# ugadiarov-la-phystech-edu/OCRL

Measured on AMD Instinct MI355X. Metric: images/sec (node) SLATE pretrain 128x128, 6 slots, 3 iters, higher is better.
Workload: dtype f32

## Files before the change

ocrl_amd/_lib.py:

```python
import ctypes
import os
from ctypes import c_void_p

from . import _abi

_HERE = os.path.dirname(os.path.abspath(__file__))
LIB_PATH = os.environ.get("OCRL_HIP_LIB") or os.path.join(_HERE, "libocrl_hip.so")
HEADER_PATH = os.path.join(_HERE, os.pardir, "include", "ocrl_hip.h")
DQN_HEADER_PATH = os.path.join(_HERE, os.pardir, "include", "ocrl_hip_dqn.h")
ROLLOUT_HEADER_PATH = os.path.join(_HERE, os.pardir, "include", "ocrl_hip_rollout.h")
_lib = None

if not os.path.exists(HEADER_PATH):
    raise RuntimeError(f"{HEADER_PATH} is missing: ocrl_amd derives its binding of libocrl_hip.so from the header and runs from the source tree.")
with open(HEADER_PATH) as _f:
    ABI = _abi.read(_f.read())
CONSTANTS = ABI.consts
SlateConfig, IodineConfig, GemmDesc, ConvDesc, ConvWgradDesc, XattnDesc, AcnetDesc, SpriteEnvDesc, ScenesDesc, FlatSegment = (
    ABI.structs["ocrl_" + n] for n in ("slate_config", "iodine_config", "gemm_desc", "conv_desc", "conv_wgrad_desc", "xattn_desc", "acnet_desc",
                                       "sprite_env_desc", "scenes_desc", "flat_segment"))
FLAT_MAX_SEGMENTS = CONSTANTS["OCRL_FLAT_MAX_SEGMENTS"]
if not os.path.exists(DQN_HEADER_PATH):
    raise RuntimeError(f"{DQN_HEADER_PATH} is missing: ocrl_amd derives its binding of libocrl_hip.so from the header and runs from the source tree.")
with open(DQN_HEADER_PATH) as _f:
    ABI_DQN = _abi.read(_f.read())
QnetDesc = ABI_DQN.structs["ocrl_qnet_desc"]
QNET_MAX_LAYERS = len(QnetDesc().dims)
if not os.path.exists(ROLLOUT_HEADER_PATH):
    raise RuntimeError(f"{ROLLOUT_HEADER_PATH} is missing: ocrl_amd derives its binding of libocrl_hip.so from the header and runs from the source tree.")
with open(ROLLOUT_HEADER_PATH) as _f:
    ABI_ROLLOUT = _abi.read(_f.read())


def flat_segments(segs):
    addr = lambda a: a.value if isinstance(a, c_void_p) else a
    return (FlatSegment * len(segs))(*[FlatSegment(addr(p), addr(g), addr(s0), addr(s1), int(n)) for p, g, s0, s1, n in segs])


def acnet_desc(B, F, A, dims, acts):
    d = AcnetDesc(B=B, F=F, A=A)
    for t in range(3):
        if len(dims[t]) > CONSTANTS["OCRL_ACNET_MAX_LAYERS"]:
            raise ValueError(f"ocrl_amd: at most {CONSTANTS['OCRL_ACNET_MAX_LAYERS']} layers per trunk (got {len(dims[t])})")
        d.n[t] = len(dims[t])
        for l, (w, a) in enumerate(zip(dims[t], acts[t])):
            d.dims[t][l], d.acts[t][l] = int(w), int(a)
    return d


def qnet_desc(B, F, A, dims, acts):
    if len(dims) > QNET_MAX_LAYERS or len(acts) != len(dims):
        raise ValueError(f"ocrl_amd: at most {QNET_MAX_LAYERS} hidden layers, one activation code each (got {len(dims)}, {len(acts)})")
    d = QnetDesc(B=B, F=F, A=A, n=len(dims))
    for l, (w, a) in enumerate(zip(dims, acts)):
        d.dims[l], d.acts[l] = int(w), int(a)
    return d


def gemm_desc(**kw):
    d = GemmDesc(batch=1, batch_inner=1, splitk=1, alpha=1.0, x_scale=1.0, e_scale=1.0, force_sb=-1)
    for k, v in kw.items():
        setattr(d, k, v)
    return d


def conv_desc(**kw):
    d = ConvDesc()
    for k, v in kw.items():
        setattr(d, k, v)
    return d


def conv_wgrad_desc(**kw):
    d = ConvWgradDesc()
    for k, v in kw.items():
        setattr(d, k, v)
    return d


def lib():
    global _lib
    if _lib is not None:
        return _lib
    if not os.path.exists(LIB_PATH):
        raise RuntimeError(
            f"{LIB_PATH} is missing: build it with `python -c 'import __graft_entry__ as g; g.build()'` "
            "(make -C ocrl_amd/csrc).  ocrl_amd has no CPU fallback.")
    import torch
    L = ctypes.CDLL(LIB_PATH)
    for abi in (ABI, ABI_DQN, ABI_ROLLOUT):
        for name, (restype, argtypes) in abi.functions.items():
            f = getattr(L, name)
            f.argtypes = argtypes
            if restype is not ctypes.c_int:
                f.restype = restype
    for name, cls in {**ABI.structs, **ABI_DQN.structs}.items():
        if name + "_size" in {**ABI.functions, **ABI_DQN.functions} and getattr(L, name + "_size")() != ctypes.sizeof(cls):
            raise RuntimeError(f"libocrl_hip.so: {name} is {getattr(L, name + '_size')()} bytes, this binding's {cls.__name__} {ctypes.sizeof(cls)}")
    if L.ocrl_abi_version() != CONSTANTS["OCRL_ABI_VERSION"]:
        raise RuntimeError(f"libocrl_hip.so ABI version mismatch: the library is {L.ocrl_abi_version()}, include/ocrl_hip.h {CONSTANTS['OCRL_ABI_VERSION']}")
    _lib = L
    return L


def check(rc):
    if rc:
        raise RuntimeError("ocrl_hip: " + lib().ocrl_last_error().decode())


def ptr(t):
    return None if t is None else ctypes.c_void_p(t.data_ptr())


def ptrs(ts):
    return (ctypes.c_void_p * len(ts))(*[t.data_ptr() if t is not None else None for t in ts])


def stream(device=None):
    import torch
    return ctypes.c_void_p(torch.cuda.current_stream(device).cuda_stream)
```

ocrl_amd/csrc/kernels.h:

```cpp
#pragma once
#include "common.h"
#include "../../include/ocrl_hip.h"

enum { PROF_CONV5 = 0, PROF_CONV_OTHER = 1, PROF_WGRAD = 2, PROF_GEMM = 3, PROF_SA_FWD = 4, PROF_SA_BWD = 5, PROF_ATTN_FWD = 6, PROF_ATTN_BWD = 7, PROF_NTAGS = 8 };
int prof_begin(int tag, hipStream_t st);
void prof_end(int idx, hipStream_t st);

struct GemmArgs {
    const float* A = nullptr;
    const float* B = nullptr;
    float* C = nullptr;
    int M = 0, N = 0, K = 0;
    int lda = 0, ldb = 0, ldc = 0;
    int akc = 1, bkc = 1;
    int batch = 1;
    int batch_inner = 1;
    long long sA = 0, sB = 0, sC = 0;
    long long sAi = 0, sBi = 0, sCi = 0;
    int splitk = 1;
    long long sCsplit = 0;
    float alpha = 1.f;
    const float* bias = nullptr;
    int relu = 0;
    float drop_p = 0.f;
    unsigned long long drop_seed = 0;
    unsigned drop_site = 0;
    const float* mask = nullptr; int ldmask = 0; long long sMask = 0;
    int mask_elu = 0;
    const float* resid = nullptr; int ldr = 0; long long sR = 0;
    float adrop_p = 0.f; unsigned adrop_site = 0; int adrop_ld = 0;
    float* bias_out = nullptr; long long sBias = 0;
    int a_mode = 0, b_mode = 0;
    const float* x_lse = nullptr; const int* x_tok = nullptr; float x_scale = 1.f;
    int epi_mode = 0;
    float* stat = nullptr; float* hstat = nullptr; int* hidx = nullptr;
    const float* e1 = nullptr; const float* e2 = nullptr; unsigned long long e_seed = 0;
    const float* e_lse = nullptr; const float* e_rowvec = nullptr; float e_scale = 1.f;
    int force_tile = 0;
    int force_sb = -1;
};
inline int gemm_stat_segments(int N) { return 2 * ((N + 127) / 128); }
struct GemmPlan { int bm = 0, bn = 0, sb = 0, xf = 0, epi = 0, layout = 0; };
int gemm_plan(const GemmArgs& a, GemmPlan* plan);
int gemm_launch(const GemmArgs& a, hipStream_t st);
int splitk_reduce_launch(const float* part, float* out, long long n, int splits, long long stride,
                         int accumulate, hipStream_t st);
void gemm_splitk_layout(GemmArgs& a, float* ws, long long bslab);
int gemm_splitk_launch(GemmArgs a, float* ws, long long bslab, int accumulate, hipStream_t st);

struct Drop { float p = 0.f; unsigned long long seed = 0; unsigned site = 0; };
struct Xf { int a_mode = 0, b_mode = 0; const float* lse = nullptr; const int* tok = nullptr; float scale = 1.f; };
int lin_fwd(const float* x, int ldx, const float* W, const float* b, float* y, int ldy, long long M, int N, int K, int relu, const float* resid,
            int ldr, hipStream_t st, Drop dr = Drop());
int lin_bwd_x(const float* dy, int ld_dy, const float* W, float* dx, int ldx, long long M, int N_out, int K_in, const float* mask, int ldmask,
              const float* resid, int ldr, hipStream_t st, Drop dr = Drop(), Xf xf = Xf(), float alpha = 1.f);
int lin_bwd_w(const float* dy, int ld_dy, const float* x, int ldx, float* dW, float* db, long long M, int N_out, int K_in, float alpha, float* sk,
              size_t sk_floats, hipStream_t st, Drop dr = Drop(), Xf xf = Xf(), int accumulate = 0, int max_splits = 0);

int pool_embed_launch(const float* lin, const float* cls, const float* pos, float* x0, int B, int K, int d, hipStream_t st);
int pool_rows_launch(const float* in, float* out, int B, int K, int d, int mode, hipStream_t st);
int pool_attn_launch(const float* qkv, float* P, float* O, const float* dO, float* dqkv, int B, int S, int d, int h, float p, unsigned long long seed,
                     unsigned site, int backward, hipStream_t st);

int pool_cols_launch(const float* src, int lds, float* dst, int ldd, long long rows, int ncols, int ncopy, hipStream_t st);
int pool_cls_drop_launch(const float* x, const float* resid, int ldr, float* out, int B, int N, int S, float p, unsigned long long seed, unsigned site,
                         hipStream_t st);
int pool_cls_add_launch(float* dX, const float* v, int B, int d, int S, hipStream_t st);
int pool_cls_nchunk(int B, int S, int* chunk);
struct PoolClsArgs {
    const float* X = nullptr;
    const float* Win = nullptr; const float* bin = nullptr;
    const float* q = nullptr;
    float* U = nullptr;
    float* part = nullptr;
    float* z = nullptr;
    float* stat = nullptr;
    float* o = nullptr;
    const float* dO = nullptr;
    float* G = nullptr; float* gD = nullptr;
    float* dX = nullptr;
    float* w = nullptr; float* dq = nullptr;
    const float* x0 = nullptr;
    float* dW = nullptr; float* db = nullptr;
    int B = 0, S = 0, d = 0, h = 0;
    float p = 0.f; unsigned long long seed = 0; unsigned site = 0;
};
int pool_cls_attn_fwd_launch(const PoolClsArgs& a, hipStream_t st);
int pool_cls_attn_bwd_launch(const PoolClsArgs& a, hipStream_t st);
int pool_flash_launch(const float* qkv, float* O, float* lse, const float* dO, float* Dd, float* dqkv, int B, int S, int d, int h, float p,
                      unsigned long long seed, unsigned site, int backward, hipStream_t st);

int rn_pair_fwd_launch(const float* AB, const float* b1, float* h1, int B, int K, int g, hipStream_t st);
int rn_pair_bwd_launch(const float* dh1, float* dAB, int B, int K, int g, hipStream_t st);
int rn_pairsum_fwd_launch(const float* gL, float* y, int B, int P, int g, hipStream_t st);
int rn_pairsum_bwd_launch(const float* dy, const float* gL, float* dgL, int B, int P, int g, hipStream_t st);

struct NcMap { long long sN = 0, sG = 0, sC = 0, sH = 0, sW = 0; };
struct NcFwdArgs {
    const float* X = nullptr; NcMap x;
    float* Y = nullptr; float* Y2 = nullptr; NcMap y;
    const float* w[OCRL_NATURECNN_MAX_GROUPS] = {}; const float* bias[OCRL_NATURECNN_MAX_GROUPS] = {};
    int B = 0, G = 1, cin = 0, cout = 0, H = 0, W = 0, OH = 0, OW = 0, ks = 0, stride = 0;
    int pad = 0;
};
struct NcBwdArgs {
    const float* X = nullptr; NcMap x;
    const float* dY = nullptr; NcMap dy;
    float* dX = nullptr;
    float* part = nullptr;
    int slabs = 1, slab_rows = 0;
    const float* w[OCRL_NATURECNN_MAX_GROUPS] = {};
    int B = 0, G = 1, cin = 0, cout = 0, H = 0, W = 0, OH = 0, OW = 0, ks = 0, stride = 0;
    int pad = 0;
    long long dw_tiles = 0, dx_tiles = 0; int dw_blocks = 0;
};
struct NcReduceLayer { const float* part = nullptr; int slabs = 0, G = 0, cout = 0, K = 0; long long n = 0; };
struct NcReduceArgs {
    NcReduceLayer L[OCRL_NATURECNN_MAX_CONVS];
    float* dw[OCRL_NATURECNN_MAX_CONVS][OCRL_NATURECNN_MAX_GROUPS] = {};
    float* db[OCRL_NATURECNN_MAX_CONVS][OCRL_NATURECNN_MAX_GROUPS] = {};
    int nlayers = 0;
};
int nc_conv_fwd_launch(const NcFwdArgs& a, hipStream_t st);
int nc_conv_bwd_launch(NcBwdArgs a, hipStream_t st);
int nc_dw_reduce_launch(const NcReduceArgs& a, hipStream_t st);
int nc_relu_mask_launch(const float* d, const float* act, float* out, long long n, hipStream_t st);

struct PcGeom {
    int OH = 0, OW = 0, OWT = 0;
    int NG = 0, nchunk = 0;
    size_t wp_floats = 0;
    long long units = 0; int slab_units = 0, slabs = 0; size_t part_floats = 0;
    int passes = 0, nbg = 0, Dp = 0; size_t wd_floats = 0;
    int HB = 0, WB = 0, WT = 0; long long dx_units = 0; int upw = 0;
};
PcGeom pc_geom(int B, int H, int W, int D);
struct PcFwdArgs {
    const float* X = nullptr; const float* Wp = nullptr; const float* bias = nullptr; float* Y = nullptr;
    int B = 0, H = 0, W = 0, D = 0, OH = 0, OW = 0, OWT = 0, nchunk = 0, NG = 0;
};
struct PcDwArgs {
    const float* X = nullptr; const float* dY = nullptr; float* part = nullptr; float* partb = nullptr;
    int B = 0, H = 0, W = 0, D = 0, OH = 0, OW = 0, OWT = 0, nchunk = 0, slab_units = 0;
    long long units = 0;
};
struct PcDxArgs {
    const float* dY = nullptr; const float* Wd = nullptr; float* dX = nullptr;
    int H = 0, W = 0, D = 0, OH = 0, OW = 0, HB = 0, WT = 0, Dp = 0, passes = 0, upw = 0;
    long long units = 0, groups = 0;
};
int pc_conv1_fwd_launch(const float* X, const float* w, const float* bias, float* Wp, float* Y, int B, int H, int W, int D, hipStream_t st);
int pc_conv1_dw_launch(const float* X, const float* dY, float* part, int B, int H, int W, int D, hipStream_t st);
int pc_conv1_dw_reduce_launch(const float* part, float* dw, float* db, int B, int H, int W, int D, hipStream_t st);
int pc_conv1_dx_launch(const float* dY, const float* w, float* Wd, float* dX, int B, int H, int W, int D, hipStream_t st);

#define PROBE_MAX_SLOTS 12
#define PROBE_MAX_PROPS 8
#define PROBE_MAX_WIDTH 256
struct ProbeSchema { int P; int t[PROBE_MAX_PROPS], a[PROBE_MAX_PROPS], b[PROBE_MAX_PROPS], kind[PROBE_MAX_PROPS]; };
int probe_schema_check(const ProbeSchema& sc, int T, int O);
int probe_match_check(int B, int K, int N, int T, int O);
int probe_match_launch(const float* out, int ld_row, long long ld_img, const float* y, const float* dloss, float* cost, int* col, float* part,
                       float* metrics, float* dout, int B, int K, int N, int T, int O, const ProbeSchema& sc, hipStream_t st);
int probe_leaky_fwd_launch(float* x, long long n, float slope, hipStream_t st);
int probe_leaky_bwd_launch(float* dx, const float* h, long long n, float slope, hipStream_t st);

int vae_permute_launch(const float* src, float* dst, long long R, int C, int HW, int rows, int pack, hipStream_t st);
int vae_pad_rows_launch(const float* src, float* dst, int rows, int rows_pad, int K, hipStream_t st);
int vae_kl_fwd_launch(const float* ml, const float* eps, float* latent, float* part, float* rep, int B, int L, hipStream_t st);
int vae_loss_launch(const float* part, float* metrics, int B, float kld_weight, hipStream_t st);
int vae_kl_bwd_launch(const float* ml, const float* eps, const float* dlat, const float* drep, const float* dloss, float* dml, int B, int L,
                      float kld_weight, hipStream_t st);
int vae_scale_launch(const float* x, float* y, const float* g, long long n, hipStream_t st);
int vae_recon_nchw_launch(const float* r4, float* out, int B, int C, int HW, hipStream_t st);

#define MAE_MAX_PATCHES 1024
int mae_rank_launch(const float* noise, int* restore, int* keep, float* mask, int* restore_out, float* mask_out, int B, int L, int len_keep,
                    hipStream_t st);
int mae_patch_gather_launch(const float* obs, const int* ids, float* out, int B, int n, int S, int p, hipStream_t st);
int mae_tokens_fwd_launch(const float* embed, const float* cls, const float* pos, const int* ids, float* x0, int B, int n, int D, hipStream_t st);
int mae_tokens_bwd_launch(const float* dx0, float* dembed, float* dcls, int B, int n, int D, hipStream_t st);
int mae_unshuffle_fwd_launch(const float* e, const float* mtok, const float* dpos, const int* restore, float* xd, int B, int L, int len_keep, int Dd,
                             hipStream_t st);
int mae_unshuffle_bwd_launch(const float* dxd, const int* keep, const float* mask, float* de, float* dmtok, float* part, int B, int L, int len_keep,
                             int Dd, hipStream_t st);
int mae_gelu_fwd_launch(const float* pre, float* y, long long n, hipStream_t st);
int mae_gelu_bwd_launch(const float* dy, const float* pre, float* dpre, long long n, hipStream_t st);
int mae_ln_fwd_launch(const float* x, const float* g, const float* b, float* y, float* mean, float* rstd, long long R, int F, float eps, hipStream_t st);
int mae_ln_chunks(long long R);
int mae_ln_bwd_launch(const float* dy, const float* x, const float* mean, const float* rstd, const float* g, const float* resid, float* dx, float* dg,
                      float* db, float* part, long long R, int F, hipStream_t st);
int mae_loss_launch(const float* pred, const float* obs, const float* mask, const float* dloss, float* part, float* loss, float* dpred, int B, int L,
                    int len_keep, int S, int p, hipStream_t st);

struct ConvArgs {
    const float* X = nullptr;
    const float* Wp = nullptr;
    float* Y = nullptr;
    int B = 0, H = 0, W = 0;
    const float* bias = nullptr;
    int relu = 0;
    const float* posmap = nullptr;
    const float* mask = nullptr;
    int mask_elu = 0;
};
size_t conv_x3_pack_floats(int KS = 5);
int conv_pack_x3_launch(const float* W, float* fwd3, float* bwd3, hipStream_t st, int KS = 5);
int conv_x3_launch(const ConvArgs& a, const float* pack3, hipStream_t st, int KS = 5);
struct WgradArgs;
int conv_wgrad_x3_stage(const WgradArgs& a, int nchunk, hipStream_t st, int KS = 5);
struct WgradArgs {
    const float* X = nullptr;
    const float* dY = nullptr;
    float* part = nullptr;
    int B = 0, H = 0, W = 0;
    float* bpart = nullptr;
};
int conv_fwd_launch(const ConvArgs& a, int KS, int CIN, int COUT, hipStream_t st, int low_latency = 0);
int conv_wgrad_launch(const WgradArgs& a, int KS, int CIN, int COUT, int cin_real, float* dW, float* db, int accumulate, hipStream_t st, int x3 = -1);
int conv_wgrad_slabs(int B, int H, int W, int KS, int CIN);
size_t conv_wgrad_ws_floats(int B, int H, int W, int KS, int CIN, bool with_db = true);
int conv_pack_launch(const float* W, float* fwd, float* bwd, int KS, int CIN, int COUT, int cin_real, hipStream_t st);

size_t conv_first_pack_floats();
int conv_first_pack_launch(const float* W, float* pack, hipStream_t st);
int conv_first_fwd_launch(const float* obs, const float* pack, const float* bias, float* Y, int B, int H, int W, int relu, hipStream_t st);
int conv_first_wgrad_workers(int B, int H, int W);
size_t conv_first_wgrad_ws_floats(int B, int H, int W);
int conv_first_wgrad_launch(const float* obs, const float* dY, float* ws, float* dW, float* db, int B, int H, int W, int accumulate, hipStream_t st);

int nchw_to_nhwc8_launch(const float* in, float* out, int B, int C, int H, int W, hipStream_t st);
int patchify4_launch(const float* in, float* out, int B, int C, int S, hipStream_t st);
int pixel_shuffle_launch(const float* in, float* out, int B, int h, int w, int Cout, int forward, const float* mask, hipStream_t st);
int layernorm_fwd_launch(const float* x, const float* g, const float* b, float* y, float* mean, float* rstd, long long R, int F, hipStream_t st);
int layernorm_bwd_launch(const float* dy, const float* x, const float* mean, const float* rstd, const float* g, float* dx,
                         float* dgb, long long R, int F, int accumulate_dx, int accumulate_dgb, float* ws, size_t ws_floats, hipStream_t st);
int colsum_launch(const float* X, long long ld, float* out, long long R, int F, int accumulate, float scale, float* ws, size_t ws_floats, hipStream_t st);

#define SA_INPUT_SLAB (2 * 4096 + 4 * 64)
void sa_input_plan(long long R, int max_wgs, int out[3]);
int sa_input_fwd_launch(const float* e4, const float* gamma, const float* beta, const float* W0, const float* b0, const float* W2, const float* b2,
                        float* mean, float* rstd, float* ln0, float* h1, float* x, long long R, int max_wgs, hipStream_t st);
int sa_input_bwd_launch(const float* dx, const float* h1, const float* e4, const float* mean, const float* rstd, const float* gamma, const float* beta,
                        const float* W0, const float* W2, float* de4, float* dW0, float* db0, float* dW2, float* db2, float* dgamma, float* dbeta,
                        long long R, int max_wgs, float* ws, size_t ws_floats, hipStream_t st);
int reduce_partials_launch(const float* part, int n, float* out, float scale, int accumulate, hipStream_t st);
int mse_launch(const float* obs, const float* recon, float* drecon, float* out, int B, int C, int H, int W, float* ws, size_t ws_floats, hipStream_t st);
int gumbel_softmax_launch(const float* raw, const float* e1, const float* e2, float* z, int* tokens, long long R, int V, float tau,
                          unsigned long long seed, hipStream_t st, float* zst = nullptr);
int softmax_bwd_rows_launch(const float* z, float* d, long long R, int V, float scale, hipStream_t st);
int softmax_stat_combine_launch(const float* stat, int nseg, long long R, float* lse, const float* hstat, const int* hidx, int* tokens,
                                const float* pred, int ldp, const int* tok, float* out, float scale, float* ws, size_t ws_floats, hipStream_t st,
                                const float* cdf_scores = nullptr, int cdf_V = 0, float cdf_tau = 1.f, unsigned long long cdf_seed = 0);
int exp_rows_launch(const float* y, const float* lse, float* z, long long R, int V, hipStream_t st);
int rowdot_bias64_launch(const float* g, const float* act, const float* bias, long long R, float* out, hipStream_t st);
int embed_fwd_launch(const int* tokens, const float* dict, const float* bos, const float* pe, float* out, int B, int T, int d, float p,
                     unsigned long long seed, hipStream_t st);
size_t embed_bwd_ws_floats(long long BT, int V, int d);
int embed_bwd_launch(float* g, const int* tokens, float* ddict, int B, int T, int V, int d, float p, unsigned long long seed, float* ws,
                     size_t ws_floats, hipStream_t st);
int dropout_apply_launch(const float* x, float* y, long long n, float p, unsigned long long seed, unsigned site, hipStream_t st);
int dropout_mask_launch(float* y, long long n, float p, unsigned long long seed, unsigned site, hipStream_t st);
int obs_u8_to_f32_launch(const unsigned char* in, float* out, int B, int H, int W, int C, hipStream_t st);
int fill_launch(float* x, long long n, float v, hipStream_t st);
int axpy_launch(const float* x, float* y, long long n, float a, hipStream_t st);
int posmap_launch(const float* Wpos, const float* bpos, float* out, int S, int C, hipStream_t st);
int posgrid_launch(float* out, int S, hipStream_t st);
int im2col5_launch(const float* x8, float* col, long long npix, int H, int W, int C, int ldc, hipStream_t st);
int unpack5_launch(const float* dWp, float* dW, int C, int ldc, hipStream_t st);
int pad_cols_launch(const float* in, int ldi, float* out, int ldo, long long R, int C, int Cout, hipStream_t st);

struct XaPlan { bool supported = false; int KP = 0, NC = 0, NM = 0; size_t lds = 0; };
bool xattn_plan(int K, int d, int h, XaPlan* out);
bool xattn_supported(int K, int d, int h);
int xattn_kp(int K, int h);
struct XaFoldHost {
    const float* mem = nullptr;
    const float* Wq[8]; const float* Wk[8]; const float* Wv[8]; const float* Wo[8];
    float* ck[8]; float* cv[8];
    float* Ab[8]; float* AbT[8]; float* Vo[8]; float* VoT[8];
    int B = 0, K = 0, d = 0, h = 0, nblk = 0;
};
int xattn_fold_fwd_launch(const XaFoldHost& f, hipStream_t st);
struct XaHost {
    const float* x = nullptr;
    const float* resid = nullptr;
    float* y = nullptr;
    float* P = nullptr;
    const float *Ab = nullptr, *AbT = nullptr, *Vo = nullptr, *VoT = nullptr;
    const float* gd = nullptr;
    float *Pd = nullptr, *dS = nullptr;
    int B = 0, T = 0, K = 0, d = 0, h = 0;
    float p = 0.f; unsigned long long seed = 0; unsigned site_p = 0, site_o = 0;
};
int xattn_launch(const XaHost& h, int backward, hipStream_t st);
struct XaFoldBwdHost {
    const float *Pd = nullptr, *dS = nullptr;
    const float *gd = nullptr, *x = nullptr;
    const float *Wq = nullptr, *Wo = nullptr;
    const float *ck = nullptr, *cv = nullptr;
    float *dVo = nullptr, *dAb = nullptr;
    float *dck = nullptr, *dcv = nullptr;
    float *pq = nullptr, *po = nullptr;
    float *dWq = nullptr, *dWo = nullptr;
    float* ws = nullptr; size_t ws_floats = 0;
    int B = 0, T = 0, K = 0, d = 0, h = 0;
};
int xattn_fold_bwd_launch(const XaFoldBwdHost& f, hipStream_t st);
int cross_attn_fwd_launch(const float* Q, const float* Km, const float* Vm, float* O, float* P, int B, int T, int K, int d, int h, float p,
                          unsigned long long seed, unsigned site, hipStream_t st);
size_t cross_attn_bwd_ws_floats(int B, int T, int K, int d, int h);
int cross_attn_bwd_launch(const float* dO, const float* Q, const float* Km, const float* Vm, const float* P, float* dQ, float* dKm, float* dVm,
                          int B, int T, int K, int d, int h, float p, unsigned long long seed, unsigned site, float* part, size_t part_floats,
                          hipStream_t st);


struct SaWts {
    int ln_in_g, ln_in_b, ln_s_g, ln_s_b, ln_m_g, ln_m_b;
    int Wq, WqT, Wk, WkT, Wv, WvT, Wih, WihT, Whh, WhhT, bih, bhh, W0, W0T, b0, W2, W2T, b2;
    int total;
};
static inline SaWts sa_wts_layout(int C, int D, int H) {
    SaWts o; int a = 0;
    auto take = [&](int n) { int r = a; a += (n + 3) & ~3; return r; };
    o.ln_in_g = take(C); o.ln_in_b = take(C); o.ln_s_g = take(D); o.ln_s_b = take(D); o.ln_m_g = take(D); o.ln_m_b = take(D);
    o.Wq = take(D * D); o.WqT = take(D * D); o.Wk = take(D * C); o.WkT = take(C * D); o.Wv = take(D * C); o.WvT = take(C * D);
    o.Wih = take(3 * D * D); o.WihT = take(3 * D * D); o.Whh = take(3 * D * D); o.WhhT = take(3 * D * D);
    o.bih = take(3 * D); o.bhh = take(3 * D);
    o.W0 = take(H * D); o.W0T = take(H * D); o.b0 = take(H); o.W2 = take(D * H); o.W2T = take(D * H); o.b2 = take(D);
    o.total = a;
    return o;
}
struct SaSave { int sprev, sn, q, u, r, z, n, hn, sg, m, hid, qp, up, upn, csum, ld; };
static inline SaSave sa_save_layout(int C, int D, int H, int NH = 1) {
    SaSave o;
    o.sprev = 0; o.sn = D; o.q = 2 * D; o.u = 3 * D; o.r = 4 * D; o.z = 5 * D; o.n = 6 * D; o.hn = 7 * D; o.sg = 8 * D; o.m = 9 * D;
    o.hid = 10 * D; o.qp = 10 * D + H; o.up = o.qp + NH * C; o.upn = o.up + NH * C; o.csum = o.upn + NH * C; o.ld = o.csum + ((NH + 3) & ~3);
    return o;
}
struct SaGrad { int out, hid, gi, gh, u, q, qp, ld; };
static inline SaGrad sa_grad_layout(int C, int D, int H, int NH = 1) {
    SaGrad o;
    o.out = 0; o.hid = D; o.gi = D + H; o.gh = 4 * D + H; o.u = 7 * D + H; o.q = 8 * D + H; o.qp = 9 * D + H; o.ld = 9 * D + H + NH * C;
    return o;
}
struct SlotAttnArgs {
    int B = 0, N = 0, C = 64, K = 0, D = 0, H = 0, I = 0;
    int NH = 1;
    float eps = 1e-8f, scale = 1.f;
    const float* x = nullptr;
    const float* slots0 = nullptr;
    const float* wts = nullptr;
    float* slots = nullptr;
    float* attn = nullptr;
    float* attn_heads = nullptr;
    float* save = nullptr;
    const float* dslots = nullptr;
    float* dx = nullptr;
    float* dslots0 = nullptr;
    float* grows = nullptr;
    float* g_small = nullptr;
    float* xchg = nullptr;
    float* parts = nullptr;
    int phase = 0;
};
size_t sa_xchg_floats_host(int K, int D);
size_t sa_parts_floats_host(int B, int K);
struct SaPlan { int G, NB, KB, KS; size_t smem_fwd, smem_bwd; };
int sa_plan(int K, int D, int H, int NH, SaPlan* plan);
int slot_attn_launch(const SlotAttnArgs& a, int backward, hipStream_t st);

struct PackEntry { const float* src; int rows, cols, dst_off, transpose; };
int pack_launch(const PackEntry* entries_dev, int n_entries, int max_elems, float* dst, hipStream_t st);

int absmax_launch(const float* g, long long n, float* out, float* ws, size_t ws_floats, hipStream_t st);
int clip_adam_launch(float* p, const float* g, float* m, float* v, long long n, const float* norm, float clip, float lr, double b1,
                     double b2, double eps, int step, float gscale, hipStream_t st);
int clip_adam_tail_launch(float* p, const float* g, float* m, float* v, int n, const float* norm, float clip, float lr, double b1, double b2,
                          double eps, int step, float gscale, hipStream_t st);
int clip_rmsprop_launch(float* p, const float* g, float* sq, long long n, const float* norm, float clip, float lr, double alpha, double eps,
                        hipStream_t st);
int clip_rmsprop_tail_launch(float* p, const float* g, float* sq, int n, const float* norm, float clip, float lr, double alpha, double eps,
                             hipStream_t st);
constexpr int FLAT_MAX_SEG = 8, FLAT_SEG_BLOCKS = 1024;
struct FlatSegs {
    float* p[FLAT_MAX_SEG];
    const float* g[FLAT_MAX_SEG];
    float* s0[FLAT_MAX_SEG];
    float* s1[FLAT_MAX_SEG];
    long long n[FLAT_MAX_SEG];
    int blk0[FLAT_MAX_SEG + 1];
    int nseg;
};
int multi_clip_adam_launch(FlatSegs t, float* norm, float clip, float lr, double b1, double b2, double eps, int step, float* ws, size_t ws_floats,
                           hipStream_t st);
int multi_clip_rmsprop_launch(FlatSegs t, float* norm, float clip, float lr, double alpha, double eps, float* ws, size_t ws_floats, hipStream_t st);
int store_u64_launch(unsigned long long* dst, unsigned long long v, hipStream_t st);
int slot_init_launch(const float* mu, const float* logsig, const float* noise, float* slots0, int BK, int D, unsigned long long seed, hipStream_t st,
                     const unsigned long long* seed_dev = nullptr);
int slot_init_bwd_launch(const float* dslots0, const float* logsig, const float* noise, float* dmu, float* dlogsig, int BK, int D, unsigned long long seed, hipStream_t st);
int copy_launch(const float* src, float* dst, long long n, hipStream_t st);
int argmax_pos_launch(const float* pred, int* tokens, int B, int T, int V, int t, hipStream_t st, int dense_rows = 0);
int embed_step_launch(const int* tokens, const float* dict, const float* bos, const float* pe, float* out, int B, int T, int d, int t, hipStream_t st);
int decode_attn_launch(const float* qkv, float* out, int B, int T, int t, int d, int h, int ld, hipStream_t st);
int onehot_launch(const int* tokens, float* z, long long rows, int V, hipStream_t st);

struct AttnArgs {
    const float *q = nullptr, *k = nullptr, *v = nullptr;
    float* o = nullptr;
    float* lse = nullptr;
    int B = 0, T = 0, d = 0, h = 0;
    int ld = 0;
    float p = 0.f;
    unsigned long long seed = 0;
    unsigned site = 0;
    const float* dO = nullptr;
    float *dq = nullptr, *dk = nullptr, *dv = nullptr, *delta = nullptr;
    float* ds = nullptr;
    size_t ds_floats = 0;
    int b0 = 0;
};
int attn_launch(const AttnArgs& a, int mode, hipStream_t st);
size_t attn_bwd_ds_floats(int B, int T, int h);
int attn_bwd_form();
size_t attn_bwd_ds_carve_floats(int B, int T, int h);

enum { BCAST_L1_RELU = 0, BCAST_L1_ELU = 1 };
int bcast_l1_class_sum_launch(const float* in, float* out, long long BK, int ks, int forward, hipStream_t st);
int bcast_l1_fwd_launch(const float* P1, const float* T, const float* bias, float* c1, long long BK, int S, int ks, int act, hipStream_t st);
size_t bcast_l1_bwd_ws_floats(long long BK, int S, int ks);
int bcast_l1_bwd_launch(const float* g, float* dT, long long BK, int S, int ks, float* ws, size_t ws_floats, hipStream_t st);
int bc_posconv_launch(const float* Wc, float* P1, int S, hipStream_t st);
int bc_posconv_bwd_launch(const float* G, float* dWc, int S, hipStream_t st);
int io_p1_launch(const float* Wxy, const float* b1, float* P1, int S, hipStream_t st);
int io_w1_grad_launch(const float* dW1r, const float* G, float* dW1, float* db1, int S, int L, hipStream_t st);

int bc_compose_launch(const float* W1, const float* Wpos, const float* bpos, float* Wc, float* W1r, int D, hipStream_t st);
int bc_compose_bwd_launch(const float* W1, const float* Wpos, const float* bpos, const float* dWc, const float* dW1r, float* dW1,
                          float* dWpos, float* dbpos, int D, hipStream_t st);
int bc_c4_pack_launch(const float* W, float* Wk, float* Wb, int co_n, hipStream_t st);
int bc_c4_fwd_launch(const float* X, const float* Wk, const float* bias4, float* Y, int Bn, int S, hipStream_t st);
int bc_c4_bwd_data_launch(const float* dY, const float* Wb, const float* act, float* dX, int Bn, int S, hipStream_t st, int elu = 0);
int bc_c4_wgrad_blocks(int Bn, int S);
int bc_c4_wgrad_launch(const float* X, const float* dY, float* part, int Bn, int S, hipStream_t st);
int bc_mix_launch(const float* out4, const float* obs, float* recon, float* dout4, float* loss_out, int B, int K, int S, int C, float* ws,
                  size_t ws_floats, hipStream_t st);

int io_sample_launch(const float* mu, const float* ls, const float* noise, float* eps_out, float* slots, float* kl_out, long long n,
                     unsigned long long seed, unsigned site, float* ws, size_t ws_floats, hipStream_t st);
int io_w1_pack_launch(const float* W1, float* W1r, float* Wxy, int L, hipStream_t st);
int io_elbo_launch(const float* out4, const float* obs, int B, int K, int S, float sigma, float* enc, float* st1, float* dout4, float* part,
                   float* masks_out, float* recon_out, float* rmasked_out, float* ws, size_t ws_floats, hipStream_t st);
int io_enc_norm_launch(float* enc, const float* st1, float* st2, long long BK, int N, float* ws, size_t ws_floats, hipStream_t st);
int io_elbo_bwd_launch(const float* out4, const float* obs, const float* denc, int B, int K, int S, float sigma, float cw, float* dout4, hipStream_t st);
int io_latent_launch(const float* mu, const float* ls, const float* eps, const float* ds, float* latent, long long BK, int L, float beta, int layer_norm,
                     int ld, hipStream_t st);
int io_im2col_launch(const float* x, float* col, long long Bn, int C, int Hi, int Wi, int ldc, hipStream_t st);
int io_col2im_launch(const float* dcol, const float* act, float* dx, long long Bn, int C, int Hi, int Wi, int ldc, hipStream_t st);
int io_refw_pack_launch(const float* W, float* Wp, int C, int ldc, hipStream_t st);
int io_refw_unpack_launch(const float* dWp, float* dW, int C, int ldc, hipStream_t st);
int io_pool_launch(const float* r, float* pool, long long BK, int n, hipStream_t st);
int io_pool_bwd_launch(const float* dpool, const float* r, float* dpre, long long BK, int n, hipStream_t st);
int io_elu2_launch(const float* a, int lda, float* y, int ldy, long long rows, int F, const float* dy, int lddy, hipStream_t st);
int io_lstm_fwd_launch(const float* gates, const float* c0, float* acts, float* c1, float* h1, long long rows, int H, hipStream_t st);
int io_lstm_bwd_launch(const float* acts, const float* c0, const float* c1, const float* dh1, const float* dc1, float* dgates, float* dc0,
                       long long rows, int H, hipStream_t st);
int io_post_grad_launch(const float* mu, const float* ls, const float* eps, const float* ds, const float* dlat, int ldl, float kw, float* gmu,
                        float* gls, long long BK, int L, hipStream_t st);
int io_l2norm_launch(const float* g, long long n, float* out, float* ws, size_t ws_floats, hipStream_t st);
int io_loss_launch(const float* parts, float* metrics, int I, int B, float beta, hipStream_t st);
```

ocrl_amd/csrc/sa_input.hip:

```cpp
#include "common.h"
#include "kernels.h"
#include "layernorm16.h"

#define SAI_TR 64
#define SAI_LD 68
#define SAI_MAX_WGS 512
#define SAI_FWD_MAX_WGS 768

__device__ __forceinline__ float4 sai_ld4(const float* __restrict__ p, long long row, long long R, int c4) {
    const float4 v = *reinterpret_cast<const float4*>(p + (row < R ? row : R - 1) * 64 + c4 * 4);
    return row < R ? v : make_float4(0.f, 0.f, 0.f, 0.f);
}
__device__ __forceinline__ float sai_ld1(const float* __restrict__ p, long long row, long long R) {
    const float v = p[row < R ? row : R - 1];
    return row < R ? v : 0.f;
}

__device__ __forceinline__ void sai_mma_kc(const float* __restrict__ as, const float (&wf)[8][4], f32x16& acc) {
    const int lane = threadIdx.x & 63, li = lane & 31, lh = lane >> 5;
#pragma unroll
    for (int c = 0; c < 8; ++c) {
        const float4 v = *reinterpret_cast<const float4*>(as + li * SAI_LD + c * 8 + 4 * lh);
        acc = __builtin_amdgcn_mfma_f32_32x32x2f32(v.x, wf[c][0], acc, 0, 0, 0);
        acc = __builtin_amdgcn_mfma_f32_32x32x2f32(v.y, wf[c][1], acc, 0, 0, 0);
        acc = __builtin_amdgcn_mfma_f32_32x32x2f32(v.z, wf[c][2], acc, 0, 0, 0);
        acc = __builtin_amdgcn_mfma_f32_32x32x2f32(v.w, wf[c][3], acc, 0, 0, 0);
    }
}
__device__ __forceinline__ void sai_mma_rows(const float* __restrict__ as, const float* __restrict__ bs, f32x16& acc) {
    const int lane = threadIdx.x & 63, li = lane & 31, lh = lane >> 5;
#pragma unroll 2
    for (int c = 0; c < 8; ++c) {
        float fa[4], fb[4];
#pragma unroll
        for (int j = 0; j < 4; ++j) {
            fa[j] = as[(c * 8 + 4 * lh + j) * SAI_LD + li];
            fb[j] = bs[(c * 8 + 4 * lh + j) * SAI_LD + li];
        }
#pragma unroll
        for (int s = 0; s < 4; ++s) acc = __builtin_amdgcn_mfma_f32_32x32x2f32(fa[s], fb[s], acc, 0, 0, 0);
    }
}

__global__ __launch_bounds__(256, 3) void sa_input_fwd_kernel(const float* __restrict__ e4, const float* __restrict__ g, const float* __restrict__ bta,
                                                              const float* __restrict__ W0, const float* __restrict__ b0,
                                                              const float* __restrict__ W2, const float* __restrict__ b2,
                                                              float* __restrict__ mean, float* __restrict__ rstd, float* __restrict__ ln0,
                                                              float* __restrict__ h1, float* __restrict__ x, long long R) {
    __shared__ __attribute__((aligned(16))) float At[SAI_TR * SAI_LD], Ht[SAI_TR * SAI_LD];
    const int lane = threadIdx.x & 63, wv = threadIdx.x >> 6, c4 = lane & 15, rsub = lane >> 4;
    const int li = lane & 31, lh = lane >> 5;
    const int wm0 = (wv >> 1) * 32, wn0 = (wv & 1) * 32;
    float w0f[8][4], w2f[8][4];
#pragma unroll
    for (int c = 0; c < 8; ++c) {
        const float4 a = *reinterpret_cast<const float4*>(W0 + (wn0 + li) * 64 + c * 8 + 4 * lh);
        const float4 b = *reinterpret_cast<const float4*>(W2 + (wn0 + li) * 64 + c * 8 + 4 * lh);
        w0f[c][0] = a.x; w0f[c][1] = a.y; w0f[c][2] = a.z; w0f[c][3] = a.w;
        w2f[c][0] = b.x; w2f[c][1] = b.y; w2f[c][2] = b.z; w2f[c][3] = b.w;
    }
    const float b0v = b0[wn0 + li], b2v = b2[wn0 + li];
    const float4 gg = *reinterpret_cast<const float4*>(g + c4 * 4), bb = *reinterpret_cast<const float4*>(bta + c4 * 4);
    const long long ntiles = (R + SAI_TR - 1) / SAI_TR;
    const int lr0 = wv * 16 + rsub;
    float4 v[4];
#pragma unroll
    for (int i = 0; i < 4; ++i) v[i] = sai_ld4(e4, (long long)blockIdx.x * SAI_TR + lr0 + 4 * i, R, c4);
    for (long long tile = blockIdx.x; tile < ntiles; tile += gridDim.x) {
        const long long r0 = tile * SAI_TR;
#pragma unroll
        for (int i = 0; i < 4; ++i) {
            const int lr = lr0 + 4 * i;
            const long long row = r0 + lr;
            float mu, rs;
            layernorm16_row_fwd<1>(&v[i], mu, rs);
            const float4 y = layernorm16_affine(v[i], rs, gg, bb);
            *reinterpret_cast<float4*>(At + lr * SAI_LD + c4 * 4) = y;
            if (row < R) {
                if (ln0) *reinterpret_cast<float4*>(ln0 + row * 64 + c4 * 4) = y;
                if (c4 == 0) { mean[row] = mu; rstd[row] = rs; }
            }
        }
#pragma unroll
        for (int i = 0; i < 4; ++i) v[i] = sai_ld4(e4, (tile + gridDim.x) * SAI_TR + lr0 + 4 * i, R, c4);
        __syncthreads();
        f32x16 acc;
#pragma unroll
        for (int r = 0; r < 16; ++r) acc[r] = 0.f;
        sai_mma_kc(At + wm0 * SAI_LD, w0f, acc);
#pragma unroll
        for (int r = 0; r < 16; ++r) {
            const int row = (r & 3) + 8 * (r >> 2) + 4 * lh;
            Ht[(wm0 + row) * SAI_LD + wn0 + li] = fmaxf(acc[r] + b0v, 0.f);
        }
        __syncthreads();
#pragma unroll
        for (int r = 0; r < 16; ++r) acc[r] = 0.f;
        sai_mma_kc(Ht + wm0 * SAI_LD, w2f, acc);
#pragma unroll
        for (int r = 0; r < 16; ++r) {
            const int row = (r & 3) + 8 * (r >> 2) + 4 * lh;
            At[(wm0 + row) * SAI_LD + wn0 + li] = acc[r] + b2v;
        }
        __syncthreads();
#pragma unroll
        for (int i = 0; i < 4; ++i) {
            const int lr = lr0 + 4 * i;
            const long long row = r0 + lr;
            if (row < R) {
                *reinterpret_cast<float4*>(h1 + row * 64 + c4 * 4) = *reinterpret_cast<const float4*>(Ht + lr * SAI_LD + c4 * 4);
                *reinterpret_cast<float4*>(x + row * 64 + c4 * 4) = *reinterpret_cast<const float4*>(At + lr * SAI_LD + c4 * 4);
            }
        }
        __syncthreads();
    }
}

__global__ __launch_bounds__(256, 2) void sa_input_bwd_kernel(const float* __restrict__ dx, const float* __restrict__ h1, const float* __restrict__ e4,
                                                              const float* __restrict__ mean, const float* __restrict__ rstd,
                                                              const float* __restrict__ g, const float* __restrict__ bta,
                                                              const float* __restrict__ W0, const float* __restrict__ W2,
                                                              float* __restrict__ de4, float* __restrict__ slab, long long R) {
    __shared__ __attribute__((aligned(16))) float T0[SAI_TR * SAI_LD], T1[SAI_TR * SAI_LD], T2[SAI_TR * SAI_LD], W0s[64 * 64], W2s[32 * 64];
    const int lane = threadIdx.x & 63, wv = threadIdx.x >> 6, c4 = lane & 15, rsub = lane >> 4;
    const int li = lane & 31, lh = lane >> 5;
    const int wm0 = (wv >> 1) * 32, wn0 = (wv & 1) * 32;
    float w2f[4][4];
#pragma unroll
    for (int c = 0; c < 4; ++c)
#pragma unroll
        for (int j = 0; j < 4; ++j) w2f[c][j] = W2[(c * 8 + 4 * lh + j) * 64 + wn0 + li];
#pragma unroll
    for (int i = 0; i < 4; ++i)
        *reinterpret_cast<float4*>(W0s + (threadIdx.x + 256 * i) * 4) = *reinterpret_cast<const float4*>(W0 + (threadIdx.x + 256 * i) * 4);
#pragma unroll
    for (int i = 0; i < 2; ++i)
        *reinterpret_cast<float4*>(W2s + (threadIdx.x + 256 * i) * 4) = *reinterpret_cast<const float4*>(W2 + 2048 + (threadIdx.x + 256 * i) * 4);
    f32x16 dW2a, dW0a;
#pragma unroll
    for (int r = 0; r < 16; ++r) { dW2a[r] = 0.f; dW0a[r] = 0.f; }
    float4 dg = make_float4(0.f, 0.f, 0.f, 0.f), db = dg, db2 = dg;
    float db0 = 0.f;
    const long long ntiles = (R + SAI_TR - 1) / SAI_TR;
    const int lr0 = wv * 16 + rsub;
    float4 dxn[4], hn[4];
#pragma unroll
    for (int i = 0; i < 4; ++i) {
        dxn[i] = sai_ld4(dx, (long long)blockIdx.x * SAI_TR + lr0 + 4 * i, R, c4);
        hn[i] = sai_ld4(h1, (long long)blockIdx.x * SAI_TR + lr0 + 4 * i, R, c4);
    }
    for (long long tile = blockIdx.x; tile < ntiles; tile += gridDim.x) {
        const long long r0 = tile * SAI_TR;
        float4 xe[4];
        float mu[4], rs[4];
        __syncthreads();
#pragma unroll
        for (int i = 0; i < 4; ++i) {
            const int lr = lr0 + 4 * i;
            *reinterpret_cast<float4*>(T0 + lr * SAI_LD + c4 * 4) = dxn[i];
            *reinterpret_cast<float4*>(T1 + lr * SAI_LD + c4 * 4) = hn[i];
            db2.x += dxn[i].x; db2.y += dxn[i].y; db2.z += dxn[i].z; db2.w += dxn[i].w;
            xe[i] = sai_ld4(e4, r0 + lr, R, c4);
            mu[i] = sai_ld1(mean, r0 + lr, R);
            rs[i] = sai_ld1(rstd, r0 + lr, R);
        }
#pragma unroll
        for (int i = 0; i < 4; ++i) {
            dxn[i] = sai_ld4(dx, (tile + gridDim.x) * SAI_TR + lr0 + 4 * i, R, c4);
            hn[i] = sai_ld4(h1, (tile + gridDim.x) * SAI_TR + lr0 + 4 * i, R, c4);
        }
        __syncthreads();
        f32x16 acc;
#pragma unroll
        for (int r = 0; r < 16; ++r) acc[r] = 0.f;
#pragma unroll
        for (int c = 0; c < 4; ++c) {
            const float4 a = *reinterpret_cast<const float4*>(T0 + (wm0 + li) * SAI_LD + c * 8 + 4 * lh);
            acc = __builtin_amdgcn_mfma_f32_32x32x2f32(a.x, w2f[c][0], acc, 0, 0, 0);
            acc = __builtin_amdgcn_mfma_f32_32x32x2f32(a.y, w2f[c][1], acc, 0, 0, 0);
            acc = __builtin_amdgcn_mfma_f32_32x32x2f32(a.z, w2f[c][2], acc, 0, 0, 0);
            acc = __builtin_amdgcn_mfma_f32_32x32x2f32(a.w, w2f[c][3], acc, 0, 0, 0);
        }
#pragma unroll 2
        for (int c = 4; c < 8; ++c) {
            const float4 a = *reinterpret_cast<const float4*>(T0 + (wm0 + li) * SAI_LD + c * 8 + 4 * lh);
            const float* const wk = W2s + ((c - 4) * 8 + 4 * lh) * 64 + wn0 + li;
            acc = __builtin_amdgcn_mfma_f32_32x32x2f32(a.x, wk[0], acc, 0, 0, 0);
            acc = __builtin_amdgcn_mfma_f32_32x32x2f32(a.y, wk[64], acc, 0, 0, 0);
            acc = __builtin_amdgcn_mfma_f32_32x32x2f32(a.z, wk[128], acc, 0, 0, 0);
            acc = __builtin_amdgcn_mfma_f32_32x32x2f32(a.w, wk[192], acc, 0, 0, 0);
        }
#pragma unroll
        for (int r = 0; r < 16; ++r) {
            const int idx = (wm0 + (r & 3) + 8 * (r >> 2) + 4 * lh) * SAI_LD + wn0 + li;
            const float mk = T1[idx];
            float t = acc[r];
            t = mk > 0.f ? t : 0.f * t * (mk + 1.f);
            T2[idx] = t;
            db0 += t;
        }
        sai_mma_rows(T0 + wm0, T1 + wn0, dW2a);
        __syncthreads();
        const float4 gg = *reinterpret_cast<const float4*>(g + c4 * 4), bb = *reinterpret_cast<const float4*>(bta + c4 * 4);
#pragma unroll
        for (int i = 0; i < 4; ++i) {
            const float4 dd = make_float4(xe[i].x - mu[i], xe[i].y - mu[i], xe[i].z - mu[i], xe[i].w - mu[i]);
            *reinterpret_cast<float4*>(T1 + (lr0 + 4 * i) * SAI_LD + c4 * 4) = layernorm16_affine(dd, rs[i], gg, bb);
        }
#pragma unroll
        for (int r = 0; r < 16; ++r) acc[r] = 0.f;
#pragma unroll 2
        for (int c = 0; c < 8; ++c) {
            const float4 a = *reinterpret_cast<const float4*>(T2 + (wm0 + li) * SAI_LD + c * 8 + 4 * lh);
            const float* const wk = W0s + (c * 8 + 4 * lh) * 64 + wn0 + li;
            acc = __builtin_amdgcn_mfma_f32_32x32x2f32(a.x, wk[0], acc, 0, 0, 0);
            acc = __builtin_amdgcn_mfma_f32_32x32x2f32(a.y, wk[64], acc, 0, 0, 0);
            acc = __builtin_amdgcn_mfma_f32_32x32x2f32(a.z, wk[128], acc, 0, 0, 0);
            acc = __builtin_amdgcn_mfma_f32_32x32x2f32(a.w, wk[192], acc, 0, 0, 0);
        }
#pragma unroll
        for (int r = 0; r < 16; ++r) T0[(wm0 + (r & 3) + 8 * (r >> 2) + 4 * lh) * SAI_LD + wn0 + li] = acc[r];
        __syncthreads();
        sai_mma_rows(T2 + wm0, T1 + wn0, dW0a);
#pragma unroll
        for (int i = 0; i < 4; ++i) {
            const int lr = lr0 + 4 * i;
            const long long row = r0 + lr;
            const float4 yv = *reinterpret_cast<const float4*>(T0 + lr * SAI_LD + c4 * 4);
            const Ln16Bwd<1> r = layernorm16_row_bwd<1>(&xe[i], &yv, mu[i], rs[i], &gg, &dg, &db);
            if (row < R) *reinterpret_cast<float4*>(de4 + row * 64 + c4 * 4) = layernorm16_row_dx(r, rs[i], 0);
        }
    }
    float* const sl = slab + (size_t)blockIdx.x * SA_INPUT_SLAB;
#pragma unroll
    for (int r = 0; r < 16; ++r) {
        const int o = (wm0 + (r & 3) + 8 * (r >> 2) + 4 * lh) * 64 + wn0 + li;
        sl[o] = dW2a[r];
        sl[4096 + o] = dW0a[r];
    }
    __syncthreads();
    float4* const red = reinterpret_cast<float4*>(T0);
    red[(0 * 16 + wv * 4 + rsub) * 16 + c4] = db2;
    red[(1 * 16 + wv * 4 + rsub) * 16 + c4] = dg;
    red[(2 * 16 + wv * 4 + rsub) * 16 + c4] = db;
    T1[(wv * 2 + lh) * 32 + li] = db0;
    __syncthreads();
    if (threadIdx.x < 48) {
        const int which = threadIdx.x >> 4, c = threadIdx.x & 15;
        float4 a = red[(which * 16) * 16 + c];
#pragma unroll
        for (int k = 1; k < 16; ++k) { const float4 t = red[(which * 16 + k) * 16 + c]; a.x += t.x; a.y += t.y; a.z += t.z; a.w += t.w; }
        *reinterpret_cast<float4*>(sl + 8192 + (which == 0 ? 0 : which == 1 ? 128 : 192) + c * 4) = a;
    } else if (threadIdx.x >= 64 && threadIdx.x < 128) {
        const int col = threadIdx.x - 64, wn = col >> 5, i = col & 31;
        sl[8192 + 64 + col] = ((T1[((0 * 2 + wn) * 2 + 0) * 32 + i] + T1[((0 * 2 + wn) * 2 + 1) * 32 + i]) +
                               (T1[((1 * 2 + wn) * 2 + 0) * 32 + i] + T1[((1 * 2 + wn) * 2 + 1) * 32 + i]));
    }
}

__global__ __launch_bounds__(256) void sa_input_reduce_kernel(const float* __restrict__ slab, int nslab, float* __restrict__ dW2, float* __restrict__ dW0,
                                                              float* __restrict__ db2, float* __restrict__ db0, float* __restrict__ dgam,
                                                              float* __restrict__ dbet) {
    __shared__ float red[8][32];
    const int ci = threadIdx.x & 31, grp = threadIdx.x >> 5, col = blockIdx.x * 32 + ci;
    const int per = (nslab + 7) / 8, s0 = grp * per, s1 = min(nslab, s0 + per);
    float a = 0.f;
    for (int s = s0; s < s1; ++s) a += slab[(size_t)s * SA_INPUT_SLAB + col];
    red[grp][ci] = a;
    __syncthreads();
    if (threadIdx.x < 32) {
        float t = red[0][ci];
#pragma unroll
        for (int k = 1; k < 8; ++k) t += red[k][ci];
        float* out = col < 4096 ? dW2 + col : col < 8192 ? dW0 + (col - 4096) : col < 8256 ? db2 + (col - 8192) : col < 8320 ? db0 + (col - 8256)
                   : col < 8384 ? dgam + (col - 8320) : dbet + (col - 8384);
        *out = t;
    }
}

void sa_input_plan(long long R, int max_wgs, int out[3]) {
    const long long ntiles = (R + SAI_TR - 1) / SAI_TR;
    long long wgs = max_wgs > 0 && max_wgs < SAI_MAX_WGS ? max_wgs : SAI_MAX_WGS;
    if (wgs > ntiles) wgs = ntiles;
    out[0] = SAI_TR; out[1] = (int)wgs; out[2] = SA_INPUT_SLAB;
}

int sa_input_fwd_launch(const float* e4, const float* gamma, const float* beta, const float* W0, const float* b0, const float* W2, const float* b2,
                        float* mean, float* rstd, float* ln0, float* h1, float* x, long long R, int max_wgs, hipStream_t st) {
    OCRL_REQUIRE(R > 0, "sa_input_fwd: no rows");
    OCRL_REQUIRE(e4 && gamma && beta && W0 && b0 && W2 && b2 && mean && rstd && h1 && x, "sa_input_fwd: null argument");
    OCRL_REQUIRE(aligned16(e4, gamma, beta, W0, W2, ln0, h1, x), "sa_input_fwd: tensors must be 16-byte aligned");
    const long long ntiles = (R + SAI_TR - 1) / SAI_TR;
    long long wgs = max_wgs > 0 && max_wgs < SAI_FWD_MAX_WGS ? max_wgs : SAI_FWD_MAX_WGS;
    if (wgs > ntiles) wgs = ntiles;
    hipLaunchKernelGGL(sa_input_fwd_kernel, dim3((unsigned)wgs), dim3(256), 0, st, e4, gamma, beta, W0, b0, W2, b2, mean, rstd, ln0, h1, x, R);
    OCRL_CHECK_LAUNCH("sa_input_fwd");
    return 0;
}

int sa_input_bwd_launch(const float* dx, const float* h1, const float* e4, const float* mean, const float* rstd, const float* gamma, const float* beta,
                        const float* W0, const float* W2, float* de4, float* dW0, float* db0, float* dW2, float* db2, float* dgamma, float* dbeta,
                        long long R, int max_wgs, float* ws, size_t ws_floats, hipStream_t st) {
    OCRL_REQUIRE(R > 0, "sa_input_bwd: no rows");
    OCRL_REQUIRE(dx && h1 && e4 && mean && rstd && gamma && beta && W0 && W2 && de4 && dW0 && db0 && dW2 && db2 && dgamma && dbeta && ws,
                 "sa_input_bwd: null argument");
    OCRL_REQUIRE(aligned16(dx, h1, e4, gamma, beta, W0, de4, ws), "sa_input_bwd: tensors must be 16-byte aligned");
    int plan[3];
    sa_input_plan(R, max_wgs, plan);
    OCRL_REQUIRE((size_t)plan[1] * SA_INPUT_SLAB <= ws_floats, "sa_input_bwd: workspace too small (%d slabs of %d floats)", plan[1], SA_INPUT_SLAB);
    hipLaunchKernelGGL(sa_input_bwd_kernel, dim3(plan[1]), dim3(256), 0, st, dx, h1, e4, mean, rstd, gamma, beta, W0, W2, de4, ws, R);
    OCRL_CHECK_LAUNCH("sa_input_bwd");
    hipLaunchKernelGGL(sa_input_reduce_kernel, dim3(SA_INPUT_SLAB / 32), dim3(256), 0, st, ws, plan[1], dW2, dW0, db2, db0, dgamma, dbeta);
    OCRL_CHECK_LAUNCH("sa_input_reduce");
    return 0;
}
```

ocrl_amd/csrc/slate_model.cpp:

```cpp
#include "slate_model.h"

#include "switches.h"

#include <math.h>
#include <stdarg.h>
#include <string.h>

static std::string fmt(const char* f, ...) {
    char buf[256];
    va_list ap;
    va_start(ap, f);
    vsnprintf(buf, sizeof buf, f, ap);
    va_end(ap);
    return buf;
}

SlateModel::SlateModel(const SlateConfig& c) : cfg(c) {
    S = c.obs_size; E = S / 4; T = E * E; N = S * S; V = c.vocab; d = c.d_model; C = c.cnn_hidden;
    K = c.num_slots; I = c.num_iters; D = c.slot_size; H = c.mlp_hidden; NB = c.num_blocks; NH = c.num_heads;
    DH = d / NH; Bmax = c.max_batch; SH = c.slot_heads > 0 ? c.slot_heads : 1;
    const int ch = c.obs_channels;
    add_param("_dvae._encoder.0.m.weight", {64, ch, 4, 4}, 0); add_param("_dvae._encoder.0.m.bias", {64}, 0);
    for (int i = 1; i < 7; ++i) { add_param(fmt("_dvae._encoder.%d.m.weight", i), {64, 64, 1, 1}, 0); add_param(fmt("_dvae._encoder.%d.m.bias", i), {64}, 0); }
    add_param("_dvae._encoder.7.weight", {V, 64, 1, 1}, 0); add_param("_dvae._encoder.7.bias", {V}, 0);
    const int di[9] = {0, 1, 2, 3, 4, 6, 7, 8, 9};
    const int dshape[9][4] = {{64, V, 1, 1}, {64, 64, 3, 3}, {64, 64, 1, 1}, {64, 64, 1, 1}, {256, 64, 1, 1},
                              {64, 64, 3, 3}, {64, 64, 1, 1}, {64, 64, 1, 1}, {256, 64, 1, 1}};
    for (int i = 0; i < 9; ++i) {
        add_param(fmt("_dvae._decoder.%d.m.weight", di[i]), {dshape[i][0], dshape[i][1], dshape[i][2], dshape[i][3]}, 0);
        add_param(fmt("_dvae._decoder.%d.m.bias", di[i]), {dshape[i][0]}, 0);
    }
    add_param("_dvae._decoder.11.weight", {ch, 64, 1, 1}, 0); add_param("_dvae._decoder.11.bias", {ch}, 0);
    add_param("_enc._encoder.0.m.weight", {C, ch, 5, 5}, 1); add_param("_enc._encoder.0.m.bias", {C}, 1);
    for (int i = 1; i < 3; ++i) { add_param(fmt("_enc._encoder.%d.m.weight", i), {C, C, 5, 5}, 1); add_param(fmt("_enc._encoder.%d.m.bias", i), {C}, 1); }
    add_param("_enc._encoder.3.weight", {C, C, 5, 5}, 1); add_param("_enc._encoder.3.bias", {C}, 1);
    add_param("_enc_pos.channels_map.weight", {C, 4, 1, 1}, 1); add_param("_enc_pos.channels_map.bias", {C}, 1);
    add_param("_slotattn.slot_mu", {1, 1, D}, 1); add_param("_slotattn.slot_log_sigma", {1, 1, D}, 1);
    add_param("_slotattn.layer_norm.weight", {C}, 1); add_param("_slotattn.layer_norm.bias", {C}, 1);
    add_param("_slotattn.mlp.0.weight", {C, C}, 1); add_param("_slotattn.mlp.0.bias", {C}, 1);
    add_param("_slotattn.mlp.2.weight", {C, C}, 1); add_param("_slotattn.mlp.2.bias", {C}, 1);
    const std::string sa = "_slotattn.slot_attention.";
    add_param(sa + "norm_inputs.weight", {C}, 1); add_param(sa + "norm_inputs.bias", {C}, 1);
    add_param(sa + "norm_slots.weight", {D}, 1); add_param(sa + "norm_slots.bias", {D}, 1);
    add_param(sa + "norm_mlp.weight", {D}, 1); add_param(sa + "norm_mlp.bias", {D}, 1);
    add_param(sa + "project_q.weight", {D, D}, 1); add_param(sa + "project_k.weight", {D, C}, 1); add_param(sa + "project_v.weight", {D, C}, 1);
    add_param(sa + "gru.weight_ih", {3 * D, D}, 1); add_param(sa + "gru.weight_hh", {3 * D, D}, 1);
    add_param(sa + "gru.bias_ih", {3 * D}, 1); add_param(sa + "gru.bias_hh", {3 * D}, 1);
    add_param(sa + "mlp.0.weight", {H, D}, 1); add_param(sa + "mlp.0.bias", {H}, 1);
    add_param(sa + "mlp.2.weight", {D, H}, 1); add_param(sa + "mlp.2.bias", {D}, 1);
    add_param("_slotproj.weight", {d, D}, 1);
    if (c.use_bcdec) {
        add_param("_dec._decoder.0.m.weight", {C, D, 5, 5}, 1); add_param("_dec._decoder.0.m.bias", {C}, 1);
        for (int i = 1; i < 3; ++i) { add_param(fmt("_dec._decoder.%d.m.weight", i), {C, C, 5, 5}, 1); add_param(fmt("_dec._decoder.%d.m.bias", i), {C}, 1); }
        add_param("_dec._decoder.3.weight", {ch + 1, C, 3, 3}, 1); add_param("_dec._decoder.3.bias", {ch + 1}, 1);
        add_param("_dec._pos_emb.channels_map.weight", {D, 4, 1, 1}, 1); add_param("_dec._pos_emb.channels_map.bias", {D}, 1);
    }
    add_param("_dict.dictionary.weight", {V, d}, 2);
    add_param("_bos_token._bos_token", {1, 1, d}, 2);
    add_param("_z_pos.pe", {1, 1 + T, d}, 2);
    for (int b = 0; b < NB; ++b) {
        const std::string p = fmt("_tfdec.blocks.%d.", b);
        add_param(p + "self_attn_layer_norm.weight", {d}, 2); add_param(p + "self_attn_layer_norm.bias", {d}, 2);
        for (const char* q : {"q", "k", "v", "o"}) add_param(p + "self_attn.proj_" + q + ".weight", {d, d}, 2);
        add_param(p + "encoder_decoder_attn_layer_norm.weight", {d}, 2); add_param(p + "encoder_decoder_attn_layer_norm.bias", {d}, 2);
        for (const char* q : {"q", "k", "v", "o"}) add_param(p + "encoder_decoder_attn.proj_" + q + ".weight", {d, d}, 2);
        add_param(p + "ffn_layer_norm.weight", {d}, 2); add_param(p + "ffn_layer_norm.bias", {d}, 2);
        add_param(p + "ffn.0.weight", {4 * d, d}, 2); add_param(p + "ffn.0.bias", {4 * d}, 2);
        add_param(p + "ffn.2.weight", {d, 4 * d}, 2); add_param(p + "ffn.2.bias", {d}, 2);
    }
    add_param("_tfdec.layer_norm.weight", {d}, 2); add_param("_tfdec.layer_norm.bias", {d}, 2);
    add_param("_out.weight", {V, d}, 2);

    finish_params(group_begin_, 3);
    resolve_params();
    blk_.resize(NB);
    conv_x3_ = (int)sw::model<sw::OCRL_CONV_X3>();
    attn_ds_floats_ = attn_bwd_ds_carve_floats(Bmax, T, NH);
    layout_workspace(false);
}

void SlateModel::resolve_params() {
    Weights& w = w_;
    for (int i = 0; i < 8; ++i) w.dvae_enc[i] = ref_pair(fmt(i < 7 ? "_dvae._encoder.%d.m" : "_dvae._encoder.%d", i));
    for (int i = 0; i < 12; ++i)
        if (i != 5 && i != 10) w.dvae_dec[i] = ref_pair(fmt(i < 11 ? "_dvae._decoder.%d.m" : "_dvae._decoder.%d", i));
    for (int i = 0; i < 4; ++i) w.enc[i] = ref_pair(fmt(i < 3 ? "_enc._encoder.%d.m" : "_enc._encoder.%d", i));
    w.enc_pos = ref_pair("_enc_pos.channels_map");
    w.sa.mu = ref("_slotattn.slot_mu"); w.sa.log_sigma = ref("_slotattn.slot_log_sigma");
    w.sa.ln = ref_pair("_slotattn.layer_norm"); w.sa.mlp0 = ref_pair("_slotattn.mlp.0"); w.sa.mlp2 = ref_pair("_slotattn.mlp.2");
    for (int i = 0; i < SA_NW; ++i) w.sa.w[i] = ref(std::string("_slotattn.slot_attention.") + SA_WEIGHT_NAMES[i]);
    w.slotproj = ref("_slotproj.weight");
    if (cfg.use_bcdec) {
        for (int i = 0; i < 4; ++i) w.bc[i] = ref_pair(fmt(i < 3 ? "_dec._decoder.%d.m" : "_dec._decoder.%d", i));
        w.bc_pos = ref_pair("_dec._pos_emb.channels_map");
    }
    w.dict = ref("_dict.dictionary.weight"); w.bos = ref("_bos_token._bos_token"); w.pe = ref("_z_pos.pe");
    w.blk.resize(NB);
    for (int b = 0; b < NB; ++b) {
        const std::string p = fmt("_tfdec.blocks.%d.", b);
        DecBlockW& k = w.blk[b];
        k.ln1 = ref_pair(p + "self_attn_layer_norm"); k.ln2 = ref_pair(p + "encoder_decoder_attn_layer_norm"); k.ln3 = ref_pair(p + "ffn_layer_norm");
        k.qkv = ref(p + "self_attn.proj_q.weight"); k.o = ref(p + "self_attn.proj_o.weight");
        k.cq = ref(p + "encoder_decoder_attn.proj_q.weight"); k.ck = ref(p + "encoder_decoder_attn.proj_k.weight");
        k.cv = ref(p + "encoder_decoder_attn.proj_v.weight"); k.co = ref(p + "encoder_decoder_attn.proj_o.weight");
        k.ffn0 = ref_pair(p + "ffn.0"); k.ffn2 = ref_pair(p + "ffn.2");
    }
    w.lnf = ref_pair("_tfdec.layer_norm"); w.out = ref("_out.weight");
    w.enc_grads_end = group_begin_[2];
    for (const ParamInfo& q : params_)
        if (q.group == 1 && (q.name.rfind("_slotproj.", 0) == 0 || q.name.rfind("_dec.", 0) == 0) && q.offset < w.enc_grads_end) w.enc_grads_end = q.offset;
}

SlateModel::~SlateModel() {
    if (ev_fork_) (void)hipEventDestroy(ev_fork_);
    if (ev_join_) (void)hipEventDestroy(ev_join_);
    if (ev_tokens_) (void)hipEventDestroy(ev_tokens_);
    if (side_) (void)hipStreamDestroy(side_);
    for (auto& kv : enc_graphs_) if (kv.second.exec) (void)hipGraphExecDestroy(kv.second.exec);
    for (hipEvent_t e : ev_dw_) if (e) (void)hipEventDestroy(e);
    if (ev_join2_) (void)hipEventDestroy(ev_join2_);
    if (side2_) (void)hipStreamDestroy(side2_);
    if (cap_) (void)hipStreamDestroy(cap_);
}

void SlateModel::layout_workspace(bool commit) {
    begin_layout(commit);
    x3_of_.clear();
    const size_t B = Bmax, BT = B * T, BN = B * N, BK = B * K;
    metrics_ = carve("metrics", 64);
    scratch_floats_ = 0;
    {
        size_t need = conv_wgrad_ws_floats((int)(B * (cfg.use_bcdec ? K : 1)), S, S, 5, 64) + (size_t)512 * 2304 * 2;
        if (conv_first_wgrad_ws_floats((int)B, S, S) > need) need = conv_first_wgrad_ws_floats((int)B, S, S);
        size_t sk = (size_t)32 * V * d + (size_t)(1 << 20);
        if (sk > need) need = sk;
        size_t cs = (size_t)N * C * 8 + (size_t)T * d * 8 + (1 << 20);
        if (cs > need) need = cs;
        if (cfg.use_bcdec && bcast_l1_bwd_ws_floats((long long)BK, S, 5) > need) need = bcast_l1_bwd_ws_floats((long long)BK, S, 5);
        const size_t ca = cross_attn_bwd_ws_floats((int)B, T, K, d, NH), eb = embed_bwd_ws_floats((long long)B * T, V, d);
        if (ca > need) need = ca;
        if (eb > need) need = eb;
        scratch_floats_ = need + (1 << 20);
    }
    scratch_ = carve(nullptr, scratch_floats_);
    scratch2_ = cfg.use_bcdec ? scratch_ : carve(nullptr, scratch_floats_);
    obs8_ = first_direct() ? nullptr : carve("obs8", BN * 8);
    obs_keep_ = first_direct() ? carve(nullptr, BN * cfg.obs_channels) : nullptr;
    obs_stage_ = carve(nullptr, (B < 32 ? B : 32) * (size_t)cfg.obs_channels * N);
    seed_dev_ = reinterpret_cast<unsigned long long*>(carve(nullptr, 64));
    e1_ = carve("enc1", BN * 64); e2_ = carve("enc2", BN * 64); e3_ = carve("enc3", BN * 64); e4_ = carve("feats", BN * 64);
    posmap_ = carve(nullptr, (size_t)N * C); gridT_ = carve(nullptr, (size_t)N * 4);
    ln0_ = carve(nullptr, BN * 64); ln0_mean_ = carve(nullptr, BN); ln0_rstd_ = carve(nullptr, BN);
    h1_ = carve("sa_mlp_hidden", BN * 64); x_ = carve("sa_inputs", BN * 64);
    slots0_ = carve("slots0", BK * D); slot_noise_ = carve(nullptr, BK * D); slots_ = carve("slots", BK * D);
    attn_ = carve("attn", BN * K);
    attn_heads_ = SH > 1 ? carve(nullptr, sa_attn_heads_floats(B, N, K, SH)) : nullptr;
    const SaSizes sz = sa_sizes(B, K, C, D, H, I, SH);
    sa_save_ = carve("sa_save", sz.save);
    sa_grows_ = carve(nullptr, sz.grows);
    sa_wts_ = carve(nullptr, sz.wts);
    sa_small_ = carve(nullptr, sz.small);
    sa_xchg_ = carve(nullptr, sz.xchg);
    sa_parts_ = carve(nullptr, sz.parts);
    sa_pack_dev_ = reinterpret_cast<PackEntry*>(carve(nullptr, sz.table));
    for (int i = 0; i < 4; ++i) {
        const int cin = i == 0 ? 8 : 64;
        cw_fwd_[i] = carve(nullptr, (size_t)25 * cin * 64);
        cw_bwd_[i] = i == 0 ? nullptr : carve(nullptr, (size_t)25 * 64 * 64);
        if (conv_x3_ && i > 0) {
            float* f3 = carve(nullptr, conv_x3_pack_floats());
            float* b3 = carve(nullptr, conv_x3_pack_floats());
            if (ws_commit_) { x3_of_[cw_fwd_[i]] = f3; x3_of_[cw_bwd_[i]] = b3; }
        }
    }
    gslots_ = carve(nullptr, BK * D); gslots0_ = carve(nullptr, BK * D);
    gA_ = carve(nullptr, BN * 64); gB_ = carve(nullptr, BN * 64); gC_ = cfg.use_bcdec ? gA_ : carve(nullptr, BN * 64);
    gmap_ = carve(nullptr, (size_t)N * C);
    if (cfg.use_bcdec) {
        const size_t BKN = BK * (size_t)N;
        bc_Wc_ = carve(nullptr, 25 * 64 * 5 + 64); bc_W1r_ = carve(nullptr, (size_t)25 * 64 * D); bc_P1_ = carve(nullptr, (size_t)N * 64);
        bc_M_ = carve(nullptr, BK * 1600); bc_T_ = carve(nullptr, BK * 1600);
        bc_c1_ = carve("bc_c1", BKN * 64); bc_c2_ = carve("bc_c2", BKN * 64); bc_c3_ = carve("bc_c3", BKN * 64);
        bc_out4_ = carve(nullptr, BKN * 4); bc_dout4_ = carve(nullptr, BKN * 4);
        bc_gA_ = carve(nullptr, BKN * 64); bc_gB_ = carve(nullptr, BKN * 64);
        for (int i = 0; i < 2; ++i) {
            bc_pk_[i] = carve(nullptr, 25 * 64 * 64); bc_pkb_[i] = carve(nullptr, 25 * 64 * 64);
            if (conv_x3_ > 0) {
                float* f3 = carve(nullptr, conv_x3_pack_floats());
                float* b3 = carve(nullptr, conv_x3_pack_floats());
                if (ws_commit_) { x3_of_[bc_pk_[i]] = f3; x3_of_[bc_pkb_[i]] = b3; }
            }
        }
        bc_Wk4_ = carve(nullptr, 9 * 64 * 4); bc_Wb4_ = carve(nullptr, 9 * 64 * 4);
        bc_dW1r_ = carve(nullptr, (size_t)25 * 64 * D); bc_dWc_ = carve(nullptr, 25 * 64 * 5 + 64);
        bc_dT_ = carve(nullptr, BK * 1600); bc_dM_ = carve(nullptr, BK * 1600); bc_G1_ = carve(nullptr, (size_t)N * 64);
        recon_ = carve("recon", BN * 4);
    } else {
    patches_ = carve("patches", BT * 16 * cfg.obs_channels);
    for (int i = 0; i < 7; ++i) de_[i] = carve(fmt("dvae_enc%d", i).c_str(), BT * 64);
    zraw_ = carve("zraw", BT * V);
    z_ = carve("z", BT * V);
    zdec_ = cfg.hard ? carve("z_st", BT * V) : z_;
    tokens_ = reinterpret_cast<int*>(carve("tokens", BT));
    {
        const size_t nseg = (size_t)gemm_stat_segments(V);
        zstat_ = carve(nullptr, BT * nseg * 2); zhstat_ = carve(nullptr, BT * nseg); zhidx_ = reinterpret_cast<int*>(carve(nullptr, BT * nseg));
        zlse_ = carve("z_lse", BT); zdot_ = carve(nullptr, BT);
        cestat_ = carve(nullptr, BT * nseg * 2); celse_ = carve("ce_lse", BT); cepart_ = carve(nullptr, BT / 16 + 16);
    }
    dd0_ = carve("dvae_dec0", BT * 64); dd1_ = carve("dvae_dec1", BT * 64); dd2_ = carve("dvae_dec2", BT * 64); dd3_ = carve("dvae_dec3", BT * 64);
    dd4_ = carve("dvae_dec4", BT * 256); ps1_ = carve(nullptr, BT * 256);
    dd6_ = carve("dvae_dec6", BT * 256); dd7_ = carve("dvae_dec7", BT * 256); dd8_ = carve("dvae_dec8", BT * 256);
    dd9_ = carve("dvae_dec9", BT * 1024); ps2_ = carve(nullptr, BN * 64);
    recon_ = carve("recon", BN * 4); drecon_ = carve(nullptr, BN * 4);
    for (int i = 0; i < 2; ++i) {
        dw_fwd_[i] = carve(nullptr, 9 * 64 * 64); dw_bwd_[i] = carve(nullptr, 9 * 64 * 64);
        if (conv_x3_ > 0) {
            float* f3 = carve(nullptr, conv_x3_pack_floats(3));
            float* b3 = carve(nullptr, conv_x3_pack_floats(3));
            if (ws_commit_) { x3_of_[dw_fwd_[i]] = f3; x3_of_[dw_bwd_[i]] = b3; }
        }
    }
    w11p_ = carve(nullptr, 4 * 64);
    mem_ = carve("mem", BK * d); emb_ = carve("emb", BT * d);
    for (int b = 0; b < NB; ++b) {
        Blk& k = blk_[b];
        k.ln1 = carve(nullptr, BT * d); k.ln1_mean = carve(nullptr, BT); k.ln1_rstd = carve(nullptr, BT);
        k.q = carve(nullptr, BT * 3 * d); k.k = k.q + d; k.v = k.q + 2 * d;
        k.lse = carve(nullptr, B * NH * (size_t)T); k.ao = carve(nullptr, BT * d); k.x1 = carve(nullptr, BT * d);
        k.ln2 = carve(nullptr, BT * d); k.ln2_mean = carve(nullptr, BT); k.ln2_rstd = carve(nullptr, BT);
        k.cq = carve(nullptr, BT * d); k.ck = carve(nullptr, BK * d); k.cv = carve(nullptr, BK * d);
        k.cP = carve(nullptr, B * NH * (size_t)T * K); k.cao = carve(nullptr, BT * d); k.x2 = carve(nullptr, BT * d);
        k.ln3 = carve(nullptr, BT * d); k.ln3_mean = carve(nullptr, BT); k.ln3_rstd = carve(nullptr, BT);
        k.f1 = carve(fmt("blk%d.ffn_hidden", b).c_str(), BT * 4 * d); k.x3 = carve(nullptr, BT * d);
    }
    bg_.resize(NB);
    {
        const size_t NC = xattn_supported(K, d, NH) ? (size_t)NH * xattn_kp(K, NH) : 16;
        xa_zero_base_ = carve_pos();
        for (int b = 0; b < NB; ++b) {
            Blk& k = blk_[b];
            k.xaAb = carve(nullptr, B * NC * d); k.xaAbT = carve(nullptr, B * NC * d); k.xaVo = carve(nullptr, B * NC * d); k.xaVoT = carve(nullptr, B * NC * d);
        }
        xa_zero_floats_ = (size_t)(carve_pos() - xa_zero_base_);
        for (int b = 0; b < NB; ++b) { bg_[b].xaPd = carve(nullptr, BT * NC); bg_[b].xaDs = carve(nullptr, BT * NC); }
        xa_dAb_ = carve(nullptr, B * NC * d); xa_dVo_ = carve(nullptr, B * NC * d);
        xa_pq_ = carve(nullptr, B * (size_t)d * d); xa_po_ = carve(nullptr, B * (size_t)d * d);
    }
    attn_delta_ = carve(nullptr, B * NH * (size_t)T);
    attn_ds_ = attn_ds_floats_ ? carve(nullptr, attn_ds_floats_) : nullptr;
    lnf_ =carve("dec_out", BT * d); lnf_mean_ = carve(nullptr, BT); lnf_rstd_ = carve(nullptr, BT);
    pred_ = carve("pred", BT * V);
    gx_ = carve(nullptr, BT * d); gbr_ = carve(nullptr, BT * d); gt1_ = carve(nullptr, BT * d); gt2_ = carve(nullptr, BT * d);
    gt3_ = carve(nullptr, BT * d); gf1_ = carve(nullptr, BT * 4 * d); gqkv_ = carve(nullptr, BT * 3 * d);
    for (int b = 0; b < NB; ++b) {
        BlkG& q = bg_[b];
        if (b == 0) { q.gbr[0] = gbr_; q.gf1 = gf1_; q.gt2 = gt2_; q.gqkv = gqkv_; }
        else { q.gbr[0] = carve(nullptr, BT * d); q.gf1 = carve(nullptr, BT * 4 * d); q.gt2 = carve(nullptr, BT * d); q.gqkv = carve(nullptr, BT * 3 * d); }
        q.gbr[1] = carve(nullptr, BT * d); q.gbr[2] = carve(nullptr, BT * d);
    }
    scratch3_ = carve(nullptr, scratch_floats_);
    gmem_ = carve(nullptr, BK * d); gck_ = carve(nullptr, BK * d); gcv_ = carve(nullptr, BK * d);
    gdA_ = carve(nullptr, BN * 64); gdB_ = carve(nullptr, BN * 64);
    }
    col0_ = dw0p_ = nullptr;
    if (!first_direct()) {
        const int ldc0 = (25 * cfg.obs_channels + 3) & ~3;
        col0_ = carve(nullptr, BN * ldc0); dw0p_ = carve(nullptr, (size_t)64 * ldc0);
    }
    end_layout();
}

int SlateModel::bind(float* p, float* g, float* m, float* v, void* ws, size_t ws_bytes) {
    RC(check_buffers(p, g, ws, ws_bytes));
    OCRL_REQUIRE(d % 64 == 0 && d <= 256 && D % 64 == 0 && C == 64 && V % 256 == 0 && S % 4 == 0 && d % NH == 0 && DH % 4 == 0 && DH <= 64,
                 "unsupported configuration (d_model/slot_size multiples of 64 <= 256, cnn hidden 64, vocab %% 256, obs_size %% 4)");
    OCRL_REQUIRE(cfg.obs_channels == 3, "obs_channels must be 3");
    OCRL_REQUIRE(T % 4 == 0, "obs_size/4 squared must be a multiple of 4");
    adopt_buffers(p, g, m, v, ws);
    clear_encode_graphs();
    packs_valid_ = false;
    layout_workspace(true);
    if (!side_) {
        plan_ = stream_plan((int)sw::model<sw::OCRL_OVERLAP>(), (int)sw::model<sw::OCRL_DW_SIDE>(), sw::model<sw::OCRL_TOKENS_LATE>() != 0, cfg.use_bcdec);
        if (plan_.side) {
            OCRL_HIP(hipStreamCreateWithFlags(&side_, hipStreamNonBlocking));
            OCRL_HIP(hipEventCreateWithFlags(&ev_fork_, hipEventDisableTiming));
            OCRL_HIP(hipEventCreateWithFlags(&ev_join_, hipEventDisableTiming));
            OCRL_HIP(hipEventCreateWithFlags(&ev_tokens_, hipEventDisableTiming));
            if (plan_.dw) {
                for (hipEvent_t& ev : ev_dw_) OCRL_HIP(hipEventCreateWithFlags(&ev, hipEventDisableTiming));
                OCRL_HIP(hipEventCreateWithFlags(&ev_join2_, hipEventDisableTiming));
                if (plan_.dw == 2) OCRL_HIP(hipStreamCreateWithFlags(&side2_, hipStreamNonBlocking));
            }
        }
    }
    sa_input_ = (int)sw::model<sw::OCRL_SA_INPUT>();
    xattn_ = !cfg.use_bcdec && xattn_supported(K, d, NH) && sw::model<sw::OCRL_XATTN>() != 0;
    if (!cfg.use_bcdec && xa_zero_floats_) OCRL_HIP(hipMemset(xa_zero_base_, 0, xa_zero_floats_ * sizeof(float)));
    RC(posgrid_launch(gridT_, S, 0));
    RC(fill_launch(recon_, (long long)Bmax * N * 4, 0.f, 0));
    const float* saw[SA_NW];
    for (int i = 0; i < SA_NW; ++i) saw[i] = P(w_.sa.w[i]);
    PackEntry ent[SA_PACK_ENTRIES];
    sa_pack_n_ = sa_pack_table(saw, C, D, H, ent, &sa_pack_max_);
    OCRL_HIP(hipMemcpy(sa_pack_dev_, ent, sa_pack_n_ * sizeof(PackEntry), hipMemcpyHostToDevice));
    OCRL_HIP(hipDeviceSynchronize());
    have_fwd_ = false;
    return 0;
}

int SlateModel::soft_z(hipStream_t st) {
    if (!fused_heads() || cfg.use_bcdec) return 0;
    OCRL_REQUIRE(have_scores_, "soft_z: no forward since the last backward (the scores have been overwritten by their gradient)");
    return exp_rows_launch(zraw_, zlse_, z_, (long long)last_.B * T, V, st);
}
int SlateModel::dropout_mask(unsigned site, long long n, float* out, hipStream_t st) const {
    return dropout_mask_launch(out, n, pdrop_, last_.seed, site, st);
}

int SlateModel::conv_layer_fwd(const float* x, const float* pack, const float* bias, float* y, int Bn, int Hh, int Ww, int KS, int CIN,
                               int relu, const float* posmap, const float* mask, const Lane& L) {
    ConvArgs a;
    a.X = x; a.Wp = pack; a.Y = y; a.B = Bn; a.H = Hh; a.W = Ww; a.bias = bias; a.relu = relu; a.posmap = posmap; a.mask = mask;
    if (conv_x3_ > 0 && (KS == 5 || KS == 3) && CIN == 64 && !conv_lowlat_) {
        auto it = x3_of_.find(pack);
        if (it != x3_of_.end()) return conv_x3_launch(a, it->second, L, KS);
    }
    return conv_fwd_launch(a, KS, CIN, 64, L, conv_lowlat_);
}
int SlateModel::conv_layer_wgrad(const float* x, const float* dy, float* dW, float* db, int Bn, int Hh, int Ww, int KS, int CIN,
                                 int cin_real, const Lane& L) {
    WgradArgs a;
    a.X = x; a.dY = dy; a.part = L.scratch; a.B = Bn; a.H = Hh; a.W = Ww;
    OCRL_REQUIRE(conv_wgrad_ws_floats(Bn, Hh, Ww, KS, CIN) <= L.scratch_floats, "conv wgrad: scratch too small");
    const bool x3 = conv_x3_ > 0 && CIN == 64;
    RC(conv_wgrad_launch(a, KS, CIN, 64, cin_real, dW, x3 ? nullptr : db, 0, L, x3 ? 1 : 0));
    if (db && x3) RC(colsum_launch(dy, 64, db, (long long)Bn * Hh * Ww, 64, 0, 1.f, L.scratch, L.scratch_floats, L));
    return 0;
}

int SlateModel::pack_weights(const Lane& L, bool encoder_only) {
    if (first_direct()) RC(conv_first_pack_launch(P(w_.enc[0].w), cw_fwd_[0], L));
    else RC(conv_pack_launch(P(w_.enc[0].w), cw_fwd_[0], nullptr, 5, 8, 64, cfg.obs_channels, L));
    RC(conv_pack_launch(P(w_.enc[1].w), cw_fwd_[1], cw_bwd_[1], 5, 64, 64, 64, L));
    RC(conv_pack_launch(P(w_.enc[2].w), cw_fwd_[2], cw_bwd_[2], 5, 64, 64, 64, L));
    RC(conv_pack_launch(P(w_.enc[3].w), cw_fwd_[3], cw_bwd_[3], 5, 64, 64, 64, L));
    if (conv_x3_ > 0) {
        for (int i = 1; i < 4; ++i) {
            auto f = x3_of_.find(cw_fwd_[i]), b = x3_of_.find(cw_bwd_[i]);
            if (f != x3_of_.end()) RC(conv_pack_x3_launch(P(w_.enc[i].w), const_cast<float*>(f->second), b != x3_of_.end() ? const_cast<float*>(b->second) : nullptr, L));
        }
    }
    if (!cfg.use_bcdec && !encoder_only) {
        RC(conv_pack_launch(P(w_.dvae_dec[1].w), dw_fwd_[0], dw_bwd_[0], 3, 64, 64, 64, L));
        RC(conv_pack_launch(P(w_.dvae_dec[6].w), dw_fwd_[1], dw_bwd_[1], 3, 64, 64, 64, L));
        if (conv_x3_ > 0) {
            for (int i = 0; i < 2; ++i) {
                auto f = x3_of_.find(dw_fwd_[i]), b = x3_of_.find(dw_bwd_[i]);
                if (f != x3_of_.end()) RC(conv_pack_x3_launch(P(w_.dvae_dec[i ? 6 : 1].w), const_cast<float*>(f->second), b != x3_of_.end() ? const_cast<float*>(b->second) : nullptr, L, 3));
            }
        }
        RC(copy_launch(P(w_.dvae_dec[11].w), w11p_, cfg.obs_channels * 64, L));
        RC(fill_launch(w11p_ + cfg.obs_channels * 64, (4 - cfg.obs_channels) * 64, 0.f, L));
    }
    RC(pack_launch(sa_pack_dev_, sa_pack_n_, sa_pack_max_, sa_wts_, L));
    RC(posmap_launch(P(w_.enc_pos.w), P(w_.enc_pos.b), posmap_, S, C, L));
    return 0;
}

int SlateModel::fwd_encoder(const StepInputs& in, const Lane& L, FwdDvae fork) {
    const int B = in.B;
    const long long BN = (long long)B * N;
    auto fork_if = [&](FwdDvae here) -> int {
        if (fork != here) return 0;
        RC(after(dvae_lane(), L, ev_fork_));
        return fwd_dvae(in, dvae_lane());
    };
    RC(slot_init_launch(P(w_.sa.mu), P(w_.sa.log_sigma), in.noise_slots, slots0_, B * K, D, in.seed, L, in.seed_dev));
    SlotAttnArgs a = sa_args(B, N, K, D, H, I, SH);
    a.x = x_; a.slots0 = slots0_; a.wts = sa_wts_; a.slots = slots_; a.attn = attn_; a.attn_heads = attn_heads_; a.save = sa_save_;
    if (conv_lowlat_ && frozen_) a.save = nullptr;
    a.xchg = sa_xchg_; a.parts = sa_parts_;
    a.phase = 1;
    RC(slot_attn_launch(a, 0, L));
    RC(fork_if(FwdDvae::AtStart));
    if (first_direct()) {
        RC(conv_first_fwd_launch(in.obs, cw_fwd_[0], P(w_.enc[0].b), e1_, B, S, S, 1, L));
        if (!(conv_lowlat_ && frozen_))
            OCRL_HIP(hipMemcpyAsync(obs_keep_, in.obs, (size_t)BN * cfg.obs_channels * sizeof(float), hipMemcpyDeviceToDevice, L));
    } else {
        RC(nchw_to_nhwc8_launch(in.obs, obs8_, B, cfg.obs_channels, S, S, L));
        RC(conv_layer_fwd(obs8_, cw_fwd_[0], P(w_.enc[0].b), e1_, B, S, S, 5, 8, 1, nullptr, nullptr, L));
    }
    RC(conv_layer_fwd(e1_, cw_fwd_[1], P(w_.enc[1].b), e2_, B, S, S, 5, 64, 1, nullptr, nullptr, L));
    RC(conv_layer_fwd(e2_, cw_fwd_[2], P(w_.enc[2].b), e3_, B, S, S, 5, 64, 1, nullptr, nullptr, L));
    RC(conv_layer_fwd(e3_, cw_fwd_[3], P(w_.enc[3].b), e4_, B, S, S, 5, 64, 0, posmap_, nullptr, L));
    RC(fork_if(FwdDvae::AfterConvs));
    if (sa_input_ && C == 64 && !(conv_lowlat_ && frozen_)) {
        RC(sa_input_fwd_launch(e4_, P(w_.sa.ln.w), P(w_.sa.ln.b), P(w_.sa.mlp0.w),
                               P(w_.sa.mlp0.b), P(w_.sa.mlp2.w), P(w_.sa.mlp2.b), ln0_mean_, ln0_rstd_,
                               sa_input_ == 2 ? ln0_ : nullptr, h1_, x_, BN, 0, L));
    } else {
        RC(layernorm_fwd_launch(e4_, P(w_.sa.ln.w), P(w_.sa.ln.b), ln0_, ln0_mean_, ln0_rstd_, BN, C, L));
        RC(lin_fwd(ln0_, C, P(w_.sa.mlp0.w), P(w_.sa.mlp0.b), h1_, C, BN, C, C, 1, nullptr, 0, 0.f, 0, L));
        RC(lin_fwd(h1_, C, P(w_.sa.mlp2.w), P(w_.sa.mlp2.b), x_, C, BN, C, C, 0, nullptr, 0, 0.f, 0, L));
    }
    RC(fork_if(FwdDvae::AtSlotAttention));
    a.phase = 2;
    RC(slot_attn_launch(a, 0, L));
    return 0;
}

int SlateModel::fwd_dvae(const StepInputs& in, const Lane& L) {
    const int B = in.B;
    const long long BT = (long long)B * T, BN = (long long)B * N;
    const int ch = cfg.obs_channels;
    RC(patchify4_launch(in.obs, patches_, B, ch, S, L));
    RC(lin_fwd(patches_, 16 * ch, P(w_.dvae_enc[0].w), P(w_.dvae_enc[0].b), de_[0], 64, BT, 64, 16 * ch, 1, nullptr, 0, 0.f, 0, L));
    for (int i = 1; i < 7; ++i)
        RC(lin_fwd(de_[i - 1], 64, P(w_.dvae_enc[i].w), P(w_.dvae_enc[i].b), de_[i], 64, BT, 64, 64, 1, nullptr, 0, 0.f, 0, L));
    if (fused_heads()) {
        GemmArgs a;
        a.A = de_[6]; a.B = P(w_.dvae_enc[7].w); a.C = zraw_; a.M = (int)BT; a.N = V; a.K = 64; a.lda = 64; a.ldb = 64; a.ldc = V;
        a.bias = P(w_.dvae_enc[7].b);
        a.epi_mode = 2; a.stat = zstat_; a.hstat = zhstat_; a.hidx = zhidx_; a.e1 = in.noise_z; a.e2 = in.noise_zh; a.e_seed = in.seed;
        a.e_scale = 1.0f / in.tau;
        RC(gemm_launch(a, L));
        RC(softmax_stat_combine_launch(zstat_, gemm_stat_segments(V), BT, zlse_, zhstat_, zhidx_, tokens_, nullptr, 0, nullptr, nullptr, 0.f, nullptr, 0, L,
                                       in.noise_z ? nullptr : zraw_, V, in.tau, in.seed));
        have_scores_ = true;
    } else {
    RC(lin_fwd(de_[6], 64, P(w_.dvae_enc[7].w), P(w_.dvae_enc[7].b), zraw_, V, BT, V, 64, 0, nullptr, 0, 0.f, 0, L));
    RC(gumbel_softmax_launch(zraw_, in.noise_z, in.noise_zh, z_, tokens_, BT, V, in.tau, in.seed, L, cfg.hard ? zdec_ : nullptr));
    }
    if (side_ && L.st == side_ && ev_tokens_) OCRL_HIP(hipEventRecord(ev_tokens_, L.st));
    RC(dvae_decode(B, drecon_, L));
    return 0;
}

int SlateModel::dvae_decode(int B, float* drecon, const Lane& L, const float* zin) {
    const long long BT = (long long)B * T, BN = (long long)B * N;
    const int ch = cfg.obs_channels;
    if (!zin && fused_heads()) {
        GemmArgs a;
        a.A = zraw_; a.B = P(w_.dvae_dec[0].w); a.C = dd0_; a.M = (int)BT; a.N = 64; a.K = V; a.lda = V; a.ldb = V; a.ldc = 64;
        a.bias = P(w_.dvae_dec[0].b); a.relu = 1; a.a_mode = 2; a.x_lse = zlse_;
        RC(gemm_launch(a, L));
    } else {
    if (!zin) zin = zdec_;
    RC(lin_fwd(zin, V, P(w_.dvae_dec[0].w), P(w_.dvae_dec[0].b), dd0_, 64, BT, 64, V, 1, nullptr, 0, 0.f, 0, L));
    }
    RC(conv_layer_fwd(dd0_, dw_fwd_[0], P(w_.dvae_dec[1].b), dd1_, B, E, E, 3, 64, 1, nullptr, nullptr, L));
    RC(lin_fwd(dd1_, 64, P(w_.dvae_dec[2].w), P(w_.dvae_dec[2].b), dd2_, 64, BT, 64, 64, 1, nullptr, 0, 0.f, 0, L));
    RC(lin_fwd(dd2_, 64, P(w_.dvae_dec[3].w), P(w_.dvae_dec[3].b), dd3_, 64, BT, 64, 64, 1, nullptr, 0, 0.f, 0, L));
    RC(lin_fwd(dd3_, 64, P(w_.dvae_dec[4].w), P(w_.dvae_dec[4].b), dd4_, 256, BT, 256, 64, 1, nullptr, 0, 0.f, 0, L));
    RC(pixel_shuffle_launch(dd4_, ps1_, B, E, E, 64, 1, nullptr, L));
    RC(conv_layer_fwd(ps1_, dw_fwd_[1], P(w_.dvae_dec[6].b), dd6_, B, 2 * E, 2 * E, 3, 64, 1, nullptr, nullptr, L));
    RC(lin_fwd(dd6_, 64, P(w_.dvae_dec[7].w), P(w_.dvae_dec[7].b), dd7_, 64, 4 * BT, 64, 64, 1, nullptr, 0, 0.f, 0, L));
    RC(lin_fwd(dd7_, 64, P(w_.dvae_dec[8].w), P(w_.dvae_dec[8].b), dd8_, 64, 4 * BT, 64, 64, 1, nullptr, 0, 0.f, 0, L));
    RC(lin_fwd(dd8_, 64, P(w_.dvae_dec[9].w), P(w_.dvae_dec[9].b), dd9_, 256, 4 * BT, 256, 64, 1, nullptr, 0, 0.f, 0, L));
    RC(pixel_shuffle_launch(dd9_, ps2_, B, 2 * E, 2 * E, 64, 1, nullptr, L));
    RC(lin_fwd(ps2_, 64, P(w_.dvae_dec[11].w), P(w_.dvae_dec[11].b), recon_, 4, BN, ch, 64, 0, nullptr, 0, 0.f, 0, L));
    RC(mse_launch(last_.obs, recon_, drecon, metrics_ + (drecon ? 0 : 4), B, ch, S, S, L.scratch, L.scratch_floats, L));
    return 0;
}

AttnArgs SlateModel::self_attn_args(int b) const {
    const Blk& k = blk_[b];
    AttnArgs a;
    a.q = k.q; a.k = k.k; a.v = k.v; a.o = k.ao; a.lse = k.lse; a.B = last_.B; a.T = T; a.d = d; a.h = NH; a.ld = 3 * d;
    a.p = pdrop_; a.seed = last_.seed; a.site = SITE_BLK_BASE + 8 * b + 0;
    return a;
}
XaHost SlateModel::xattn_args(int b) const {
    const Blk& k = blk_[b];
    const unsigned site = SITE_BLK_BASE + 8 * b;
    XaHost hx;
    hx.x = k.ln2; hx.P = k.cP; hx.Ab = k.xaAb; hx.AbT = k.xaAbT; hx.Vo = k.xaVo; hx.VoT = k.xaVoT;
    hx.B = last_.B; hx.T = T; hx.K = K; hx.d = d; hx.h = NH; hx.p = pdrop_; hx.seed = last_.seed; hx.site_p = site + 2; hx.site_o = site + 3;
    return hx;
}

int SlateModel::fwd_decoder(const Lane& L, bool with_ce) {
    const int B = last_.B;
    const long long BT = (long long)B * T;
    const float p = pdrop_;
    RC(lin_fwd(slots_, D, P(w_.slotproj), nullptr, mem_, d, (long long)B * K, d, D, 0, nullptr, 0, 0.f, 0, L));
    RC(embed_fwd_launch(tokens_, P(w_.dict), P(w_.bos), P(w_.pe), emb_, B, T, d, p, last_.seed, L));
    const Lane F = plan_.dw == 2 ? dw_lane(L) : L;
    if (xattn_) {
        XaFoldHost f;
        f.mem = mem_; f.B = B; f.K = K; f.d = d; f.h = NH; f.nblk = NB;
        OCRL_REQUIRE(NB <= 8, "more than 8 decoder blocks: set OCRL_XATTN=0");
        for (int b = 0; b < NB; ++b) {
            const DecBlockW& bw = w_.blk[b];
            f.Wq[b] = P(bw.cq); f.Wk[b] = P(bw.ck); f.Wv[b] = P(bw.cv); f.Wo[b] = P(bw.co);
            f.ck[b] = blk_[b].ck; f.cv[b] = blk_[b].cv; f.Ab[b] = blk_[b].xaAb; f.AbT[b] = blk_[b].xaAbT; f.Vo[b] = blk_[b].xaVo; f.VoT[b] = blk_[b].xaVoT;
        }
        RC(after(F, L, ring_event()));
        RC(xattn_fold_fwd_launch(f, F));
    }
    const float* xin = emb_;
    for (int b = 0; b < NB; ++b) {
        Blk& k = blk_[b];
        const DecBlockW& bw = w_.blk[b];
        const unsigned site = SITE_BLK_BASE + 8 * b;
        RC(layernorm_fwd_launch(xin, P(bw.ln1.w), P(bw.ln1.b), k.ln1, k.ln1_mean, k.ln1_rstd, BT, d, L));
        const float* res = (b == 0) ? k.ln1 : xin;
        RC(lin_fwd(k.ln1, d, P(bw.qkv), nullptr, k.q, 3 * d, BT, 3 * d, d, 0, nullptr, 0, 0.f, 0, L));
        {
            const AttnArgs a = self_attn_args(b);
            RC(attn_launch(a, 0, L));
        }
        RC(lin_fwd(k.ao, d, P(bw.o), nullptr, k.x1, d, BT, d, d, 0, res, d, p, site + 1, L));
        RC(layernorm_fwd_launch(k.x1, P(bw.ln2.w), P(bw.ln2.b), k.ln2, k.ln2_mean, k.ln2_rstd, BT, d, L));
        if (xattn_) {
            if (b == 0) RC(after(L, F, ev_join2_));
            XaHost hx = xattn_args(b);
            hx.resid = k.x1; hx.y = k.x2;
            RC(xattn_launch(hx, 0, L));
        } else {
        RC(lin_fwd(k.ln2, d, P(bw.cq), nullptr, k.cq, d, BT, d, d, 0, nullptr, 0, 0.f, 0, L));
        RC(lin_fwd(mem_, d, P(bw.ck), nullptr, k.ck, d, (long long)B * K, d, d, 0, nullptr, 0, 0.f, 0, L));
        RC(lin_fwd(mem_, d, P(bw.cv), nullptr, k.cv, d, (long long)B * K, d, d, 0, nullptr, 0, 0.f, 0, L));
        RC(cross_attn_fwd_launch(k.cq, k.ck, k.cv, k.cao, k.cP, B, T, K, d, NH, p, last_.seed, site + 2, L));
        RC(lin_fwd(k.cao, d, P(bw.co), nullptr, k.x2, d, BT, d, d, 0, k.x1, d, p, site + 3, L));
        }
        RC(layernorm_fwd_launch(k.x2, P(bw.ln3.w), P(bw.ln3.b), k.ln3, k.ln3_mean, k.ln3_rstd, BT, d, L));
        RC(lin_fwd(k.ln3, d, P(bw.ffn0.w), P(bw.ffn0.b), k.f1, 4 * d, BT, 4 * d, d, 1, nullptr, 0, 0.f, 0, L));
        RC(lin_fwd(k.f1, 4 * d, P(bw.ffn2.w), P(bw.ffn2.b), k.x3, d, BT, d, 4 * d, 0, k.x2, d, p, site + 4, L));
        xin = k.x3;
    }
    RC(layernorm_fwd_launch(xin, P(w_.lnf.w), P(w_.lnf.b), lnf_, lnf_mean_, lnf_rstd_, BT, d, L));
    if (with_ce) {
        GemmArgs a;
        a.A = lnf_; a.B = P(w_.out); a.C = pred_; a.M = (int)BT; a.N = V; a.K = d; a.lda = d; a.ldb = d; a.ldc = V;
        a.epi_mode = 1; a.stat = cestat_;
        RC(gemm_launch(a, L));
        RC(softmax_stat_combine_launch(cestat_, gemm_stat_segments(V), BT, celse_, nullptr, nullptr, nullptr, pred_, V, tokens_, metrics_ + 1, 1.0f / B,
                                       cepart_, (size_t)(BT / 16 + 16), L));
    } else RC(lin_fwd(lnf_, d, P(w_.out), nullptr, pred_, V, BT, V, d, 0, nullptr, 0, 0.f, 0, L));
    return 0;
}

int SlateModel::forward(const StepInputs& in, hipStream_t st) {
    OCRL_REQUIRE(p_ && ws_, "forward: model not bound");
    OCRL_REQUIRE(in.B >= 1 && in.B <= Bmax, "forward: batch %d outside [1,%d]", in.B, Bmax);
    OCRL_REQUIRE(in.obs && in.tau > 0.f, "forward: bad inputs");
    last_ = in;
    have_enc_ = false;
    pdrop_ = in.train ? cfg.dropout : 0.f;
    const Lane L = main_lane(st);
    RC(pack_weights(L));
    if (cfg.use_bcdec) {
        RC(fwd_encoder(in, L));
        RC(pack_bcdec(L));
        RC(fwd_bcdec(L));
        RC(fill_launch(metrics_ + 1, 1, 0.f, L));
        RC(copy_launch(metrics_ + 0, metrics_ + 2, 1, L));
        have_fwd_ = true;
        return 0;
    }
    if (plan_.fwd_dvae == FwdDvae::Serial) RC(fwd_dvae(in, L));
    if (plan_.fwd_dvae == FwdDvae::BesideEncoder) {
        RC(after(dvae_lane(), L, ev_fork_));
        RC(fwd_dvae(in, dvae_lane()));
    }
    RC(fwd_encoder(in, L, plan_.fwd_dvae));
    if (plan_.tokens_early) OCRL_HIP(hipStreamWaitEvent(L, ev_tokens_, 0));
    else if (plan_.side) RC(after(L, dvae_lane(), ev_join_));
    RC(fwd_decoder(L));
    if (plan_.tokens_early) RC(after(L, dvae_lane(), ev_join_));
    RC(copy_launch(metrics_ + 0, metrics_ + 2, 1, L));
    RC(axpy_launch(metrics_ + 1, metrics_ + 2, 1, 1.f, L));
    have_fwd_ = true;
    return 0;
}

int SlateModel::encode(const StepInputs& in, hipStream_t st) {
    OCRL_REQUIRE(p_ && ws_, "encode: model not bound");
    OCRL_REQUIRE(in.B >= 1 && in.B <= Bmax && in.obs, "encode: bad inputs");
    last_ = in;
    pdrop_ = 0.f;
    have_fwd_ = false;
    have_enc_ = true;
    const Lane L = main_lane(st);
    if (enc_graph_mode_ < 0) enc_graph_mode_ = (int)sw::model<sw::OCRL_ENCODE_GRAPH>();
    const bool graph = enc_graph_mode_ && in.B <= 32 && !in.noise_slots && obs_stage_;
    const bool need_pack = !(frozen_ && packs_valid_);
    struct LowLat { int& f; LowLat(int& x) : f(x) { f = 1; } ~LowLat() { f = 0; } } lowlat(conv_lowlat_);
    if (!graph) {
        if (need_pack) RC(pack_weights(L, true));
        packs_valid_ = frozen_;
        return fwd_encoder(in, L);
    }
    EncGraph& eg = enc_graphs_[in.B];
    if (!eg.warm || need_pack) {
        eg.warm = 1;
        if (need_pack) RC(pack_weights(L, true));
        packs_valid_ = frozen_;
        return fwd_encoder(in, L);
    }
    const size_t bytes = (size_t)in.B * cfg.obs_channels * N * sizeof(float);
    OCRL_HIP(hipMemcpyAsync(obs_stage_, in.obs, bytes, hipMemcpyDeviceToDevice, L));
    RC(store_u64_launch(seed_dev_, in.seed, L));
    if (!eg.exec) {
        StepInputs gi = in;
        gi.obs = obs_stage_; gi.seed_dev = seed_dev_;
        hipGraph_t g = nullptr;
        if (!cap_) OCRL_HIP(hipStreamCreateWithFlags(&cap_, hipStreamNonBlocking));
        OCRL_HIP(hipStreamBeginCapture(cap_, hipStreamCaptureModeThreadLocal));
        const Lane cap = main_lane(cap_);
        int rc = frozen_ ? 0 : pack_weights(cap, true);
        if (!rc) rc = fwd_encoder(gi, cap);
        const hipError_t ce = hipStreamEndCapture(cap_, &g);
        if (rc) { if (g) (void)hipGraphDestroy(g); return rc; }
        OCRL_HIP(ce);
        OCRL_HIP(hipGraphInstantiate(&eg.exec, g, nullptr, nullptr, 0));
        OCRL_HIP(hipGraphDestroy(g));
    }
    OCRL_HIP(hipGraphLaunch(eg.exec, L));
    return 0;
}

void SlateModel::clear_encode_graphs() {
    for (auto& kv : enc_graphs_) if (kv.second.exec) (void)hipGraphExecDestroy(kv.second.exec);
    enc_graphs_.clear();
}

int SlateModel::encode_backward(const float* dslots, hipStream_t st) {
    OCRL_REQUIRE(have_enc_, "encode_backward: call encode first (its activations are what is differentiated)");
    OCRL_REQUIRE(!frozen_, "encode_backward: the weights are frozen (ocrl_slate_freeze_weights): encode() kept no activations");
    OCRL_REQUIRE(g_ && dslots, "encode_backward: no gradient buffer bound / null dslots");
    const Lane L = main_lane(st);
    RC(fill_launch(g_, flat_size_, 0.f, L));
    RC(copy_launch(dslots, gslots_, (long long)last_.B * K * D, L));
    RC(bwd_encoder(L));
    have_enc_ = false;
    enc_only_grads_ = true;
    return 0;
}

int SlateModel::generate(hipStream_t st) {
    OCRL_REQUIRE(!cfg.use_bcdec, "generate: the autoregressive decoder is not part of the use_bcdec configuration");
    OCRL_REQUIRE(last_.B > 0 && last_.obs, "generate: run forward or encode first");
    have_enc_ = false;
    const int B = last_.B;
    const long long BK = (long long)B * K;
    pdrop_ = 0.f;
    have_fwd_ = false;
    const Lane L = main_lane(st);
    OCRL_HIP(hipMemsetAsync(tokens_, 0, sizeof(int) * (size_t)B * T, L));
    RC(lin_fwd(slots_, D, P(w_.slotproj), nullptr, mem_, d, BK, d, D, 0, nullptr, 0, 0.f, 0, L));
    for (int b = 0; b < NB; ++b) {
        const DecBlockW& bw = w_.blk[b];
        RC(lin_fwd(mem_, d, P(bw.ck), nullptr, blk_[b].ck, d, BK, d, d, 0, nullptr, 0, 0.f, 0, L));
        RC(lin_fwd(mem_, d, P(bw.cv), nullptr, blk_[b].cv, d, BK, d, d, 0, nullptr, 0, 0.f, 0, L));
    }
    float* x0 = emb_;
    for (int t = 0; t < T; ++t) {
        RC(embed_step_launch(tokens_, P(w_.dict), P(w_.bos), P(w_.pe), x0, B, T, d, t, L));
        const float* xin = x0;
        for (int b = 0; b < NB; ++b) {
            Blk& k = blk_[b];
            const DecBlockW& bw = w_.blk[b];
            RC(layernorm_fwd_launch(xin, P(bw.ln1.w), P(bw.ln1.b), k.ln1, k.ln1_mean, k.ln1_rstd, B, d, L));
            const float* res = (b == 0) ? k.ln1 : xin;
            RC(lin_fwd(k.ln1, d, P(bw.qkv), nullptr, k.q + (size_t)t * 3 * d, T * 3 * d, B, 3 * d, d, 0, nullptr, 0, 0.f, 0, L));
            RC(decode_attn_launch(k.q, k.ao, B, T, t, d, NH, 3 * d, L));
            RC(lin_fwd(k.ao, d, P(bw.o), nullptr, k.x1, d, B, d, d, 0, res, d, 0.f, 0, L));
            RC(layernorm_fwd_launch(k.x1, P(bw.ln2.w), P(bw.ln2.b), k.ln2, k.ln2_mean, k.ln2_rstd, B, d, L));
            RC(lin_fwd(k.ln2, d, P(bw.cq), nullptr, k.cq, d, B, d, d, 0, nullptr, 0, 0.f, 0, L));
            RC(cross_attn_fwd_launch(k.cq, k.ck, k.cv, k.cao, k.cP, B, 1, K, d, NH, 0.f, 0, 0, L));
            RC(lin_fwd(k.cao, d, P(bw.co), nullptr, k.x2, d, B, d, d, 0, k.x1, d, 0.f, 0, L));
            RC(layernorm_fwd_launch(k.x2, P(bw.ln3.w), P(bw.ln3.b), k.ln3, k.ln3_mean, k.ln3_rstd, B, d, L));
            RC(lin_fwd(k.ln3, d, P(bw.ffn0.w), P(bw.ffn0.b), k.f1, 4 * d, B, 4 * d, d, 1, nullptr, 0, 0.f, 0, L));
            RC(lin_fwd(k.f1, 4 * d, P(bw.ffn2.w), P(bw.ffn2.b), k.x3, d, B, d, 4 * d, 0, k.x2, d, 0.f, 0, L));
            xin = k.x3;
        }
        RC(layernorm_fwd_launch(xin, P(w_.lnf.w), P(w_.lnf.b), lnf_, lnf_mean_, lnf_rstd_, B, d, L));
        RC(lin_fwd(lnf_, d, P(w_.out), nullptr, pred_, V, B, V, d, 0, nullptr, 0, 0.f, 0, L));
        RC(argmax_pos_launch(pred_, tokens_, B, T, V, t, L, 1));
    }
    RC(onehot_launch(tokens_, z_, (long long)B * T, V, L));
    RC(dvae_decode(B, nullptr, L, z_));
    return 0;
}

int SlateModel::bwd_decoder(const Lane& L) {
    const int B = last_.B;
    const long long BT = (long long)B * T, BK = (long long)B * K;
    const float p = pdrop_;
    const Lane W = dw_lane(L);
    const bool dws = plan_.dw != 0;
    Xf ce; ce.a_mode = 3; ce.lse = celse_; ce.tok = tokens_; ce.scale = 1.0f / last_.B;
    RC(after(W, L, ring_event()));
    RC(lin_bwd_w(pred_, V, lnf_, d, G(w_.out), nullptr, BT, V, d, 1.f, W, ce));
    RC(lin_bwd_x(pred_, V, P(w_.out), gt1_, d, BT, V, d, nullptr, 0, nullptr, 0, L, Drop(), ce));
    const float* xlast = blk_[NB - 1].x3;
    RC(layernorm_bwd_launch(gt1_, xlast, lnf_mean_, lnf_rstd_, P(w_.lnf.w), gx_, G(w_.lnf.w), BT, d, 0, 0,
                            L.scratch, L.scratch_floats, L));
    RC(fill_launch(gmem_, BK * d, 0.f, L));
    for (int b = NB - 1; b >= 0; --b) {
        Blk& k = blk_[b];
        const BlkG& q = bg_[dws ? b : 0];
        const DecBlockW& bw = w_.blk[b];
        const unsigned site = SITE_BLK_BASE + 8 * b;
        const float* xin = (b == 0) ? emb_ : blk_[b - 1].x3;
        const float* gd = gx_;
        auto drop_gx = [&](unsigned s_, float* into) -> int {
            gd = gx_;
            if (p > 0.f || dws) { RC(dropout_apply_launch(gx_, into, BT * d, p, last_.seed, s_, L)); gd = into; }
            return 0;
        };
        RC(drop_gx(site + 4, q.gbr[0]));
        RC(lin_bwd_x(gd, d, P(bw.ffn2.w), q.gf1, 4 * d, BT, d, 4 * d, k.f1, 4 * d, nullptr, 0, L));
        RC(after(W, L, ring_event()));
        RC(lin_bwd_w(gd, d, k.f1, 4 * d, G(bw.ffn2.w), G(bw.ffn2.b), BT, d, 4 * d, 1.f, W));
        RC(lin_bwd_w(q.gf1, 4 * d, k.ln3, d, G(bw.ffn0.w), G(bw.ffn0.b), BT, 4 * d, d, 1.f, W));
        RC(lin_bwd_x(q.gf1, 4 * d, P(bw.ffn0.w), gt1_, d, BT, 4 * d, d, nullptr, 0, nullptr, 0, L));
        RC(layernorm_bwd_launch(gt1_, k.x2, k.ln3_mean, k.ln3_rstd, P(bw.ln3.w), gx_, G(bw.ln3.w), BT, d, 1, 0,
                                L.scratch, L.scratch_floats, L));
        RC(drop_gx(site + 3, q.gbr[1]));
        const float* gd_co = gd;
        if (xattn_) {
            XaHost hx = xattn_args(b);
            hx.y = gt1_; hx.gd = gd_co; hx.Pd = q.xaPd; hx.dS = q.xaDs;
            RC(xattn_launch(hx, 1, L));
            RC(after(W, L, ring_event()));
            XaFoldBwdHost f;
            f.Pd = q.xaPd; f.dS = q.xaDs; f.gd = gd_co; f.x = k.ln2; f.Wq = P(bw.cq); f.Wo = P(bw.co); f.ck = k.ck; f.cv = k.cv;
            f.dVo = xa_dVo_; f.dAb = xa_dAb_; f.dck = gck_; f.dcv = gcv_; f.pq = xa_pq_; f.po = xa_po_; f.dWq = G(bw.cq); f.dWo = G(bw.co);
            f.ws = W.scratch; f.ws_floats = W.scratch_floats; f.B = B; f.T = T; f.K = K; f.d = d; f.h = NH;
            RC(xattn_fold_bwd_launch(f, W));
        } else {
        RC(lin_bwd_x(gd, d, P(bw.co), gt1_, d, BT, d, d, nullptr, 0, nullptr, 0, L));
        RC(cross_attn_bwd_launch(gt1_, k.cq, k.ck, k.cv, k.cP, q.gt2, gck_, gcv_, B, T, K, d, NH, p, last_.seed, site + 2, L.scratch, L.scratch_floats, L));
        RC(after(W, L, ring_event()));
        RC(lin_bwd_w(gd_co, d, k.cao, d, G(bw.co), nullptr, BT, d, d, 1.f, W));
        RC(lin_bwd_w(q.gt2, d, k.ln2, d, G(bw.cq), nullptr, BT, d, d, 1.f, W));
        RC(lin_bwd_x(q.gt2, d, P(bw.cq), gt1_, d, BT, d, d, nullptr, 0, nullptr, 0, L));
        }
        {
            const Lane& X = xattn_ ? W : L;
            RC(lin_bwd_w(gck_, d, mem_, d, G(bw.ck), nullptr, BK, d, d, 1.f, X));
            RC(lin_bwd_w(gcv_, d, mem_, d, G(bw.cv), nullptr, BK, d, d, 1.f, X));
            RC(lin_bwd_x(gck_, d, P(bw.ck), gmem_, d, BK, d, d, nullptr, 0, gmem_, d, X));
            RC(lin_bwd_x(gcv_, d, P(bw.cv), gmem_, d, BK, d, d, nullptr, 0, gmem_, d, X));
        }
        RC(layernorm_bwd_launch(gt1_, k.x1, k.ln2_mean, k.ln2_rstd, P(bw.ln2.w), gx_,
                                G(bw.ln2.w), BT, d, 1, 0, L.scratch, L.scratch_floats, L));
        RC(drop_gx(site + 1, q.gbr[2]));
        const float* gd_o = gd;
        RC(lin_bwd_x(gd, d, P(bw.o), gt1_, d, BT, d, d, nullptr, 0, nullptr, 0, L));
        {
            AttnArgs a = self_attn_args(b);
            a.dO = gt1_; a.dq = q.gqkv; a.dk = q.gqkv + d; a.dv = q.gqkv + 2 * d; a.delta = attn_delta_;
            a.ds = attn_ds_; a.ds_floats = attn_ds_floats_;
            RC(attn_launch(a, 1, L));
        }
        RC(after(W, L, ring_event()));
        RC(lin_bwd_w(gd_o, d, k.ao, d, G(bw.o), nullptr, BT, d, d, 1.f, W));
        RC(lin_bwd_w(q.gqkv, 3 * d, k.ln1, d, G(bw.qkv), nullptr, BT, 3 * d, d, 1.f, W));
        RC(lin_bwd_x(q.gqkv, 3 * d, P(bw.qkv), gt1_, d, BT, 3 * d, d, nullptr, 0, nullptr, 0, L));
        if (b == 0) {
            RC(axpy_launch(gx_, gt1_, BT * d, 1.f, L));
            RC(layernorm_bwd_launch(gt1_, xin, k.ln1_mean, k.ln1_rstd, P(bw.ln1.w), gx_,
                                    G(bw.ln1.w), BT, d, 0, 0, L.scratch, L.scratch_floats, L));
        } else {
            RC(layernorm_bwd_launch(gt1_, xin, k.ln1_mean, k.ln1_rstd, P(bw.ln1.w), gx_,
                                    G(bw.ln1.w), BT, d, 1, 0, L.scratch, L.scratch_floats, L));
        }
    }
    RC(embed_bwd_launch(gx_, tokens_, G(w_.dict), B, T, V, d, p, last_.seed, L.scratch, L.scratch_floats, L));
    RC(fill_launch(G(w_.pe), (long long)(T + 1) * d, 0.f, L));
    RC(colsum_launch(gx_, (long long)T * d, G(w_.pe), B, T * d, 0, 1.f, L.scratch, L.scratch_floats, L));
    RC(copy_launch(G(w_.pe), G(w_.bos), d, L));
    if (xattn_) RC(after(L, W, ring_event()));
    RC(lin_bwd_w(gmem_, d, slots_, D, G(w_.slotproj), nullptr, BK, d, D, 1.f, L));
    RC(lin_bwd_x(gmem_, d, P(w_.slotproj), gslots_, D, BK, d, D, nullptr, 0, nullptr, 0, L));
    return 0;
}

int SlateModel::bwd_encoder(const Lane& L, BwdDvae fork) {
    const bool fork_dvae = fork == BwdDvae::AtSlotAttention;
    const int B = last_.B;
    const long long BN = (long long)B * N, R = (long long)B * I * K;
    const SlotAttnW& sa = w_.sa;
    SlotAttnArgs a = sa_args(B, N, K, D, H, I, SH);
    a.x = x_; a.wts = sa_wts_; a.save = sa_save_; a.dslots = gslots_; a.dx = gA_; a.dslots0 = gslots0_; a.grows = sa_grows_; a.g_small = sa_small_;
    a.xchg = sa_xchg_; a.parts = sa_parts_;
    if (fork_dvae) {
        RC(after(dvae_lane(), L, ev_fork_));
        RC(bwd_dvae(dvae_lane()));
    }
    RC(slot_attn_launch(a, 1, L));
    const bool side_w = plan_.sa_wgrads_on_side;
    const Lane W = side_w ? dvae_lane() : L;
    if (side_w) RC(after(W, L, ev_fork_));
    const bool sa_in_bwd = sa_input_ == 1 && C == 64;
    SaWgrad wg[SA_MAX_WGRADS];
    const int nwg = sa_wgrad_list(C, D, H, SH, a.scale, wg);
    for (int i = 0; i < nwg; ++i) {
        const SaWgrad& e = wg[i];
        RC(lin_bwd_w(e.dy.at(sa_save_, sa_grows_), e.dy.ld, e.x.at(sa_save_, sa_grows_), e.x.ld, G(sa.w[e.w]) + e.w_off,
                     e.b < 0 ? nullptr : G(sa.w[e.b]), R, e.N_out, e.K_in, e.alpha, W));
    }
    const int SM = 4 * D + 2 * C;
    RC(colsum_launch(sa_small_ + 0, SM, G(sa.w[SAW_NORM_SLOTS_W]), B, 2 * D, 0, 1.f, W.scratch, W.scratch_floats, W));
    RC(colsum_launch(sa_small_ + 2 * D, SM, G(sa.w[SAW_NORM_MLP_W]), B, 2 * D, 0, 1.f, W.scratch, W.scratch_floats, W));
    RC(colsum_launch(sa_small_ + 4 * D, SM, G(sa.w[SAW_NORM_INPUTS_W]), B, 2 * C, 0, 1.f, W.scratch, W.scratch_floats, W));
    RC(slot_init_bwd_launch(gslots0_, P(w_.sa.log_sigma), last_.noise_slots, G(w_.sa.mu), G(w_.sa.log_sigma),
                            B * K, D, last_.seed, W));
    if (!sa_in_bwd) RC(lin_bwd_w(gA_, C, h1_, C, G(w_.sa.mlp2.w), G(w_.sa.mlp2.b), BN, C, C, 1.f, W));
    if (side_w && !first_direct()) RC(im2col5_launch(obs8_, col0_, BN, S, S, cfg.obs_channels, (25 * cfg.obs_channels + 3) & ~3, W));
    if (sa_in_bwd) {
        const size_t slabs = L.scratch_floats / SA_INPUT_SLAB;
        OCRL_REQUIRE(slabs >= 1, "bwd_encoder: scratch too small for the input-chain slabs");
        RC(sa_input_bwd_launch(gA_, h1_, e4_, ln0_mean_, ln0_rstd_, P(w_.sa.ln.w), P(w_.sa.ln.b),
                               P(w_.sa.mlp0.w), P(w_.sa.mlp2.w), gB_, G(w_.sa.mlp0.w), G(w_.sa.mlp0.b),
                               G(w_.sa.mlp2.w), G(w_.sa.mlp2.b), G(w_.sa.ln.w), G(w_.sa.ln.b),
                               BN, slabs < 512 ? (int)slabs : 0, L.scratch, L.scratch_floats, L));
    } else {
        RC(lin_bwd_x(gA_, C, P(w_.sa.mlp2.w), gB_, C, BN, C, C, h1_, C, nullptr, 0, L));
        RC(lin_bwd_w(gB_, C, ln0_, C, G(w_.sa.mlp0.w), G(w_.sa.mlp0.b), BN, C, C, 1.f, L));
        float* gL = side_w ? gC_ : gA_;
        RC(lin_bwd_x(gB_, C, P(w_.sa.mlp0.w), gL, C, BN, C, C, nullptr, 0, nullptr, 0, L));
        RC(layernorm_bwd_launch(gL, e4_, ln0_mean_, ln0_rstd_, P(w_.sa.ln.w), gB_, G(w_.sa.ln.w), BN, C, 0, 0,
                                L.scratch, L.scratch_floats, L));
    }
    RC(colsum_launch(gB_, (long long)N * C, gmap_, B, N * C, 0, 1.f, L.scratch, L.scratch_floats, L));
    RC(lin_bwd_w(gmap_, C, gridT_, 4, G(w_.enc_pos.w), G(w_.enc_pos.b), N, C, 4, 1.f, L));
    if (fork_dvae || side_w) RC(after(L, dvae_lane(), ev_join_));
    if (plan_.dw == 2) RC(after(L, dw_lane(L), ev_join2_));
    RC(colsum_launch(gmap_, C, G(w_.enc[3].b), N, C, 0, 1.f, L.scratch, L.scratch_floats, L));
    RC(conv_layer_wgrad(e3_, gB_, G(w_.enc[3].w), nullptr, B, S, S, 5, 64, 64, L));
    RC(conv_layer_fwd(gB_, cw_bwd_[3], nullptr, gA_, B, S, S, 5, 64, 0, nullptr, e3_, L));
    RC(conv_layer_wgrad(e2_, gA_, G(w_.enc[2].w), G(w_.enc[2].b), B, S, S, 5, 64, 64, L));
    RC(conv_layer_fwd(gA_, cw_bwd_[2], nullptr, gB_, B, S, S, 5, 64, 0, nullptr, e2_, L));
    RC(conv_layer_wgrad(e1_, gB_, G(w_.enc[1].w), G(w_.enc[1].b), B, S, S, 5, 64, 64, L));
    RC(conv_layer_fwd(gB_, cw_bwd_[1], nullptr, gA_, B, S, S, 5, 64, 0, nullptr, e1_, L));
    if (first_direct()) {
        OCRL_REQUIRE(conv_first_wgrad_ws_floats(B, S, S) <= L.scratch_floats, "first conv wgrad: scratch too small");
        RC(conv_first_wgrad_launch(obs_keep_, gA_, L.scratch, G(w_.enc[0].w), G(w_.enc[0].b), B, S, S, 0, L));
    } else {
        const int ch = cfg.obs_channels, ldc0 = (25 * ch + 3) & ~3;
        if (!side_w) RC(im2col5_launch(obs8_, col0_, BN, S, S, ch, ldc0, L));
        RC(lin_bwd_w(gA_, 64, col0_, ldc0, dw0p_, G(w_.enc[0].b), BN, 64, ldc0, 1.f, L));
        RC(unpack5_launch(dw0p_, G(w_.enc[0].w), ch, ldc0, L));
    }
    return 0;
}

int SlateModel::bwd_dvae(const Lane& L) {
    const int B = last_.B;
    const long long BT = (long long)B * T, BN = (long long)B * N;
    const int ch = cfg.obs_channels;
    float* w4 = L.scratch + L.scratch_floats - 1024;
    {
        GemmArgs a;
        a.A = drecon_; a.B = ps2_; a.C = w4; a.M = 4; a.N = 64; a.K = (int)BN; a.lda = 4; a.ldb = 64; a.ldc = 64; a.akc = 0; a.bkc = 0;
        long long splits = BN / 512; if (splits > 512) splits = 512; if (splits < 1) splits = 1;
        if (splits > 1) {
            a.splitk = (int)splits; a.C = L.scratch; a.sCsplit = 256;
            RC(gemm_launch(a, L));
            RC(splitk_reduce_launch(L.scratch, w4, 256, (int)splits, 256, 0, L));
        } else RC(gemm_launch(a, L));
        RC(copy_launch(w4, G(w_.dvae_dec[11].w), ch * 64, L));
        RC(colsum_launch(drecon_, 4, w4 + 256, BN, 4, 0, 1.f, L.scratch, L.scratch_floats - 1024, L));
        RC(copy_launch(w4 + 256, G(w_.dvae_dec[11].b), ch, L));
    }
    RC(lin_bwd_x(drecon_, 4, w11p_, gdA_, 64, BN, 4, 64, nullptr, 0, nullptr, 0, L));
    RC(pixel_shuffle_launch(gdA_, gdB_, B, 2 * E, 2 * E, 64, 0, dd9_, L));
    RC(lin_bwd_w(gdB_, 256, dd8_, 64, G(w_.dvae_dec[9].w), G(w_.dvae_dec[9].b), 4 * BT, 256, 64, 1.f, L));
    RC(lin_bwd_x(gdB_, 256, P(w_.dvae_dec[9].w), gdA_, 64, 4 * BT, 256, 64, dd8_, 64, nullptr, 0, L));
    RC(lin_bwd_w(gdA_, 64, dd7_, 64, G(w_.dvae_dec[8].w), G(w_.dvae_dec[8].b), 4 * BT, 64, 64, 1.f, L));
    RC(lin_bwd_x(gdA_, 64, P(w_.dvae_dec[8].w), gdB_, 64, 4 * BT, 64, 64, dd7_, 64, nullptr, 0, L));
    RC(lin_bwd_w(gdB_, 64, dd6_, 64, G(w_.dvae_dec[7].w), G(w_.dvae_dec[7].b), 4 * BT, 64, 64, 1.f, L));
    RC(lin_bwd_x(gdB_, 64, P(w_.dvae_dec[7].w), gdA_, 64, 4 * BT, 64, 64, dd6_, 64, nullptr, 0, L));
    RC(conv_layer_wgrad(ps1_, gdA_, G(w_.dvae_dec[6].w), G(w_.dvae_dec[6].b), B, 2 * E, 2 * E, 3, 64, 64, L));
    RC(conv_layer_fwd(gdA_, dw_bwd_[1], nullptr, gdB_, B, 2 * E, 2 * E, 3, 64, 0, nullptr, ps1_, L));
    RC(pixel_shuffle_launch(gdB_, gdA_, B, E, E, 64, 0, nullptr, L));
    RC(lin_bwd_w(gdA_, 256, dd3_, 64, G(w_.dvae_dec[4].w), G(w_.dvae_dec[4].b), BT, 256, 64, 1.f, L));
    RC(lin_bwd_x(gdA_, 256, P(w_.dvae_dec[4].w), gdB_, 64, BT, 256, 64, dd3_, 64, nullptr, 0, L));
    RC(lin_bwd_w(gdB_, 64, dd2_, 64, G(w_.dvae_dec[3].w), G(w_.dvae_dec[3].b), BT, 64, 64, 1.f, L));
    RC(lin_bwd_x(gdB_, 64, P(w_.dvae_dec[3].w), gdA_, 64, BT, 64, 64, dd2_, 64, nullptr, 0, L));
    RC(lin_bwd_w(gdA_, 64, dd1_, 64, G(w_.dvae_dec[2].w), G(w_.dvae_dec[2].b), BT, 64, 64, 1.f, L));
    RC(lin_bwd_x(gdA_, 64, P(w_.dvae_dec[2].w), gdB_, 64, BT, 64, 64, dd1_, 64, nullptr, 0, L));
    RC(conv_layer_wgrad(dd0_, gdB_, G(w_.dvae_dec[1].w), G(w_.dvae_dec[1].b), B, E, E, 3, 64, 64, L));
    RC(conv_layer_fwd(gdB_, dw_bwd_[0], nullptr, gdA_, B, E, E, 3, 64, 0, nullptr, dd0_, L));
    float* dz = zraw_;
    have_scores_ = false;
    if (fused_heads()) {
        Xf zx; zx.b_mode = 2; zx.lse = zlse_;
        RC(lin_bwd_w(gdA_, 64, zraw_, V, G(w_.dvae_dec[0].w), G(w_.dvae_dec[0].b), BT, 64, V, 1.f, L, zx));
        RC(rowdot_bias64_launch(gdA_, dd0_, P(w_.dvae_dec[0].b), BT, zdot_, L));
        GemmArgs a;
        a.A = gdA_; a.B = P(w_.dvae_dec[0].w); a.C = dz; a.M = (int)BT; a.N = V; a.K = 64; a.lda = 64; a.ldb = V; a.ldc = V; a.bkc = 0;
        a.epi_mode = 3; a.mask = zraw_; a.ldmask = V; a.e_lse = zlse_; a.e_rowvec = zdot_; a.e_scale = 1.0f / last_.tau;
        RC(gemm_launch(a, L));
    } else {
    RC(lin_bwd_w(gdA_, 64, zdec_, V, G(w_.dvae_dec[0].w), G(w_.dvae_dec[0].b), BT, 64, V, 1.f, L));
    RC(lin_bwd_x(gdA_, 64, P(w_.dvae_dec[0].w), dz, V, BT, 64, V, nullptr, 0, nullptr, 0, L));
    RC(softmax_bwd_rows_launch(z_, dz, BT, V, 1.0f / last_.tau, L));
    }
    RC(lin_bwd_w(dz, V, de_[6], 64, G(w_.dvae_enc[7].w), G(w_.dvae_enc[7].b), BT, V, 64, 1.f, L));
    RC(lin_bwd_x(dz, V, P(w_.dvae_enc[7].w), gdA_, 64, BT, V, 64, de_[6], 64, nullptr, 0, L));
    float* cur = gdA_;
    float* oth = gdB_;
    for (int i = 6; i >= 1; --i) {
        RC(lin_bwd_w(cur, 64, de_[i - 1], 64, G(w_.dvae_enc[i].w), G(w_.dvae_enc[i].b), BT, 64, 64, 1.f, L));
        RC(lin_bwd_x(cur, 64, P(w_.dvae_enc[i].w), oth, 64, BT, 64, 64, de_[i - 1], 64, nullptr, 0, L));
        float* t = cur; cur = oth; oth = t;
    }
    RC(lin_bwd_w(cur, 64, patches_, 16 * ch, G(w_.dvae_enc[0].w), G(w_.dvae_enc[0].b), BT, 64, 16 * ch, 1.f, L));
    return 0;
}

int SlateModel::backward(hipStream_t st) {
    OCRL_REQUIRE(have_fwd_, "backward: call forward first");
    OCRL_REQUIRE(g_, "backward: no gradient buffer bound");
    enc_only_grads_ = false;
    const Lane L = main_lane(st);
    if (cfg.use_bcdec) {
        RC(fill_launch(g_, flat_size_, 0.f, L));
        RC(bwd_bcdec(L));
        RC(bwd_encoder(L));
        have_fwd_ = false;
        return 0;
    }
    const BwdDvae at = plan_.bwd_dvae;
    if (at == BwdDvae::BesideAll || at == BwdDvae::BesideDecoder) {
        RC(after(dvae_lane(), L, ev_fork_));
        RC(bwd_dvae(dvae_lane()));
    }
    RC(bwd_decoder(L));
    if (at == BwdDvae::BesideDecoder && !plan_.dw) RC(after(L, dvae_lane(), ev_join_));
    RC(bwd_encoder(L, at));
    if (at == BwdDvae::BesideAll) RC(after(L, dvae_lane(), ev_join_));
    if (at == BwdDvae::SerialLast) RC(bwd_dvae(L));
    have_fwd_ = false;
    return 0;
}

int SlateModel::after(const Lane& waiter, const Lane& producer, hipEvent_t ev) {
    if (waiter.st == producer.st) return 0;
    OCRL_HIP(hipEventRecord(ev, producer.st));
    OCRL_HIP(hipStreamWaitEvent(waiter.st, ev, 0));
    return 0;
}

int SlateModel::grad_norm(hipStream_t st) {
    const Lane L = main_lane(st);
    return absmax_launch(g_, flat_size_, metrics_ + 3, L.scratch, L.scratch_floats, L);
}

int SlateModel::clip_adam(const float lr[3], float clip, int step, float gscale, hipStream_t st) {
    OCRL_REQUIRE(m_ && v_, "clip_adam: optimiser state not bound");
    packs_valid_ = false;
    RC(grad_norm(st));
    if (enc_only_grads_) {
        const long long b0 = group_begin_[1], end = w_.enc_grads_end;
        return clip_adam_launch(p_ + b0, g_ + b0, m_ + b0, v_ + b0, end - b0, metrics_ + 3, clip, lr[1], 0.9, 0.999, 1e-8, step, gscale, st);
    }
    for (int g = 0; g < 3; ++g) {
        if (cfg.use_bcdec && g != 1) continue;
        const long long b0 = group_begin_[g], n = group_begin_[g + 1] - b0;
        RC(clip_adam_launch(p_ + b0, g_ + b0, m_ + b0, v_ + b0, n, metrics_ + 3, clip, lr[g], 0.9, 0.999, 1e-8, step, gscale, st));
    }
    return 0;
}

int SlateModel::pack_bcdec(const Lane& L) {
    RC(bc_compose_launch(P(w_.bc[0].w), P(w_.bc_pos.w), P(w_.bc_pos.b), bc_Wc_,
                         bc_W1r_, D, L));
    RC(conv_pack_launch(P(w_.bc[1].w), bc_pk_[0], bc_pkb_[0], 5, 64, 64, 64, L));
    RC(conv_pack_launch(P(w_.bc[2].w), bc_pk_[1], bc_pkb_[1], 5, 64, 64, 64, L));
    if (conv_x3_ > 0) {
        for (int i = 0; i < 2; ++i) {
            auto f = x3_of_.find(bc_pk_[i]), b = x3_of_.find(bc_pkb_[i]);
            if (f != x3_of_.end()) RC(conv_pack_x3_launch(P(w_.bc[i + 1].w), const_cast<float*>(f->second), b != x3_of_.end() ? const_cast<float*>(b->second) : nullptr, L));
        }
    }
    RC(bc_c4_pack_launch(P(w_.bc[3].w), bc_Wk4_, bc_Wb4_, cfg.obs_channels + 1, L));
    return 0;
}

int SlateModel::fwd_bcdec(const Lane& L) {
    const int B = last_.B, BK = B * K;
    RC(bc_posconv_launch(bc_Wc_, bc_P1_, S, L));
    RC(lin_fwd(slots_, D, bc_W1r_, nullptr, bc_M_, 1600, BK, 1600, D, 0, nullptr, 0, 0.f, 0, L));
    RC(bcast_l1_class_sum_launch(bc_M_, bc_T_, BK, 5, 1, L));
    RC(bcast_l1_fwd_launch(bc_P1_, bc_T_, P(w_.bc[0].b), bc_c1_, BK, S, 5, BCAST_L1_RELU, L));
    RC(conv_layer_fwd(bc_c1_, bc_pk_[0], P(w_.bc[1].b), bc_c2_, BK, S, S, 5, 64, 1, nullptr, nullptr, L));
    RC(conv_layer_fwd(bc_c2_, bc_pk_[1], P(w_.bc[2].b), bc_c3_, BK, S, S, 5, 64, 1, nullptr, nullptr, L));
    RC(bc_c4_fwd_launch(bc_c3_, bc_Wk4_, P(w_.bc[3].b), bc_out4_, BK, S, L));
    RC(bc_mix_launch(bc_out4_, last_.obs, recon_, bc_dout4_, metrics_ + 0, B, K, S, cfg.obs_channels, L.scratch, L.scratch_floats, L));
    return 0;
}

int SlateModel::bwd_bcdec(const Lane& L) {
    const int B = last_.B, BK = B * K;
    const long long BKN = (long long)BK * N;
    const int nb = bc_c4_wgrad_blocks(BK, S);
    RC(bc_c4_wgrad_launch(bc_c3_, bc_dout4_, L.scratch, BK, S, L));
    RC(colsum_launch(L.scratch, 4 * 64 * 9, G(w_.bc[3].w), nb, 4 * 64 * 9, 0, 1.f, L.scratch + (size_t)nb * 2304, L.scratch_floats - (size_t)nb * 2304, L));
    RC(colsum_launch(bc_dout4_, 4, G(w_.bc[3].b), BKN, cfg.obs_channels + 1, 0, 1.f, L.scratch, L.scratch_floats, L));
    RC(bc_c4_bwd_data_launch(bc_dout4_, bc_Wb4_, bc_c3_, bc_gA_, BK, S, L));
    RC(conv_layer_wgrad(bc_c2_, bc_gA_, G(w_.bc[2].w), G(w_.bc[2].b), BK, S, S, 5, 64, 64, L));
    RC(conv_layer_fwd(bc_gA_, bc_pkb_[1], nullptr, bc_gB_, BK, S, S, 5, 64, 0, nullptr, bc_c2_, L));
    RC(conv_layer_wgrad(bc_c1_, bc_gB_, G(w_.bc[1].w), G(w_.bc[1].b), BK, S, S, 5, 64, 64, L));
    RC(conv_layer_fwd(bc_gB_, bc_pkb_[0], nullptr, bc_gA_, BK, S, S, 5, 64, 0, nullptr, bc_c1_, L));
    RC(bcast_l1_bwd_launch(bc_gA_, bc_dT_, BK, S, 5, L.scratch, L.scratch_floats, L));
    RC(colsum_launch(bc_dT_, 64, G(w_.bc[0].b), (long long)BK * 25, 64, 0, 1.f, L.scratch, L.scratch_floats, L));
    RC(bcast_l1_class_sum_launch(bc_dT_, bc_dM_, BK, 5, 0, L));
    RC(lin_bwd_x(bc_dM_, 1600, bc_W1r_, gslots_, D, BK, 1600, D, nullptr, 0, nullptr, 0, L));
    RC(lin_bwd_w(bc_dM_, 1600, slots_, D, bc_dW1r_, nullptr, BK, 1600, D, 1.f, L));
    RC(colsum_launch(bc_gA_, (long long)N * 64, bc_G1_, BK, N * 64, 0, 1.f, L.scratch, L.scratch_floats, L));
    RC(bc_posconv_bwd_launch(bc_G1_, bc_dWc_, S, L));
    RC(bc_compose_bwd_launch(P(w_.bc[0].w), P(w_.bc_pos.w), P(w_.bc_pos.b), bc_dWc_,
                             bc_dW1r_, G(w_.bc[0].w), G(w_.bc_pos.w), G(w_.bc_pos.b), D, L));
    return 0;
}
```

ocrl_amd/csrc/slate_model.h:

```cpp
#pragma once
#include <map>
#include <string>
#include <vector>

#include "kernels.h"
#include "model_base.h"
#include "slot_attn_host.h"
#include "stream_plan.h"

struct SlateConfig {
    int obs_size = 64, obs_channels = 3, vocab = 4096, d_model = 192, cnn_hidden = 64;
    int num_slots = 5, num_iters = 3, slot_size = 192, mlp_hidden = 192;
    int num_blocks = 4, num_heads = 4;
    float dropout = 0.1f;
    int max_batch = 1;
    int use_bcdec = 0;
    int hard = 0;
    int slot_heads = 1;
};

struct StepInputs {
    const float* obs = nullptr;
    int B = 0;
    float tau = 1.f;
    int train = 1;
    unsigned long long seed = 0;
    const float* noise_z = nullptr;
    const float* noise_zh = nullptr;
    const float* noise_slots = nullptr;
    const unsigned long long* seed_dev = nullptr;
};

struct Lane {
    hipStream_t st = nullptr;
    float* scratch = nullptr;
    size_t scratch_floats = 0;
    operator hipStream_t() const { return st; }
};

class SlateModel : public ModelBase {
public:
    explicit SlateModel(const SlateConfig& c);
    ~SlateModel();
    long long group_begin(int g) const { return group_begin_[g]; }
    int bind(float* p, float* g, float* m, float* v, void* ws, size_t ws_bytes);
    int forward(const StepInputs& in, hipStream_t st);
    int backward(hipStream_t st);
    int encode(const StepInputs& in, hipStream_t st);
    void freeze_weights(bool on) { frozen_ = on; packs_valid_ = false; clear_encode_graphs(); }
    void clear_encode_graphs();
    int encode_backward(const float* dslots, hipStream_t st);
    int generate(hipStream_t st);
    int clip_adam(const float lr[3], float clip, int step, float gscale, hipStream_t st);
    int grad_norm(hipStream_t st);
    int dropout_mask(unsigned site, long long n, float* out, hipStream_t st) const;
    int soft_z(hipStream_t st);
    const SlateConfig cfg;

private:
    void layout_workspace(bool commit);
    int lin_fwd(const float* x, int ldx, const float* W, const float* b, float* y, int ldy, long long M, int N, int K, int relu,
                const float* resid, int ldr, float drop_p, unsigned site, hipStream_t st) {
        return ::lin_fwd(x, ldx, W, b, y, ldy, M, N, K, relu, resid, ldr, st, Drop{drop_p, last_.seed, site});
    }
    int lin_bwd_w(const float* dy, int ld_dy, const float* x, int ldx, float* dW, float* db, long long M, int N_out, int K_in,
                  float alpha, const Lane& L, Xf xf = Xf()) {
        return ::lin_bwd_w(dy, ld_dy, x, ldx, dW, db, M, N_out, K_in, alpha, L.scratch, L.scratch_floats, L.st, Drop(), xf);
    }
    bool fused_heads() const { return !cfg.hard; }
    int conv_layer_fwd(const float* x, const float* pack, const float* bias, float* y, int Bn, int Hh, int Ww, int KS, int CIN, int relu,
                       const float* posmap, const float* mask, const Lane& L);
    int conv_layer_wgrad(const float* x, const float* dy, float* dW, float* db, int Bn, int Hh, int Ww, int KS, int CIN, int cin_real,
                         const Lane& L);
    int pack_weights(const Lane& L, bool encoder_only = false);
    int fwd_encoder(const StepInputs& in, const Lane& L, FwdDvae fork = FwdDvae::Serial);
    int fwd_dvae(const StepInputs& in, const Lane& L);
    int fwd_decoder(const Lane& L, bool with_ce = true);
    int dvae_decode(int B, float* drecon, const Lane& L, const float* zin = nullptr);
    int bwd_decoder(const Lane& L);
    int bwd_encoder(const Lane& L, BwdDvae fork = BwdDvae::SerialLast);
    int bwd_dvae(const Lane& L);
    int pack_bcdec(const Lane& L);
    int fwd_bcdec(const Lane& L);
    int bwd_bcdec(const Lane& L);
    AttnArgs self_attn_args(int b) const;
    XaHost xattn_args(int b) const;

    Lane main_lane(hipStream_t st) const { return Lane{st, scratch_, scratch_floats_}; }
    Lane dvae_lane() const { return Lane{side_, scratch2_, scratch_floats_}; }
    Lane dw_lane(const Lane& main) const { return plan_.dw == 2 ? Lane{side2_, scratch3_, scratch_floats_} : plan_.dw ? dvae_lane() : main; }
    int after(const Lane& waiter, const Lane& producer, hipEvent_t ev);
    hipEvent_t ring_event() { return ev_dw_[ev_dw_next_++ & 7]; }

    struct DecBlockW { ParamPair ln1, ln2, ln3, ffn0, ffn2; ParamRef qkv, o, cq, ck, cv, co; };
    struct SlotAttnW {
        ParamRef mu, log_sigma;
        ParamPair ln, mlp0, mlp2;
        ParamRef w[SA_NW];
    };
    struct Weights {
        ParamPair dvae_enc[8], dvae_dec[12];
        ParamPair enc[4], enc_pos;
        SlotAttnW sa;
        ParamPair bc[4], bc_pos;
        ParamRef slotproj, dict, bos, pe, out;
        ParamPair lnf;
        std::vector<DecBlockW> blk;
        long long enc_grads_end = 0;
    } w_;
    void resolve_params();

    long long group_begin_[4] = {0, 0, 0, 0};

    int S, E, T, N, V, d, C, K, I, D, H, NB, NH, DH, Bmax;
    int SH = 1;
    StepInputs last_;
    float pdrop_ = 0.f;
    bool have_fwd_ = false;
    int conv_lowlat_ = 0;
    bool frozen_ = false, packs_valid_ = false;
    bool have_enc_ = false;
    bool enc_only_grads_ = false;
    bool have_scores_ = false;

    float *scratch_ = nullptr;
    size_t scratch_floats_ = 0;
    float* scratch2_ = nullptr;
    StreamPlan plan_;
    hipStream_t side_ = nullptr;
    hipEvent_t ev_fork_ = nullptr, ev_join_ = nullptr, ev_tokens_ = nullptr;
    float *zstat_ = nullptr, *zhstat_ = nullptr, *zlse_ = nullptr, *zdot_ = nullptr, *cestat_ = nullptr, *celse_ = nullptr, *cepart_ = nullptr;
    int* zhidx_ = nullptr;
    float *obs8_, *patches_, *de_[7], *zraw_, *z_, *zdec_;
    int* tokens_;
    float *dd0_, *dd1_, *dd2_, *dd3_, *dd4_, *ps1_, *dd6_, *dd7_, *dd8_, *dd9_, *ps2_, *recon_, *drecon_;
    float *e1_, *e2_, *e3_, *e4_, *posmap_, *gridT_, *ln0_, *ln0_mean_, *ln0_rstd_, *h1_, *x_;
    float *slots0_, *slot_noise_, *slots_, *attn_, *sa_save_, *sa_wts_, *sa_grows_, *sa_small_, *sa_xchg_;
    float* attn_heads_ = nullptr;
    float* sa_parts_;
    PackEntry* sa_pack_dev_ = nullptr;
    int sa_pack_n_ = 0, sa_pack_max_ = 0;
    float *cw_fwd_[4], *cw_bwd_[4];
    int conv_x3_ = 0;
    std::map<const float*, const float*> x3_of_;
    float *dw_fwd_[2], *dw_bwd_[2];
    float *w11p_;
    float *mem_, *emb_;
    struct Blk {
        float *ln1, *ln1_mean, *ln1_rstd, *q, *k, *v, *lse, *ao, *x1;
        float *ln2, *ln2_mean, *ln2_rstd, *cq, *ck, *cv, *cP, *cao, *x2;
        float *ln3, *ln3_mean, *ln3_rstd, *f1, *x3;
        float *xaAb, *xaAbT, *xaVo, *xaVoT;
    };
    int sa_input_ = 1;
    bool xattn_ = false;
    float *xa_dAb_ = nullptr, *xa_dVo_ = nullptr, *xa_pq_ = nullptr, *xa_po_ = nullptr;
    size_t xa_zero_floats_ = 0;
    float* xa_zero_base_ = nullptr;
    std::vector<Blk> blk_;
    struct BlkG { float *gbr[3], *gf1, *gt2, *gqkv, *xaPd, *xaDs; };
    std::vector<BlkG> bg_;
    struct EncGraph { hipGraphExec_t exec = nullptr; int warm = 0; };
    std::map<int, EncGraph> enc_graphs_;
    int enc_graph_mode_ = -1;
    hipStream_t cap_ = nullptr;
    float* obs_stage_ = nullptr;
    unsigned long long* seed_dev_ = nullptr;
    hipStream_t side2_ = nullptr;
    float* scratch3_ = nullptr;
    hipEvent_t ev_dw_[8] = {nullptr, nullptr, nullptr, nullptr, nullptr, nullptr, nullptr, nullptr};
    hipEvent_t ev_join2_ = nullptr;
    int ev_dw_next_ = 0;
    float *attn_delta_;
    float *attn_ds_ = nullptr;
    size_t attn_ds_floats_ = 0;
    float *lnf_, *lnf_mean_, *lnf_rstd_, *pred_;
    float *gqkv_;
    float *gx_, *gbr_, *gt1_, *gt2_, *gt3_, *gf1_, *gmem_, *gck_, *gcv_, *gslots_, *gslots0_;
    float *gA_, *gB_, *gC_;
    float *gdA_, *gdB_;
    float *gmap_;
    float *col0_, *dw0p_;
    float* obs_keep_ = nullptr;
    bool first_direct() const { return cfg.obs_channels == 3; }
    float *bc_Wc_, *bc_W1r_, *bc_P1_, *bc_M_, *bc_T_, *bc_c1_, *bc_c2_, *bc_c3_, *bc_out4_, *bc_dout4_, *bc_gA_, *bc_gB_;
    float *bc_pk_[2], *bc_pkb_[2], *bc_Wk4_, *bc_Wb4_, *bc_dW1r_, *bc_dWc_, *bc_dT_, *bc_dM_, *bc_G1_;
};
```

Measured before the change: 1813.

## Fuse chains of 64x64 dVAE linear layers into single persistent MFMA kernels

Adds forward and backward kernels that run 2 or 3 consecutive 64-wide ReLU linear layers of the dVAE encoder and decoder in one persistent launch, keeping the intermediate tile in LDS and the weights in registers or LDS. The backward kernel computes input gradients and accumulates weight and bias gradients per workgroup into slabs, which a separate reduce kernel sums. This replaces many separate lin_fwd, lin_bwd_w and lin_bwd_x launches and the round trips of intermediates through global memory. In exchange it adds a slab reduction, depends on scratch size, and the backward ReLU mask now comes from the stored outputs.

```diff
diff --git a/include/ocrl_hip_dvae_chain.h b/include/ocrl_hip_dvae_chain.h
--- /dev/null
+++ b/include/ocrl_hip_dvae_chain.h
@@ -0,0 +1,21 @@
+#ifndef OCRL_HIP_DVAE_CHAIN_H
+#define OCRL_HIP_DVAE_CHAIN_H
+#include <stddef.h>
+
+#ifdef __cplusplus
+extern "C" {
+#endif
+
+#define OCRL_DVAE_CHAIN_MIN_L 2
+#define OCRL_DVAE_CHAIN_MAX_L 3
+
+int ocrl_dvae_chain_plan(long long R, int L, int out[3]);
+int ocrl_dvae_chain_fwd(int L, const float* y0, const float* const* W, const float* const* b, float* const* y, long long R, int max_wgs,
+                        void* stream);
+int ocrl_dvae_chain_bwd(int L, const float* dY, const float* const* y, const float* const* W, float* dY0, float* const* dW,
+                        float* const* db, long long R, int max_wgs, float* ws, size_t ws_floats, void* stream);
+
+#ifdef __cplusplus
+}
+#endif
+#endif
diff --git a/ocrl_amd/_lib.py b/ocrl_amd/_lib.py
--- a/ocrl_amd/_lib.py
+++ b/ocrl_amd/_lib.py
@@ -9,6 +9,7 @@
 HEADER_PATH = os.path.join(_HERE, os.pardir, "include", "ocrl_hip.h")
 DQN_HEADER_PATH = os.path.join(_HERE, os.pardir, "include", "ocrl_hip_dqn.h")
 ROLLOUT_HEADER_PATH = os.path.join(_HERE, os.pardir, "include", "ocrl_hip_rollout.h")
+DVAE_CHAIN_HEADER_PATH = os.path.join(_HERE, os.pardir, "include", "ocrl_hip_dvae_chain.h")
 _lib = None
 
 if not os.path.exists(HEADER_PATH):
@@ -30,6 +31,10 @@
     raise RuntimeError(f"{ROLLOUT_HEADER_PATH} is missing: ocrl_amd derives its binding of libocrl_hip.so from the header and runs from the source tree.")
 with open(ROLLOUT_HEADER_PATH) as _f:
     ABI_ROLLOUT = _abi.read(_f.read())
+if not os.path.exists(DVAE_CHAIN_HEADER_PATH):
+    raise RuntimeError(f"{DVAE_CHAIN_HEADER_PATH} is missing: ocrl_amd derives its binding of libocrl_hip.so from the header and runs from the source tree.")
+with open(DVAE_CHAIN_HEADER_PATH) as _f:
+    ABI_DVAE_CHAIN = _abi.read(_f.read())
 
 
 def flat_segments(segs):
@@ -88,7 +93,7 @@
             "(make -C ocrl_amd/csrc).  ocrl_amd has no CPU fallback.")
     import torch
     L = ctypes.CDLL(LIB_PATH)
-    for abi in (ABI, ABI_DQN, ABI_ROLLOUT):
+    for abi in (ABI, ABI_DQN, ABI_ROLLOUT, ABI_DVAE_CHAIN):
         for name, (restype, argtypes) in abi.functions.items():
             f = getattr(L, name)
             f.argtypes = argtypes
diff --git a/ocrl_amd/csrc/dvae_chain.hip b/ocrl_amd/csrc/dvae_chain.hip
--- /dev/null
+++ b/ocrl_amd/csrc/dvae_chain.hip
@@ -0,0 +1,283 @@
+#include "common.h"
+#include "kernels.h"
+#include "row_tile64.h"
+
+#define DVC_BWD_MAX_WGS 512
+
+struct DvcFwd { const float* W[DVAE_CHAIN_MAX_L]; const float* b[DVAE_CHAIN_MAX_L]; float* y[DVAE_CHAIN_MAX_L]; };
+struct DvcBwd { const float* W[DVAE_CHAIN_MAX_L]; const float* y[DVAE_CHAIN_MAX_L]; };
+struct DvcGrads { float* dW[DVAE_CHAIN_MAX_L]; float* db[DVAE_CHAIN_MAX_L]; };
+
+template <int L>
+__global__ __launch_bounds__(256, L == 2 ? 3 : 2) void dvae_chain_fwd_kernel(const float* __restrict__ y0, const DvcFwd p, long long R) {
+    __shared__ __attribute__((aligned(16))) float T[2][RT_ROWS * RT_LD];
+    const int lane = threadIdx.x & 63, wv = threadIdx.x >> 6, c4 = lane & 15, rsub = lane >> 4;
+    const int li = lane & 31, lh = lane >> 5;
+    const int wm0 = (wv >> 1) * 32, wn0 = (wv & 1) * 32;
+    float wf[L][8][4], bv[L];
+#pragma unroll
+    for (int l = 0; l < L; ++l) {
+#pragma unroll
+        for (int c = 0; c < 8; ++c) {
+            const float4 a = *reinterpret_cast<const float4*>(p.W[l] + (wn0 + li) * 64 + c * 8 + 4 * lh);
+            wf[l][c][0] = a.x; wf[l][c][1] = a.y; wf[l][c][2] = a.z; wf[l][c][3] = a.w;
+        }
+        bv[l] = p.b[l][wn0 + li];
+    }
+    const long long ntiles = (R + RT_ROWS - 1) / RT_ROWS;
+    const int lr0 = wv * 16 + rsub;
+    float4 v[4];
+#pragma unroll
+    for (int i = 0; i < 4; ++i) v[i] = rt_ld4(y0, (long long)blockIdx.x * RT_ROWS + lr0 + 4 * i, R, c4);
+    for (long long tile = blockIdx.x; tile < ntiles; tile += gridDim.x) {
+        const long long r0 = tile * RT_ROWS;
+#pragma unroll
+        for (int i = 0; i < 4; ++i) *reinterpret_cast<float4*>(T[0] + (lr0 + 4 * i) * RT_LD + c4 * 4) = v[i];
+#pragma unroll
+        for (int i = 0; i < 4; ++i) v[i] = rt_ld4(y0, (tile + gridDim.x) * RT_ROWS + lr0 + 4 * i, R, c4);
+        __syncthreads();
+#pragma unroll
+        for (int l = 0; l < L; ++l) {
+            const float* const in = T[l & 1];
+            float* const out = T[(l + 1) & 1];
+            f32x16 acc;
+#pragma unroll
+            for (int r = 0; r < 16; ++r) acc[r] = 0.f;
+            rt_mma_kc(in + wm0 * RT_LD, wf[l], acc);
+#pragma unroll
+            for (int r = 0; r < 16; ++r) {
+                const int row = (r & 3) + 8 * (r >> 2) + 4 * lh;
+                out[(wm0 + row) * RT_LD + wn0 + li] = fmaxf(acc[r] + bv[l], 0.f);
+            }
+            __syncthreads();
+#pragma unroll
+            for (int i = 0; i < 4; ++i) {
+                const int lr = lr0 + 4 * i;
+                const long long row = r0 + lr;
+                if (row < R) *reinterpret_cast<float4*>(p.y[l] + row * 64 + c4 * 4) = *reinterpret_cast<const float4*>(out + lr * RT_LD + c4 * 4);
+            }
+        }
+        __syncthreads();
+    }
+}
+
+template <int L>
+__global__ __launch_bounds__(256, 2) void dvae_chain_bwd_kernel(const float* __restrict__ dY, const DvcBwd p, float* __restrict__ dY0,
+                                                                float* __restrict__ slab, long long R) {
+    constexpr int KR = L == 3 ? 2 : 0;
+    __shared__ __attribute__((aligned(16))) float T[2][RT_ROWS * RT_LD], Ws[L * 4096 - KR * 512];
+    const int lane = threadIdx.x & 63, wv = threadIdx.x >> 6, c4 = lane & 15, rsub = lane >> 4;
+    const int li = lane & 31, lh = lane >> 5;
+    const int wm0 = (wv >> 1) * 32, wn0 = (wv & 1) * 32;
+    float wtop[KR ? KR : 1][4];
+#pragma unroll
+    for (int c = 0; c < KR; ++c)
+#pragma unroll
+        for (int j = 0; j < 4; ++j) wtop[c][j] = p.W[L - 1][(c * 8 + 4 * lh + j) * 64 + wn0 + li];
+#pragma unroll
+    for (int l = 0; l < L; ++l) {
+        const int skip = l == L - 1 ? KR * 512 : 0;
+#pragma unroll
+        for (int i = 0; i < 4; ++i)
+            if ((threadIdx.x + 256 * i) * 4 < 4096 - skip)
+                *reinterpret_cast<float4*>(Ws + l * 4096 + (threadIdx.x + 256 * i) * 4) =
+                    *reinterpret_cast<const float4*>(p.W[l] + skip + (threadIdx.x + 256 * i) * 4);
+    }
+    f32x16 dWa[L];
+    float dbl[L];
+#pragma unroll
+    for (int l = 0; l < L; ++l) {
+        dbl[l] = 0.f;
+#pragma unroll
+        for (int r = 0; r < 16; ++r) dWa[l][r] = 0.f;
+    }
+    float4 dbt = make_float4(0.f, 0.f, 0.f, 0.f);
+    const long long ntiles = (R + RT_ROWS - 1) / RT_ROWS;
+    const int lr0 = wv * 16 + rsub;
+    float4 gn[4], yn[L][4];
+#pragma unroll
+    for (int i = 0; i < 4; ++i) {
+        const long long row = (long long)blockIdx.x * RT_ROWS + lr0 + 4 * i;
+        gn[i] = rt_ld4(dY, row, R, c4);
+#pragma unroll
+        for (int l = 0; l < L; ++l) yn[l][i] = rt_ld4(p.y[l], row, R, c4);
+    }
+    for (long long tile = blockIdx.x; tile < ntiles; tile += gridDim.x) {
+        const long long r0 = tile * RT_ROWS, rn = (tile + gridDim.x) * RT_ROWS;
+        __syncthreads();
+#pragma unroll
+        for (int i = 0; i < 4; ++i) {
+            const int lr = lr0 + 4 * i;
+            *reinterpret_cast<float4*>(T[0] + lr * RT_LD + c4 * 4) = gn[i];
+            *reinterpret_cast<float4*>(T[1] + lr * RT_LD + c4 * 4) = yn[L - 1][i];
+            dbt.x += gn[i].x; dbt.y += gn[i].y; dbt.z += gn[i].z; dbt.w += gn[i].w;
+            gn[i] = rt_ld4(dY, rn + lr, R, c4);
+            yn[L - 1][i] = rt_ld4(p.y[L - 1], rn + lr, R, c4);
+        }
+        int g = 0, m = 1;
+#pragma unroll
+        for (int l = L - 1; l >= 0; --l) {
+            __syncthreads();
+            f32x16 acc;
+#pragma unroll
+            for (int r = 0; r < 16; ++r) acc[r] = 0.f;
+            if (l == L - 1 && KR > 0) {
+#pragma unroll
+                for (int c = 0; c < KR; ++c) {
+                    const float4 a = *reinterpret_cast<const float4*>(T[g] + (wm0 + li) * RT_LD + c * 8 + 4 * lh);
+                    acc = __builtin_amdgcn_mfma_f32_32x32x2f32(a.x, wtop[c][0], acc, 0, 0, 0);
+                    acc = __builtin_amdgcn_mfma_f32_32x32x2f32(a.y, wtop[c][1], acc, 0, 0, 0);
+                    acc = __builtin_amdgcn_mfma_f32_32x32x2f32(a.z, wtop[c][2], acc, 0, 0, 0);
+                    acc = __builtin_amdgcn_mfma_f32_32x32x2f32(a.w, wtop[c][3], acc, 0, 0, 0);
+                }
+                rt_mma_kn_lds<KR>(T[g] + wm0 * RT_LD, Ws + l * 4096 + wn0, acc);
+            } else {
+                rt_mma_kn_lds<0>(T[g] + wm0 * RT_LD, Ws + l * 4096 + wn0, acc);
+            }
+            rt_mma_rows(T[g] + wm0, T[m] + wn0, dWa[l]);
+            __syncthreads();
+#pragma unroll
+            for (int r = 0; r < 16; ++r) {
+                const int idx = (wm0 + (r & 3) + 8 * (r >> 2) + 4 * lh) * RT_LD + wn0 + li;
+                const float mk = T[m][idx];
+                float t = acc[r];
+                t = mk > 0.f ? t : 0.f * t * (mk + 1.f);
+                T[m][idx] = t;
+                if (l > 0) dbl[l - 1] += t;
+            }
+            if (l > 0) {
+#pragma unroll
+                for (int i = 0; i < 4; ++i) {
+                    const int lr = lr0 + 4 * i;
+                    *reinterpret_cast<float4*>(T[g] + lr * RT_LD + c4 * 4) = yn[l - 1][i];
+                    yn[l - 1][i] = rt_ld4(p.y[l - 1], rn + lr, R, c4);
+                }
+            }
+            const int g0 = g;
+            g = m; m = g0;
+        }
+        __syncthreads();
+#pragma unroll
+        for (int i = 0; i < 4; ++i) {
+            const int lr = lr0 + 4 * i;
+            const long long row = r0 + lr;
+            if (row < R) *reinterpret_cast<float4*>(dY0 + row * 64 + c4 * 4) = *reinterpret_cast<const float4*>(T[g] + lr * RT_LD + c4 * 4);
+        }
+    }
+    float* const sl = slab + (size_t)blockIdx.x * DVAE_CHAIN_SLAB(L);
+#pragma unroll
+    for (int l = 0; l < L; ++l)
+#pragma unroll
+        for (int r = 0; r < 16; ++r) sl[l * 4096 + (wm0 + (r & 3) + 8 * (r >> 2) + 4 * lh) * 64 + wn0 + li] = dWa[l][r];
+    __syncthreads();
+    float4* const red = reinterpret_cast<float4*>(T[0]);
+    float* const part = T[1];
+    red[(wv * 4 + rsub) * 16 + c4] = dbt;
+#pragma unroll
+    for (int l = 0; l + 1 < L; ++l) part[(l * 8 + wv * 2 + lh) * 32 + li] = dbl[l];
+    __syncthreads();
+    if (threadIdx.x < 16) {
+        float4 a = red[threadIdx.x];
+#pragma unroll
+        for (int k = 1; k < 16; ++k) { const float4 t = red[k * 16 + threadIdx.x]; a.x += t.x; a.y += t.y; a.z += t.z; a.w += t.w; }
+        *reinterpret_cast<float4*>(sl + L * 4096 + (L - 1) * 64 + threadIdx.x * 4) = a;
+    } else if (threadIdx.x >= 64 && threadIdx.x < 64 + 64 * (L - 1)) {
+        const int l = (threadIdx.x - 64) >> 6, col = threadIdx.x & 63, wn = col >> 5, i = col & 31;
+        const float* const q = part + l * 256;
+        sl[L * 4096 + l * 64 + col] = ((q[((0 * 2 + wn) * 2 + 0) * 32 + i] + q[((0 * 2 + wn) * 2 + 1) * 32 + i]) +
+                                       (q[((1 * 2 + wn) * 2 + 0) * 32 + i] + q[((1 * 2 + wn) * 2 + 1) * 32 + i]));
+    }
+}
+
+template <int L>
+__global__ __launch_bounds__(256) void dvae_chain_reduce_kernel(const float* __restrict__ slab, int nslab, const DvcGrads p) {
+    __shared__ float red[8][32];
+    const int ci = threadIdx.x & 31, grp = threadIdx.x >> 5, col = blockIdx.x * 32 + ci;
+    const int per = (nslab + 7) / 8, s0 = grp * per, s1 = min(nslab, s0 + per);
+    float a = 0.f;
+    int s = s0;
+    for (; s + 8 <= s1; s += 8) {
+        float v[8];
+#pragma unroll
+        for (int k = 0; k < 8; ++k) v[k] = slab[(size_t)(s + k) * DVAE_CHAIN_SLAB(L) + col];
+#pragma unroll
+        for (int k = 0; k < 8; ++k) a += v[k];
+    }
+    for (; s < s1; ++s) a += slab[(size_t)s * DVAE_CHAIN_SLAB(L) + col];
+    red[grp][ci] = a;
+    __syncthreads();
+    if (threadIdx.x < 32) {
+        float t = red[0][ci];
+#pragma unroll
+        for (int k = 1; k < 8; ++k) t += red[k][ci];
+        const bool w = col < L * 4096;
+        const int l = w ? col >> 12 : (col - L * 4096) >> 6;
+        float* out = nullptr;
+#pragma unroll
+        for (int k = 0; k < L; ++k)
+            if (l == k) out = w ? p.dW[k] + (col & 4095) : p.db[k] + (col & 63);
+        *out = t;
+    }
+}
+
+bool dvae_chain_built(int L) { return L == 2 || L == 3; }
+
+static long long dvc_fwd_max_wgs(int L) { return L == 2 ? 768 : 512; }
+
+void dvae_chain_plan(long long R, int L, int max_wgs, int out[3]) {
+    const long long ntiles = (R + RT_ROWS - 1) / RT_ROWS;
+    long long wgs = max_wgs > 0 && max_wgs < DVC_BWD_MAX_WGS ? max_wgs : DVC_BWD_MAX_WGS;
+    if (wgs > ntiles) wgs = ntiles;
+    out[0] = RT_ROWS; out[1] = (int)wgs; out[2] = DVAE_CHAIN_SLAB(L);
+}
+
+int dvae_chain_fwd_launch(int L, const float* y0, const float* const* W, const float* const* b, float* const* y, long long R, int max_wgs,
+                          hipStream_t st) {
+    OCRL_REQUIRE(dvae_chain_built(L), "dvae_chain_fwd: chains of 2 or 3 layers are built (got %d)", L);
+    OCRL_REQUIRE(R > 0, "dvae_chain_fwd: no rows");
+    OCRL_REQUIRE(y0 && W && b && y, "dvae_chain_fwd: null argument");
+    DvcFwd p = {};
+    for (int l = 0; l < L; ++l) {
+        OCRL_REQUIRE(W[l] && b[l] && y[l], "dvae_chain_fwd: null argument (layer %d)", l);
+        OCRL_REQUIRE(aligned16(W[l], y[l]), "dvae_chain_fwd: tensors must be 16-byte aligned");
+        p.W[l] = W[l]; p.b[l] = b[l]; p.y[l] = y[l];
+    }
+    OCRL_REQUIRE(aligned16(y0), "dvae_chain_fwd: tensors must be 16-byte aligned");
+    const long long ntiles = (R + RT_ROWS - 1) / RT_ROWS;
+    long long wgs = max_wgs > 0 && max_wgs < dvc_fwd_max_wgs(L) ? max_wgs : dvc_fwd_max_wgs(L);
+    if (wgs > ntiles) wgs = ntiles;
+    if (L == 2) hipLaunchKernelGGL(dvae_chain_fwd_kernel<2>, dim3((unsigned)wgs), dim3(256), 0, st, y0, p, R);
+    else hipLaunchKernelGGL(dvae_chain_fwd_kernel<3>, dim3((unsigned)wgs), dim3(256), 0, st, y0, p, R);
+    OCRL_CHECK_LAUNCH("dvae_chain_fwd");
+    return 0;
+}
+
+int dvae_chain_bwd_launch(int L, const float* dY, const float* const* y, const float* const* W, float* dY0, float* const* dW, float* const* db,
+                          long long R, int max_wgs, float* ws, size_t ws_floats, hipStream_t st) {
+    OCRL_REQUIRE(dvae_chain_built(L), "dvae_chain_bwd: chains of 2 or 3 layers are built (got %d)", L);
+    OCRL_REQUIRE(R > 0, "dvae_chain_bwd: no rows");
+    OCRL_REQUIRE(dY && y && W && dY0 && dW && db && ws, "dvae_chain_bwd: null argument");
+    DvcBwd p = {};
+    DvcGrads q = {};
+    for (int l = 0; l < L; ++l) {
+        OCRL_REQUIRE(W[l] && y[l] && dW[l] && db[l], "dvae_chain_bwd: null argument (layer %d)", l);
+        OCRL_REQUIRE(aligned16(W[l], y[l]), "dvae_chain_bwd: tensors must be 16-byte aligned");
+        p.W[l] = W[l]; p.y[l] = y[l]; q.dW[l] = dW[l]; q.db[l] = db[l];
+    }
+    OCRL_REQUIRE(aligned16(dY, dY0, ws), "dvae_chain_bwd: tensors must be 16-byte aligned");
+    OCRL_REQUIRE(dY != dY0, "dvae_chain_bwd: d y_0 must not overwrite the incoming gradient");
+    int plan[3];
+    dvae_chain_plan(R, L, max_wgs, plan);
+    OCRL_REQUIRE((size_t)plan[1] * plan[2] <= ws_floats, "dvae_chain_bwd: workspace too small (%d slabs of %d floats)", plan[1], plan[2]);
+    if (L == 2) {
+        hipLaunchKernelGGL(dvae_chain_bwd_kernel<2>, dim3(plan[1]), dim3(256), 0, st, dY, p, dY0, ws, R);
+        OCRL_CHECK_LAUNCH("dvae_chain_bwd");
+        hipLaunchKernelGGL(dvae_chain_reduce_kernel<2>, dim3(DVAE_CHAIN_SLAB(2) / 32), dim3(256), 0, st, ws, plan[1], q);
+    } else {
+        hipLaunchKernelGGL(dvae_chain_bwd_kernel<3>, dim3(plan[1]), dim3(256), 0, st, dY, p, dY0, ws, R);
+        OCRL_CHECK_LAUNCH("dvae_chain_bwd");
+        hipLaunchKernelGGL(dvae_chain_reduce_kernel<3>, dim3(DVAE_CHAIN_SLAB(3) / 32), dim3(256), 0, st, ws, plan[1], q);
+    }
+    OCRL_CHECK_LAUNCH("dvae_chain_reduce");
+    return 0;
+}
diff --git a/ocrl_amd/csrc/dvae_chain_unit.cpp b/ocrl_amd/csrc/dvae_chain_unit.cpp
--- /dev/null
+++ b/ocrl_amd/csrc/dvae_chain_unit.cpp
@@ -0,0 +1,26 @@
+#include "../../include/ocrl_hip_dvae_chain.h"
+#include "common.h"
+#include "kernels.h"
+
+extern "C" {
+
+int ocrl_dvae_chain_plan(long long R, int L, int out[3]) {
+    if (!out || R <= 0 || !dvae_chain_built(L)) {
+        ocrl_set_error("ocrl_dvae_chain_plan: needs R > 0, a built chain length (2 or 3 layers) and an output array");
+        return 1;
+    }
+    dvae_chain_plan(R, L, 0, out);
+    return 0;
+}
+
+int ocrl_dvae_chain_fwd(int L, const float* y0, const float* const* W, const float* const* b, float* const* y, long long R, int max_wgs,
+                        void* stream) {
+    return dvae_chain_fwd_launch(L, y0, W, b, y, R, max_wgs, static_cast<hipStream_t>(stream));
+}
+
+int ocrl_dvae_chain_bwd(int L, const float* dY, const float* const* y, const float* const* W, float* dY0, float* const* dW,
+                        float* const* db, long long R, int max_wgs, float* ws, size_t ws_floats, void* stream) {
+    return dvae_chain_bwd_launch(L, dY, y, W, dY0, dW, db, R, max_wgs, ws, ws_floats, static_cast<hipStream_t>(stream));
+}
+
+}
diff --git a/ocrl_amd/csrc/kernels.h b/ocrl_amd/csrc/kernels.h
--- a/ocrl_amd/csrc/kernels.h
+++ b/ocrl_amd/csrc/kernels.h
@@ -244,6 +244,14 @@
 int sa_input_bwd_launch(const float* dx, const float* h1, const float* e4, const float* mean, const float* rstd, const float* gamma, const float* beta,
                         const float* W0, const float* W2, float* de4, float* dW0, float* db0, float* dW2, float* db2, float* dgamma, float* dbeta,
                         long long R, int max_wgs, float* ws, size_t ws_floats, hipStream_t st);
+#define DVAE_CHAIN_MAX_L 3
+#define DVAE_CHAIN_SLAB(L) ((L) * (4096 + 64))
+bool dvae_chain_built(int L);
+void dvae_chain_plan(long long R, int L, int max_wgs, int out[3]);
+int dvae_chain_fwd_launch(int L, const float* y0, const float* const* W, const float* const* b, float* const* y, long long R, int max_wgs,
+                          hipStream_t st);
+int dvae_chain_bwd_launch(int L, const float* dY, const float* const* y, const float* const* W, float* dY0, float* const* dW, float* const* db,
+                          long long R, int max_wgs, float* ws, size_t ws_floats, hipStream_t st);
 int reduce_partials_launch(const float* part, int n, float* out, float scale, int accumulate, hipStream_t st);
 int mse_launch(const float* obs, const float* recon, float* drecon, float* out, int B, int C, int H, int W, float* ws, size_t ws_floats, hipStream_t st);
 int gumbel_softmax_launch(const float* raw, const float* e1, const float* e2, float* z, int* tokens, long long R, int V, float tau,
diff --git a/ocrl_amd/csrc/row_tile64.h b/ocrl_amd/csrc/row_tile64.h
--- /dev/null
+++ b/ocrl_amd/csrc/row_tile64.h
@@ -0,0 +1,53 @@
+#pragma once
+#include "common.h"
+
+#define RT_ROWS 64
+#define RT_LD 68
+
+__device__ __forceinline__ float4 rt_ld4(const float* __restrict__ p, long long row, long long R, int c4) {
+    const float4 v = *reinterpret_cast<const float4*>(p + (row < R ? row : R - 1) * 64 + c4 * 4);
+    return row < R ? v : make_float4(0.f, 0.f, 0.f, 0.f);
+}
+__device__ __forceinline__ float rt_ld1(const float* __restrict__ p, long long row, long long R) {
+    const float v = p[row < R ? row : R - 1];
+    return row < R ? v : 0.f;
+}
+
+__device__ __forceinline__ void rt_mma_kc(const float* __restrict__ as, const float (&wf)[8][4], f32x16& acc) {
+    const int lane = threadIdx.x & 63, li = lane & 31, lh = lane >> 5;
+#pragma unroll
+    for (int c = 0; c < 8; ++c) {
+        const float4 v = *reinterpret_cast<const float4*>(as + li * RT_LD + c * 8 + 4 * lh);
+        acc = __builtin_amdgcn_mfma_f32_32x32x2f32(v.x, wf[c][0], acc, 0, 0, 0);
+        acc = __builtin_amdgcn_mfma_f32_32x32x2f32(v.y, wf[c][1], acc, 0, 0, 0);
+        acc = __builtin_amdgcn_mfma_f32_32x32x2f32(v.z, wf[c][2], acc, 0, 0, 0);
+        acc = __builtin_amdgcn_mfma_f32_32x32x2f32(v.w, wf[c][3], acc, 0, 0, 0);
+    }
+}
+template <int C0>
+__device__ __forceinline__ void rt_mma_kn_lds(const float* __restrict__ as, const float* __restrict__ ws, f32x16& acc) {
+    const int lane = threadIdx.x & 63, li = lane & 31, lh = lane >> 5;
+#pragma unroll 2
+    for (int c = C0; c < 8; ++c) {
+        const float4 a = *reinterpret_cast<const float4*>(as + li * RT_LD + c * 8 + 4 * lh);
+        const float* const wk = ws + ((c - C0) * 8 + 4 * lh) * 64 + li;
+        acc = __builtin_amdgcn_mfma_f32_32x32x2f32(a.x, wk[0], acc, 0, 0, 0);
+        acc = __builtin_amdgcn_mfma_f32_32x32x2f32(a.y, wk[64], acc, 0, 0, 0);
+        acc = __builtin_amdgcn_mfma_f32_32x32x2f32(a.z, wk[128], acc, 0, 0, 0);
+        acc = __builtin_amdgcn_mfma_f32_32x32x2f32(a.w, wk[192], acc, 0, 0, 0);
+    }
+}
+__device__ __forceinline__ void rt_mma_rows(const float* __restrict__ as, const float* __restrict__ bs, f32x16& acc) {
+    const int lane = threadIdx.x & 63, li = lane & 31, lh = lane >> 5;
+#pragma unroll 2
+    for (int c = 0; c < 8; ++c) {
+        float fa[4], fb[4];
+#pragma unroll
+        for (int j = 0; j < 4; ++j) {
+            fa[j] = as[(c * 8 + 4 * lh + j) * RT_LD + li];
+            fb[j] = bs[(c * 8 + 4 * lh + j) * RT_LD + li];
+        }
+#pragma unroll
+        for (int s = 0; s < 4; ++s) acc = __builtin_amdgcn_mfma_f32_32x32x2f32(fa[s], fb[s], acc, 0, 0, 0);
+    }
+}
diff --git a/ocrl_amd/csrc/sa_input.hip b/ocrl_amd/csrc/sa_input.hip
--- a/ocrl_amd/csrc/sa_input.hip
+++ b/ocrl_amd/csrc/sa_input.hip
@@ -1,46 +1,12 @@
 #include "common.h"
 #include "kernels.h"
 #include "layernorm16.h"
-
-#define SAI_TR 64
-#define SAI_LD 68
+#include "row_tile64.h"
+
+#define SAI_TR RT_ROWS
+#define SAI_LD RT_LD
 #define SAI_MAX_WGS 512
 #define SAI_FWD_MAX_WGS 768
-
-__device__ __forceinline__ float4 sai_ld4(const float* __restrict__ p, long long row, long long R, int c4) {
-    const float4 v = *reinterpret_cast<const float4*>(p + (row < R ? row : R - 1) * 64 + c4 * 4);
-    return row < R ? v : make_float4(0.f, 0.f, 0.f, 0.f);
-}
-__device__ __forceinline__ float sai_ld1(const float* __restrict__ p, long long row, long long R) {
-    const float v = p[row < R ? row : R - 1];
-    return row < R ? v : 0.f;
-}
-
-__device__ __forceinline__ void sai_mma_kc(const float* __restrict__ as, const float (&wf)[8][4], f32x16& acc) {
-    const int lane = threadIdx.x & 63, li = lane & 31, lh = lane >> 5;
-#pragma unroll
-    for (int c = 0; c < 8; ++c) {
-        const float4 v = *reinterpret_cast<const float4*>(as + li * SAI_LD + c * 8 + 4 * lh);
-        acc = __builtin_amdgcn_mfma_f32_32x32x2f32(v.x, wf[c][0], acc, 0, 0, 0);
-        acc = __builtin_amdgcn_mfma_f32_32x32x2f32(v.y, wf[c][1], acc, 0, 0, 0);
-        acc = __builtin_amdgcn_mfma_f32_32x32x2f32(v.z, wf[c][2], acc, 0, 0, 0);
-        acc = __builtin_amdgcn_mfma_f32_32x32x2f32(v.w, wf[c][3], acc, 0, 0, 0);
-    }
-}
-__device__ __forceinline__ void sai_mma_rows(const float* __restrict__ as, const float* __restrict__ bs, f32x16& acc) {
-    const int lane = threadIdx.x & 63, li = lane & 31, lh = lane >> 5;
-#pragma unroll 2
-    for (int c = 0; c < 8; ++c) {
-        float fa[4], fb[4];
-#pragma unroll
-        for (int j = 0; j < 4; ++j) {
-            fa[j] = as[(c * 8 + 4 * lh + j) * SAI_LD + li];
-            fb[j] = bs[(c * 8 + 4 * lh + j) * SAI_LD + li];
-        }
-#pragma unroll
-        for (int s = 0; s < 4; ++s) acc = __builtin_amdgcn_mfma_f32_32x32x2f32(fa[s], fb[s], acc, 0, 0, 0);
-    }
-}
 
 __global__ __launch_bounds__(256, 3) void sa_input_fwd_kernel(const float* __restrict__ e4, const float* __restrict__ g, const float* __restrict__ bta,
                                                               const float* __restrict__ W0, const float* __restrict__ b0,
@@ -65,7 +31,7 @@
     const int lr0 = wv * 16 + rsub;
     float4 v[4];
 #pragma unroll
-    for (int i = 0; i < 4; ++i) v[i] = sai_ld4(e4, (long long)blockIdx.x * SAI_TR + lr0 + 4 * i, R, c4);
+    for (int i = 0; i < 4; ++i) v[i] = rt_ld4(e4, (long long)blockIdx.x * SAI_TR + lr0 + 4 * i, R, c4);
     for (long long tile = blockIdx.x; tile < ntiles; tile += gridDim.x) {
         const long long r0 = tile * SAI_TR;
 #pragma unroll
@@ -82,12 +48,12 @@
             }
         }
 #pragma unroll
-        for (int i = 0; i < 4; ++i) v[i] = sai_ld4(e4, (tile + gridDim.x) * SAI_TR + lr0 + 4 * i, R, c4);
+        for (int i = 0; i < 4; ++i) v[i] = rt_ld4(e4, (tile + gridDim.x) * SAI_TR + lr0 + 4 * i, R, c4);
         __syncthreads();
         f32x16 acc;
 #pragma unroll
         for (int r = 0; r < 16; ++r) acc[r] = 0.f;
-        sai_mma_kc(At + wm0 * SAI_LD, w0f, acc);
+        rt_mma_kc(At + wm0 * SAI_LD, w0f, acc);
 #pragma unroll
         for (int r = 0; r < 16; ++r) {
             const int row = (r & 3) + 8 * (r >> 2) + 4 * lh;
@@ -96,7 +62,7 @@
         __syncthreads();
 #pragma unroll
         for (int r = 0; r < 16; ++r) acc[r] = 0.f;
-        sai_mma_kc(Ht + wm0 * SAI_LD, w2f, acc);
+        rt_mma_kc(Ht + wm0 * SAI_LD, w2f, acc);
 #pragma unroll
         for (int r = 0; r < 16; ++r) {
             const int row = (r & 3) + 8 * (r >> 2) + 4 * lh;
@@ -146,8 +112,8 @@
     float4 dxn[4], hn[4];
 #pragma unroll
     for (int i = 0; i < 4; ++i) {
-        dxn[i] = sai_ld4(dx, (long long)blockIdx.x * SAI_TR + lr0 + 4 * i, R, c4);
-        hn[i] = sai_ld4(h1, (long long)blockIdx.x * SAI_TR + lr0 + 4 * i, R, c4);
+        dxn[i] = rt_ld4(dx, (long long)blockIdx.x * SAI_TR + lr0 + 4 * i, R, c4);
+        hn[i] = rt_ld4(h1, (long long)blockIdx.x * SAI_TR + lr0 + 4 * i, R, c4);
     }
     for (long long tile = blockIdx.x; tile < ntiles; tile += gridDim.x) {
         const long long r0 = tile * SAI_TR;
@@ -160,14 +126,14 @@
             *reinterpret_cast<float4*>(T0 + lr * SAI_LD + c4 * 4) = dxn[i];
             *reinterpret_cast<float4*>(T1 + lr * SAI_LD + c4 * 4) = hn[i];
             db2.x += dxn[i].x; db2.y += dxn[i].y; db2.z += dxn[i].z; db2.w += dxn[i].w;
-            xe[i] = sai_ld4(e4, r0 + lr, R, c4);
-            mu[i] = sai_ld1(mean, r0 + lr, R);
-            rs[i] = sai_ld1(rstd, r0 + lr, R);
-        }
-#pragma unroll
-        for (int i = 0; i < 4; ++i) {
-            dxn[i] = sai_ld4(dx, (tile + gridDim.x) * SAI_TR + lr0 + 4 * i, R, c4);
-            hn[i] = sai_ld4(h1, (tile + gridDim.x) * SAI_TR + lr0 + 4 * i, R, c4);
+            xe[i] = rt_ld4(e4, r0 + lr, R, c4);
+            mu[i] = rt_ld1(mean, r0 + lr, R);
+            rs[i] = rt_ld1(rstd, r0 + lr, R);
+        }
+#pragma unroll
+        for (int i = 0; i < 4; ++i) {
+            dxn[i] = rt_ld4(dx, (tile + gridDim.x) * SAI_TR + lr0 + 4 * i, R, c4);
+            hn[i] = rt_ld4(h1, (tile + gridDim.x) * SAI_TR + lr0 + 4 * i, R, c4);
         }
         __syncthreads();
         f32x16 acc;
@@ -199,7 +165,7 @@
             T2[idx] = t;
             db0 += t;
         }
-        sai_mma_rows(T0 + wm0, T1 + wn0, dW2a);
+        rt_mma_rows(T0 + wm0, T1 + wn0, dW2a);
         __syncthreads();
         const float4 gg = *reinterpret_cast<const float4*>(g + c4 * 4), bb = *reinterpret_cast<const float4*>(bta + c4 * 4);
 #pragma unroll
@@ -221,7 +187,7 @@
 #pragma unroll
         for (int r = 0; r < 16; ++r) T0[(wm0 + (r & 3) + 8 * (r >> 2) + 4 * lh) * SAI_LD + wn0 + li] = acc[r];
         __syncthreads();
-        sai_mma_rows(T2 + wm0, T1 + wn0, dW0a);
+        rt_mma_rows(T2 + wm0, T1 + wn0, dW0a);
 #pragma unroll
         for (int i = 0; i < 4; ++i) {
             const int lr = lr0 + 4 * i;
diff --git a/ocrl_amd/csrc/slate_model.cpp b/ocrl_amd/csrc/slate_model.cpp
--- a/ocrl_amd/csrc/slate_model.cpp
+++ b/ocrl_amd/csrc/slate_model.cpp
@@ -412,14 +412,31 @@
     return 0;
 }
 
+int SlateModel::dvae_chain_fwd(const ParamPair* layers, int n, const float* y0, float* const* y, long long R, const Lane& L) {
+    const float *W[DVAE_CHAIN_MAX_L], *b[DVAE_CHAIN_MAX_L];
+    for (int l = 0; l < n; ++l) { W[l] = P(layers[l].w); b[l] = P(layers[l].b); }
+    return dvae_chain_fwd_launch(n, y0, W, b, y, R, 0, L);
+}
+
+int SlateModel::dvae_chain_bwd(const ParamPair* layers, int n, const float* dy, const float* const* y, float* dy0, long long R, const Lane& L) {
+    const float* W[DVAE_CHAIN_MAX_L];
+    float *dW[DVAE_CHAIN_MAX_L], *db[DVAE_CHAIN_MAX_L];
+    for (int l = 0; l < n; ++l) { W[l] = P(layers[l].w); dW[l] = G(layers[l].w); db[l] = G(layers[l].b); }
+    int plan[3];
+    dvae_chain_plan(R, n, 0, plan);
+    const size_t slabs = L.scratch_floats / plan[2];
+    OCRL_REQUIRE(slabs >= 1, "bwd_dvae: scratch too small for the layer-chain slabs");
+    return dvae_chain_bwd_launch(n, dy, y, W, dy0, dW, db, R, slabs < (size_t)plan[1] ? (int)slabs : 0, L.scratch, L.scratch_floats, L);
+}
+
 int SlateModel::fwd_dvae(const StepInputs& in, const Lane& L) {
     const int B = in.B;
     const long long BT = (long long)B * T, BN = (long long)B * N;
     const int ch = cfg.obs_channels;
     RC(patchify4_launch(in.obs, patches_, B, ch, S, L));
     RC(lin_fwd(patches_, 16 * ch, P(w_.dvae_enc[0].w), P(w_.dvae_enc[0].b), de_[0], 64, BT, 64, 16 * ch, 1, nullptr, 0, 0.f, 0, L));
-    for (int i = 1; i < 7; ++i)
-        RC(lin_fwd(de_[i - 1], 64, P(w_.dvae_enc[i].w), P(w_.dvae_enc[i].b), de_[i], 64, BT, 64, 64, 1, nullptr, 0, 0.f, 0, L));
+    RC(dvae_chain_fwd(w_.dvae_enc + 1, 3, de_[0], de_ + 1, BT, L));
+    RC(dvae_chain_fwd(w_.dvae_enc + 4, 3, de_[3], de_ + 4, BT, L));
     if (fused_heads()) {
         GemmArgs a;
         a.A = de_[6]; a.B = P(w_.dvae_enc[7].w); a.C = zraw_; a.M = (int)BT; a.N = V; a.K = 64; a.lda = 64; a.ldb = 64; a.ldc = V;
@@ -452,13 +469,13 @@
     RC(lin_fwd(zin, V, P(w_.dvae_dec[0].w), P(w_.dvae_dec[0].b), dd0_, 64, BT, 64, V, 1, nullptr, 0, 0.f, 0, L));
     }
     RC(conv_layer_fwd(dd0_, dw_fwd_[0], P(w_.dvae_dec[1].b), dd1_, B, E, E, 3, 64, 1, nullptr, nullptr, L));
-    RC(lin_fwd(dd1_, 64, P(w_.dvae_dec[2].w), P(w_.dvae_dec[2].b), dd2_, 64, BT, 64, 64, 1, nullptr, 0, 0.f, 0, L));
-    RC(lin_fwd(dd2_, 64, P(w_.dvae_dec[3].w), P(w_.dvae_dec[3].b), dd3_, 64, BT, 64, 64, 1, nullptr, 0, 0.f, 0, L));
+    float* const y23[2] = {dd2_, dd3_};
+    RC(dvae_chain_fwd(w_.dvae_dec + 2, 2, dd1_, y23, BT, L));
     RC(lin_fwd(dd3_, 64, P(w_.dvae_dec[4].w), P(w_.dvae_dec[4].b), dd4_, 256, BT, 256, 64, 1, nullptr, 0, 0.f, 0, L));
     RC(pixel_shuffle_launch(dd4_, ps1_, B, E, E, 64, 1, nullptr, L));
     RC(conv_layer_fwd(ps1_, dw_fwd_[1], P(w_.dvae_dec[6].b), dd6_, B, 2 * E, 2 * E, 3, 64, 1, nullptr, nullptr, L));
-    RC(lin_fwd(dd6_, 64, P(w_.dvae_dec[7].w), P(w_.dvae_dec[7].b), dd7_, 64, 4 * BT, 64, 64, 1, nullptr, 0, 0.f, 0, L));
-    RC(lin_fwd(dd7_, 64, P(w_.dvae_dec[8].w), P(w_.dvae_dec[8].b), dd8_, 64, 4 * BT, 64, 64, 1, nullptr, 0, 0.f, 0, L));
+    float* const y78[2] = {dd7_, dd8_};
+    RC(dvae_chain_fwd(w_.dvae_dec + 7, 2, dd6_, y78, 4 * BT, L));
     RC(lin_fwd(dd8_, 64, P(w_.dvae_dec[9].w), P(w_.dvae_dec[9].b), dd9_, 256, 4 * BT, 256, 64, 1, nullptr, 0, 0.f, 0, L));
     RC(pixel_shuffle_launch(dd9_, ps2_, B, 2 * E, 2 * E, 64, 1, nullptr, L));
     RC(lin_fwd(ps2_, 64, P(w_.dvae_dec[11].w), P(w_.dvae_dec[11].b), recon_, 4, BN, ch, 64, 0, nullptr, 0, 0.f, 0, L));
@@ -875,19 +892,15 @@
     RC(pixel_shuffle_launch(gdA_, gdB_, B, 2 * E, 2 * E, 64, 0, dd9_, L));
     RC(lin_bwd_w(gdB_, 256, dd8_, 64, G(w_.dvae_dec[9].w), G(w_.dvae_dec[9].b), 4 * BT, 256, 64, 1.f, L));
     RC(lin_bwd_x(gdB_, 256, P(w_.dvae_dec[9].w), gdA_, 64, 4 * BT, 256, 64, dd8_, 64, nullptr, 0, L));
-    RC(lin_bwd_w(gdA_, 64, dd7_, 64, G(w_.dvae_dec[8].w), G(w_.dvae_dec[8].b), 4 * BT, 64, 64, 1.f, L));
-    RC(lin_bwd_x(gdA_, 64, P(w_.dvae_dec[8].w), gdB_, 64, 4 * BT, 64, 64, dd7_, 64, nullptr, 0, L));
-    RC(lin_bwd_w(gdB_, 64, dd6_, 64, G(w_.dvae_dec[7].w), G(w_.dvae_dec[7].b), 4 * BT, 64, 64, 1.f, L));
-    RC(lin_bwd_x(gdB_, 64, P(w_.dvae_dec[7].w), gdA_, 64, 4 * BT, 64, 64, dd6_, 64, nullptr, 0, L));
-    RC(conv_layer_wgrad(ps1_, gdA_, G(w_.dvae_dec[6].w), G(w_.dvae_dec[6].b), B, 2 * E, 2 * E, 3, 64, 64, L));
-    RC(conv_layer_fwd(gdA_, dw_bwd_[1], nullptr, gdB_, B, 2 * E, 2 * E, 3, 64, 0, nullptr, ps1_, L));
-    RC(pixel_shuffle_launch(gdB_, gdA_, B, E, E, 64, 0, nullptr, L));
-    RC(lin_bwd_w(gdA_, 256, dd3_, 64, G(w_.dvae_dec[4].w), G(w_.dvae_dec[4].b), BT, 256, 64, 1.f, L));
-    RC(lin_bwd_x(gdA_, 256, P(w_.dvae_dec[4].w), gdB_, 64, BT, 256, 64, dd3_, 64, nullptr, 0, L));
-    RC(lin_bwd_w(gdB_, 64, dd2_, 64, G(w_.dvae_dec[3].w), G(w_.dvae_dec[3].b), BT, 64, 64, 1.f, L));
-    RC(lin_bwd_x(gdB_, 64, P(w_.dvae_dec[3].w), gdA_, 64, BT, 64, 64, dd2_, 64, nullptr, 0, L));
-    RC(lin_bwd_w(gdA_, 64, dd1_, 64, G(w_.dvae_dec[2].w), G(w_.dvae_dec[2].b), BT, 64, 64, 1.f, L));
-    RC(lin_bwd_x(gdA_, 64, P(w_.dvae_dec[2].w), gdB_, 64, BT, 64, 64, dd1_, 64, nullptr, 0, L));
+    const float* const y67[2] = {dd6_, dd7_};
+    RC(dvae_chain_bwd(w_.dvae_dec + 7, 2, gdA_, y67, gdB_, 4 * BT, L));
+    RC(conv_layer_wgrad(ps1_, gdB_, G(w_.dvae_dec[6].w), G(w_.dvae_dec[6].b), B, 2 * E, 2 * E, 3, 64, 64, L));
+    RC(conv_layer_fwd(gdB_, dw_bwd_[1], nullptr, gdA_, B, 2 * E, 2 * E, 3, 64, 0, nullptr, ps1_, L));
+    RC(pixel_shuffle_launch(gdA_, gdB_, B, E, E, 64, 0, nullptr, L));
+    RC(lin_bwd_w(gdB_, 256, dd3_, 64, G(w_.dvae_dec[4].w), G(w_.dvae_dec[4].b), BT, 256, 64, 1.f, L));
+    RC(lin_bwd_x(gdB_, 256, P(w_.dvae_dec[4].w), gdA_, 64, BT, 256, 64, dd3_, 64, nullptr, 0, L));
+    const float* const y12[2] = {dd1_, dd2_};
+    RC(dvae_chain_bwd(w_.dvae_dec + 2, 2, gdA_, y12, gdB_, BT, L));
     RC(conv_layer_wgrad(dd0_, gdB_, G(w_.dvae_dec[1].w), G(w_.dvae_dec[1].b), B, E, E, 3, 64, 64, L));
     RC(conv_layer_fwd(gdB_, dw_bwd_[0], nullptr, gdA_, B, E, E, 3, 64, 0, nullptr, dd0_, L));
     float* dz = zraw_;
@@ -907,14 +920,9 @@
     }
     RC(lin_bwd_w(dz, V, de_[6], 64, G(w_.dvae_enc[7].w), G(w_.dvae_enc[7].b), BT, V, 64, 1.f, L));
     RC(lin_bwd_x(dz, V, P(w_.dvae_enc[7].w), gdA_, 64, BT, V, 64, de_[6], 64, nullptr, 0, L));
-    float* cur = gdA_;
-    float* oth = gdB_;
-    for (int i = 6; i >= 1; --i) {
-        RC(lin_bwd_w(cur, 64, de_[i - 1], 64, G(w_.dvae_enc[i].w), G(w_.dvae_enc[i].b), BT, 64, 64, 1.f, L));
-        RC(lin_bwd_x(cur, 64, P(w_.dvae_enc[i].w), oth, 64, BT, 64, 64, de_[i - 1], 64, nullptr, 0, L));
-        float* t = cur; cur = oth; oth = t;
-    }
-    RC(lin_bwd_w(cur, 64, patches_, 16 * ch, G(w_.dvae_enc[0].w), G(w_.dvae_enc[0].b), BT, 64, 16 * ch, 1.f, L));
+    RC(dvae_chain_bwd(w_.dvae_enc + 4, 3, gdA_, de_ + 3, gdB_, BT, L));
+    RC(dvae_chain_bwd(w_.dvae_enc + 1, 3, gdB_, de_, gdA_, BT, L));
+    RC(lin_bwd_w(gdA_, 64, patches_, 16 * ch, G(w_.dvae_enc[0].w), G(w_.dvae_enc[0].b), BT, 64, 16 * ch, 1.f, L));
     return 0;
 }
 
diff --git a/ocrl_amd/csrc/slate_model.h b/ocrl_amd/csrc/slate_model.h
--- a/ocrl_amd/csrc/slate_model.h
+++ b/ocrl_amd/csrc/slate_model.h
@@ -77,6 +77,8 @@
     int fwd_dvae(const StepInputs& in, const Lane& L);
     int fwd_decoder(const Lane& L, bool with_ce = true);
     int dvae_decode(int B, float* drecon, const Lane& L, const float* zin = nullptr);
+    int dvae_chain_fwd(const ParamPair* layers, int n, const float* y0, float* const* y, long long R, const Lane& L);
+    int dvae_chain_bwd(const ParamPair* layers, int n, const float* dy, const float* const* y, float* dy0, long long R, const Lane& L);
     int bwd_decoder(const Lane& L);
     int bwd_encoder(const Lane& L, BwdDvae fork = BwdDvae::SerialLast);
     int bwd_dvae(const Lane& L);
```

Result: no change. 1812 (-0.0%).
